# omerbt/Splice

Measured on AMD Instinct MI355X. Metric: opt_steps_per_sec, higher is better.
Workload: dtype bf16

## Files before the change

### include/splice_hip.h

```cpp
#ifndef SPLICE_HIP_H
#define SPLICE_HIP_H
#include <stddef.h>
#include <stdint.h>

#ifdef __cplusplus
extern "C" {
#endif

typedef uint16_t splice_bf16;
typedef void* splice_stream_t;

#define SPLICE_OK 0
#define SPLICE_ERR_ARG -1
#define SPLICE_ERR_HIP -2
#define SPLICE_ERR_STATE -3
#define SPLICE_ERR_NOMEM -4

int splice_version(void);
int splice_dev_switches(void);
const char* splice_last_error(void);

typedef struct splice_gemm_epilogue {
    const float* bias;
    const float* resid;
    int ldr, resid_mod;
    float* out_f32;
    int ldo;
    splice_bf16* out_bf;
    int ldbf;
    splice_bf16* out_bf_t;
    int ldt;
    splice_bf16* out_pre;
    int ldp, pre_row_lo;
    const splice_bf16* aux;
    int ldaux;
    float* out_f32_cols;
    int ld_cols, col_lo, col_hi;
    float alpha;
    int ksplit;
    long long slab_stride;
    const splice_bf16* rd_other;
    int ld_rd, rd_rows;
    float* rowdot;
    const float* row_scale;
    const float* col_scale;
    uint8_t* out_f8;
    int ld8;
    uint8_t* out_f8_t;
    int ldt8;
} splice_gemm_epilogue;

enum {
    SPLICE_EPI_BIAS = 1, SPLICE_EPI_RESID = 2, SPLICE_EPI_OUT_F32 = 4, SPLICE_EPI_OUT_BF = 8,
    SPLICE_EPI_OUT_T = 16, SPLICE_EPI_GELU = 32, SPLICE_EPI_GELU_GRAD = 64,
    SPLICE_EPI_COLS_F32 = 128, SPLICE_EPI_ALPHA = 256, SPLICE_EPI_ROWDOT = 512, SPLICE_EPI_SCALE_RC = 1024, SPLICE_EPI_OUT_F8 = 2048,
    SPLICE_EPI_OUT_F8T = 4096
};

int splice_gemm_nt_bf16(unsigned flags, const splice_bf16* A, int lda, const splice_bf16* B, int ldb,
                        int M, int N, int K, const splice_gemm_epilogue* epi, splice_stream_t stream);

int splice_gemm_nt_fp8(unsigned flags, const uint8_t* A, int lda, const uint8_t* B, int ldb, int M, int N, int K,
                       const splice_gemm_epilogue* epi, splice_stream_t stream);
int splice_quantize_rows_fp8(const float* x, int ldx, uint8_t* q, int ldq, float* scale, int rows, int cols, splice_stream_t stream);
int splice_gemm_splitk_slabs(int M, int ksplit);
int splice_gemm_force_tile(int tile);
int splice_attention_variant(int variant);
int splice_attention_qfold(int on);
int splice_attention_bwd_variant(int variant);

int splice_layernorm_fwd(const float* x, const float* gamma, const float* beta, splice_bf16* y,
                         float* mean, float* rstd, int rows, int D, float eps, splice_stream_t stream);
int splice_layernorm_bwd(const float* dy, const float* x, const float* gamma, const float* mean,
                         const float* rstd, const float* g_in, float* g_out, splice_bf16* g_out_bf,
                         int rows, int D, splice_stream_t stream);

int splice_attention_fwd(const splice_bf16* qkv, const splice_bf16* qkvT, int ldt, int B, int T, int Tld,
                         int D, int H, float scale, splice_bf16* out, float* lse, splice_stream_t stream);
int splice_attention_fwd_fp8(const uint8_t* qkv8, const uint8_t* qkvT8, int ldt8, int B, int T, int Tld, int D, int H, float scale,
                             splice_bf16* out, float* lse, splice_stream_t stream);
int splice_attention_bwd(const splice_bf16* qkv, const splice_bf16* qkvT, int ldt, int B, int T, int Tld,
                         int D, int H, float scale, const splice_bf16* out, const float* lse,
                         const splice_bf16* dout, const splice_bf16* doutT, float* delta,
                         splice_bf16* dqkv, splice_stream_t stream);
int splice_attention_probs(const splice_bf16* qkv, int B, int T, int Tld, int D, int H, float scale,
                           const float* lse, float* probs, splice_stream_t stream);

int splice_augment_structure(const float* img, float* out, float* scratch, int H, int W, int flip, int n_ops, const int* order,
                             const float* factors, float blur_sigma, splice_stream_t stream);

size_t splice_keys_selfsim_ws_bytes(int T, int D);
int splice_keys_selfsim_fwd(const float* K, int ldk, int T, int D, float eps, float* S, void* ws,
                            splice_stream_t stream);
int splice_keys_selfsim_bwd(const float* dS, const float* S, int T, int D, float eps, float* dK, int lddk,
                            int accumulate, void* ws, splice_stream_t stream);

int splice_mse(const float* a, int lda, const float* b, int ldb, int rows, int cols, float weight,
               float* loss_accum, float* grad, int ldg, splice_stream_t stream);

int splice_patchify(const float* img, splice_bf16* patches, int B, int H, int W, int p, int Tld,
                    int normalize, splice_stream_t stream);
int splice_unpatchify(const float* dpatches, float* dimg, int B, int H, int W, int p, int Tld,
                      int normalize, splice_stream_t stream);
int splice_cast_f32_bf16(const float* x, splice_bf16* y, size_t n, splice_stream_t stream);
int splice_cast_bf16_f32(const splice_bf16* x, float* y, size_t n, splice_stream_t stream);
int splice_transpose_f32_bf16(const float* x, splice_bf16* y, int rows, int cols, int ldy, splice_stream_t stream);
int splice_resize_bilinear_fwd(const float* in, float* out, int planes, int h, int w, int oh, int ow, splice_stream_t stream);
int splice_resize_bilinear_bwd(const float* dout, float* din, int planes, int h, int w, int oh, int ow, splice_stream_t stream);

int splice_vit_create(int patch, int dim, int depth, int heads, void** out_handle);
void splice_vit_destroy(void* vit);
int splice_vit_set_param(void* vit, const char* name, const float* data, long long numel, splice_stream_t stream);
float splice_vit_qscale(void* vit);
int splice_vit_params_complete(void* vit);
int splice_vit_enable_fp8(void* vit, splice_stream_t stream);
int splice_vit_ctx_create(void* vit, int B, int H, int W, const float* pos_TD, int need_grad,
                          splice_stream_t stream, void** out_ctx);
void splice_vit_ctx_destroy(void* ctx);
int splice_vit_ctx_info(void* ctx, int* T, int* Tld, int* rows);
int splice_vit_ctx_set_top_cls_only(void* ctx, int on);
int splice_vit_ctx_set_fp8(void* ctx, int mode);
int splice_vit_forward(void* ctx, const float* img, int normalize, splice_stream_t stream);
int splice_vit_forward_ex(void* ctx, const float* img, int normalize, int grad_pass_begin, splice_stream_t stream);
int splice_vit_forward_passes(void* ctx, const float* img, int normalize, int grad_pass_begin, int pass_begin, int pass_end,
                              splice_stream_t stream);
int splice_vit_get_tensor(void* ctx, int kind, int layer, void** out_ptr);
int splice_vit_read_tensor(void* ctx, int kind, int layer, void* dst, size_t bytes, splice_stream_t stream);
int splice_vit_backward(void* ctx, int pass_begin, int pass_end, const float* const* d_block,
                        const float* const* d_qkv, const float* const* d_keys, float* d_img,
                        int normalize, splice_stream_t stream);

int splice_gen_create(void** out_handle);
#define SPLICE_GEN_MAX_SCALES 6
typedef struct splice_gen_arch {
    int n_scales, in_channels, out_channels;
    int down[SPLICE_GEN_MAX_SCALES], up[SPLICE_GEN_MAX_SCALES], skip[SPLICE_GEN_MAX_SCALES];
    int filter_down[SPLICE_GEN_MAX_SCALES], filter_up[SPLICE_GEN_MAX_SCALES];
    int filter_skip;
    int reflect;
} splice_gen_arch;
int splice_gen_create_arch(const splice_gen_arch* arch, void** out_handle);
void splice_gen_destroy(void* gen);
long long splice_gen_param_count(void* gen);
int splice_gen_num_tensors(void* gen);
int splice_gen_tensor_info(void* gen, int i, const char** name, long long* offset, long long* numel);
int splice_gen_plan_create(void* gen, int N, int H, int W, int need_grad, void** out_plan);
void splice_gen_plan_destroy(void* plan);
int splice_gen_forward(void* plan, const float* params, const float* x, float* y, splice_stream_t stream);
int splice_gen_forward_borrowed(void* plan, const float* params, const float* x, float* y, splice_stream_t stream);
int splice_gen_backward(void* plan, const float* params, const float* dy, float* grads, int accumulate,
                        splice_stream_t stream);
long long splice_gen_buffer_count(void* gen);
int splice_gen_num_buffers(void* gen);
int splice_gen_buffer_info(void* gen, int i, const char** name, long long* offset, long long* numel);
int splice_gen_running_stats_update(void* const* plans, int n_plans, float* running, long long running_stride, float momentum,
                                    splice_stream_t stream);
int splice_adam_step(float* params, float* grads, float* m, float* v, long long n, float lr, float beta1,
                     float beta2, float eps, int step, int zero_grad, splice_stream_t stream);
int splice_optim_step(int kind, float* params, float* grads, float* m, float* v, long long n, float lr, float hp0, float hp1,
                      float eps, int step, int zero_grad, splice_stream_t stream);
int splice_optim_step_ex(int kind, float* params, float* grads, const float* g2, float* m, float* v, long long n, float lr,
                         const float* lr_dev, float hp0, float hp1, float eps, int step, int zero_grad, splice_stream_t stream);
int splice_optim_step_pairs(int kind, float* params, float* grads, const float* g2, float* m, float* v, int n_pairs, long long stride,
                            long long n, const float* lr_dev, float hp0, float hp1, float eps, int step, int zero_grad,
                            splice_stream_t stream);
int splice_optim_step_ema(int kind, float* params, float* grads, const float* g2, float* m, float* v, float* ema, long long n, float lr,
                          const float* lr_dev, float hp0, float hp1, float eps, int step, int zero_grad, float ema_decay, int ema_start,
                          splice_stream_t stream);

int splice_prof_begin(int which);
int splice_prof_end(float* total_ms, int* launches);
int splice_prof_end_ex(float* total_ms, int* calls, int* kernels);
int splice_prof_end_detail(float* total_ms, int* calls, int* kernels, char* detail, int detail_len);
int splice_prof_active(void);
int splice_vit_ctx_dims(void* ctx, int* B, int* H, int* W, int* D, int* depth, int* heads, int* patch);
int splice_gen_plan_dims(void* plan, int* N, int* H, int* W, long long* nparams);
int splice_gen_plan_set_arena_stride(void* plan, long long stride);
int splice_gen_plan_set_batch_stats(void* plan, int on);
int splice_gen_plan_set_groups(void* plan, int images_per_group);
int splice_gen_plan_resize(void* plan, int H, int W);

typedef struct splice_step_config {
    int crop_h, crop_w;
    int vit_h, vit_w;
    int ent_h, ent_w;
    int ent_vit_h, ent_vit_w;
    float lambda_global_cls, lambda_global_ssim, lambda_global_identity, lambda_entire_cls, lambda_entire_ssim;
    int entire_every, cls_warmup;
    float lr, beta1, beta2, eps;
    int pairs;
    long long arena_stride;
    int fp8_selfsim;
    int top_cls_only;
    int n_crops;
    int n_crops_b;
} splice_step_config;
#define SPLICE_STEP_MAX_PAIR_CFGS 32
#define SPLICE_STEP_MAX_GROUP_IMAGES 32
int splice_step_create(const splice_step_config* cfg, void* vit_ctx_global, void* vit_ctx_entire, void* gen_plan_a, void* gen_plan_b,
                       void* gen_plan_entire, void** out_handle);
void splice_step_destroy(void* step);
int splice_step_run(void* step, float* params, float* grads, float* m, float* v, const float* A_crop, const float* B_crop,
                    const float* A_entire, int step_idx, float* losses_out, splice_stream_t stream);
int splice_step_output(void* step, int which, float** out_ptr);
int splice_step_graph_stats(void* step, long long* out);
int splice_step_use_graph(void* step, int on);
int splice_step_use_overlap(void* step, int on);
int splice_step_set_crops(void* step, int a_h, int a_w, int b_h, int b_w);
int splice_step_set_mode(void* step, int skip_adam, int accumulate);
int splice_step_set_optimizer(void* step, int kind, float hp0, float hp1, float eps);
int splice_step_set_lr(void* step, float lr);
int splice_step_set_pair_weights(void* step, const float* lambdas);
int splice_step_set_pair_lr(void* step, const float* lr);
int splice_step_set_phases(void* step, int phases, void* leader);
int splice_step_set_running_stats(void* step, float* running, long long stride);

typedef struct splice_stop_state {
    float sum;
    int count;
    int windows;
    float best;
    int bad;
    int stop_step;
} splice_stop_state;
int splice_step_set_stop_rule(void* step, int window, float rel, int patience, int min_steps);
int splice_step_stop_state(void* step, splice_stop_state* out, splice_stream_t stream);
int splice_plateau_update(splice_stop_state* state, const float* losses8, int pairs, int window, float rel, int patience, int min_steps,
                          int step_idx, int counted, splice_stream_t stream);

int splice_step_set_ema(void* step, float* ema, float decay, int start);
int splice_optim_step_pairs_ema(int kind, float* params, float* grads, const float* g2, float* m, float* v, float* ema, int n_pairs,
                                long long stride, long long n, const float* lr_dev, float hp0, float hp1, float eps, const int* step_dev,
                                const splice_stop_state* stop, int zero_grad, float ema_decay, int ema_start, splice_stream_t stream);

#define SPLICE_CLIP_CHUNK 4096
typedef struct splice_clip_state {
    float sumsq;
    float norm;
    float coef;
    int skip;
    int clipped;
    int skipped;
} splice_clip_state;
int splice_grad_norm_pairs(const float* grads, const float* g2, int n_pairs, long long stride, long long n, float max_norm, float* partials,
                           splice_clip_state* state, const splice_stop_state* stop, const int* step_dev, splice_stream_t stream);
int splice_optim_step_pairs_clip(int kind, float* params, float* grads, const float* g2, float* m, float* v, float* ema, int n_pairs,
                                 long long stride, long long n, const float* lr_dev, float hp0, float hp1, float eps, const int* step_dev,
                                 const splice_stop_state* stop, int zero_grad, float ema_decay, int ema_start, const splice_clip_state* clip,
                                 splice_stream_t stream);
int splice_optim_step_clip(int kind, float* params, float* grads, const float* g2, float* m, float* v, float* ema, long long n, float lr,
                           const float* lr_dev, float hp0, float hp1, float eps, int step, int zero_grad, float ema_decay, int ema_start,
                           const splice_clip_state* clip, splice_stream_t stream);
int splice_step_set_grad_clip(void* step, float max_norm, splice_clip_state* state);

#define SPLICE_STOP_HISTORY 64
typedef struct splice_best_state {
    int best_step;
    int best_window;
} splice_best_state;
int splice_plateau_update_best(splice_stop_state* state, splice_best_state* best, float* means, const float* losses8, int pairs, int window,
                               float rel, int patience, int min_steps, int step_idx, int counted, splice_stream_t stream);
int splice_optim_step_pairs_best(int kind, float* params, float* grads, const float* g2, float* m, float* v, float* ema, int n_pairs,
                                 long long stride, long long n, const float* lr_dev, float hp0, float hp1, float eps, const int* step_dev,
                                 const splice_stop_state* stop, int zero_grad, float ema_decay, int ema_start, const splice_clip_state* clip,
                                 const splice_best_state* best, float* best_params, float* best_ema, splice_stream_t stream);
int splice_step_set_keep_best(void* step, float* best_params, float* best_ema, splice_best_state* state, float* means);

int splice_step_set_loss_trace(void* step, float* trace, int capacity);

typedef struct splice_lr_state {
    float scale;
    int bad;
    int cuts;
    int last_cut_step;
} splice_lr_state;
int splice_step_set_lr_plateau(void* step, float factor, int patience, float min_scale, splice_lr_state* state, int* cut_steps);
int splice_plateau_update_lr(splice_stop_state* state, splice_lr_state* lr_state, int* cut_steps, const float* losses8, const float* lr_in,
                             int per_pair, float* lr_eff, int pairs, int window, float rel, int patience, int min_steps, float factor,
                             int lr_patience, float min_scale, int step_idx, int counted, splice_stream_t stream);

size_t splice_selfsim_loss_pairs_ws_bytes(int T, int D, int pairs);
int splice_selfsim_loss_pairs(const splice_bf16* k_tgt, const splice_bf16* k_x, int ldk, size_t k_pstride, const splice_bf16* kT_x, int ldt,
                              size_t kT_pstride, int T, int D, int pairs, float lambda, const float* e_scale_tab, int fp8, float eps,
                              float* loss_part, size_t part_pstride, float* dk, int lddk, size_t dk_pstride, void* ws, splice_stream_t stream);
int splice_mse_pairs(const float* a, int lda, size_t a_ps, const float* b, int ldb, size_t b_ps, int rows, int cols, float loss_weight,
                     float grad_weight, float* part, size_t part_ps, float* grad, int ldg, size_t g_ps, int pairs, const float* grad_tab,
                     splice_stream_t stream);
int splice_total_loss_pairs(float* lbase, size_t lstride, int lp, float w_ssim, float w_essim, float w_ecls, float w_cls, float w_id,
                            float* out8, int pairs, int n_a, int n_b, int n_c, int n_e, const float* wtab, int ssim_on, int entire,
                            splice_stream_t stream);
int splice_total_loss_pairs_trace(float* lbase, size_t lstride, int lp, float w_ssim, float w_essim, float w_ecls, float w_cls, float w_id,
                                  float* out8, int pairs, int n_a, int n_b, int n_c, int n_e, const float* wtab, int ssim_on, int entire,
                                  splice_stop_state* stop, int window, float rel, int patience, int min_steps, const int* dev_t,
                                  float* trace, int capacity, splice_stream_t stream);

int splice_attn_cls_fwd(const splice_bf16* qkv, const splice_bf16* qkvT, int ldt, int B, int T, int Tld, int D, int H, float scale, splice_bf16* out,
                        float* probs, splice_stream_t stream);
int splice_attn_cls_bwd(const splice_bf16* qkv, const splice_bf16* qkvT, int ldt, int B, int T, int Tld, int D, int H, float scale, const float* probs,
                        const float* dout_slabs, int n_slabs, size_t slab_stride, splice_bf16* dqkv, splice_stream_t stream);
int splice_ln_rows_fwd(float* x, size_t xs, const float* gamma, const float* beta, splice_bf16* y, size_t ys, float* mean, float* rstd, size_t ss,
                       int rows, int D, float eps, const float* slabs, int n_slabs, size_t slab_stride, const float* bias, const float* resid, size_t rs,
                       splice_stream_t stream);
int splice_ln_rows_bwd(float* dy, size_t dys, const float* x, size_t xs, const float* gamma, const float* mean, const float* rstd, size_t ss, float* g,
                       splice_bf16* g_bf, int rows, int D, int n_slabs, size_t slab_stride, splice_stream_t stream);
int splice_rows_finish(int mode, const float* slabs, int n_slabs, size_t slab_stride, int rows, int N, const float* bias, const float* resid, size_t rs,
                       float* out_f32, size_t os, splice_bf16* out_bf, splice_bf16* pre_bf, const splice_bf16* aux, size_t ps, int pre_lo,
                       splice_stream_t stream);

typedef struct splice_gen_conv_args {
    const float* in;
    const float* w;
    const float* bias;
    float* out;
    size_t in_nstride, in_cstride, out_nstride, out_cstride, w_jstride, w_cstride, p_nstride;
    int N, Cin, Hi, Wi, Cout, Ho, Wo, ks, stride, pad;
    int reflect, act, transposed, accumulate;
    float* ws;
    size_t ws_floats;
    int p_group, defer_reduce;
} splice_gen_conv_args;
#define SPLICE_GEN_CONV_FORM_INTS 5
int splice_gen_conv(const splice_gen_conv_args* args, int* form_out, splice_stream_t stream);
int splice_gen_conv_pair(const splice_gen_conv_args* a, const splice_gen_conv_args* b, int* forms_out, splice_stream_t stream);
int splice_gen_conv_reflect_dgrad(const splice_gen_conv_args* args, float* pad_scratch, size_t scratch_floats, splice_stream_t stream);

typedef struct splice_gen_wgrad_args {
    const float* x;
    const float* dy;
    float* ws;
    size_t ws_floats;
    size_t x_nstride, x_cstride, dy_nstride, dy_cstride;
    int N, Cin, Hi, Wi, Cout, Ho, Wo, ks, stride, pad, reflect;
} splice_gen_wgrad_args;
#define SPLICE_GEN_WGRAD_FORM_INTS 6
size_t splice_gen_conv_wgrad_ws_floats(int N, int Cin, int Cout, int ks, int Ho, int Wo);
int splice_gen_conv_wgrad(const splice_gen_wgrad_args* args, float* dw, int accumulate, int n_img, size_t p_nstride, int* form_out,
                          splice_stream_t stream);

typedef struct splice_gen_bn_args {
    float* y;
    float* out;
    size_t y_nstride, out_nstride;
    int N, C, HW, batch;
    const float* gamma;
    const float* beta;
    float eps, slope;
    size_t p_nstride;
    float* part;
    size_t part_floats;
    float* mean;
    float* rstd;
    const float* up_src;
    float* up_d_src;
    size_t up_src_ns, up_d_src_ns;
    int up_c0, up_h, up_w, up_Ho, up_Wo;
    const float* slabs;
    const float* bias;
    int ksplit;
    const float* da;
    float* dy;
    size_t da_nstride, dy_nstride;
    float* dgamma;
    float* dbeta;
    int accumulate;
    const float* da_slabs;
    int da_ksplit, da_accumulate;
    float* pre_y;
    size_t pre_y_ns;
    const float* pre_slabs;
    const float* pre_bias;
    int pre_ksplit, pre_C;
    const float* pre_gamma;
    const float* pre_beta;
    float* pre_mean;
    float* pre_rstd;
    float pre_slope;
    float* pre_dy;
    float* pre_dgamma;
    float* pre_dbeta;
} splice_gen_bn_args;
#define SPLICE_GEN_BN_FORM_INTS 7
int splice_gen_bn_form(int HW, int N, size_t p_nstride, int batch, int* out);
size_t splice_gen_bn_part_floats(int N, int C);
int splice_gen_bn_fwd(const splice_gen_bn_args* args, splice_stream_t stream);
int splice_gen_bn_bwd(const splice_gen_bn_args* args, splice_stream_t stream);

int splice_gen_upsample2x_fwd(const float* in, size_t in_nstride, float* out, size_t out_nstride, int N, int C, int h, int w, int Ho, int Wo,
                              splice_stream_t stream);
int splice_gen_upsample2x_bwd(const float* dout, size_t dout_nstride, float* din, size_t din_nstride, int N, int C, int h, int w, int Ho, int Wo,
                              splice_stream_t stream);
size_t splice_gen_sigmoid_bias_part_floats(int N, int C);
int splice_gen_sigmoid_bwd_bias(const float* dout, const float* sout, float* dpre, int N, int C, int HW, float* part, size_t part_floats,
                                size_t p_nstride, int group, int* chunks_out, splice_stream_t stream);

#ifdef __cplusplus
}
#endif
#endif
```

### splice_amd/_lib.py

```python
import ctypes as C
import os

_HERE = os.path.dirname(os.path.abspath(__file__))
LIB_PATH = os.path.join(_HERE, "libsplice_hip.so")

_lib = None


class GemmEpilogue(C.Structure):
    _fields_ = [
        ("bias", C.c_void_p), ("resid", C.c_void_p), ("ldr", C.c_int), ("resid_mod", C.c_int),
        ("out_f32", C.c_void_p), ("ldo", C.c_int),
        ("out_bf", C.c_void_p), ("ldbf", C.c_int),
        ("out_bf_t", C.c_void_p), ("ldt", C.c_int),
        ("out_pre", C.c_void_p), ("ldp", C.c_int), ("pre_row_lo", C.c_int),
        ("aux", C.c_void_p), ("ldaux", C.c_int),
        ("out_f32_cols", C.c_void_p), ("ld_cols", C.c_int), ("col_lo", C.c_int), ("col_hi", C.c_int),
        ("alpha", C.c_float), ("ksplit", C.c_int), ("slab_stride", C.c_longlong),
        ("rd_other", C.c_void_p), ("ld_rd", C.c_int), ("rd_rows", C.c_int), ("rowdot", C.c_void_p),
        ("row_scale", C.c_void_p), ("col_scale", C.c_void_p),
        ("out_f8", C.c_void_p), ("ld8", C.c_int),
        ("out_f8_t", C.c_void_p), ("ldt8", C.c_int),
    ]


class GenArch(C.Structure):
    _fields_ = [("n_scales", C.c_int), ("in_channels", C.c_int), ("out_channels", C.c_int),
                ("down", C.c_int * 6), ("up", C.c_int * 6), ("skip", C.c_int * 6),
                ("filter_down", C.c_int * 6), ("filter_up", C.c_int * 6), ("filter_skip", C.c_int), ("reflect", C.c_int)]


class StepConfig(C.Structure):
    _fields_ = [
        ("crop_h", C.c_int), ("crop_w", C.c_int), ("vit_h", C.c_int), ("vit_w", C.c_int),
        ("ent_h", C.c_int), ("ent_w", C.c_int), ("ent_vit_h", C.c_int), ("ent_vit_w", C.c_int),
        ("lambda_global_cls", C.c_float), ("lambda_global_ssim", C.c_float), ("lambda_global_identity", C.c_float),
        ("lambda_entire_cls", C.c_float), ("lambda_entire_ssim", C.c_float),
        ("entire_every", C.c_int), ("cls_warmup", C.c_int),
        ("lr", C.c_float), ("beta1", C.c_float), ("beta2", C.c_float), ("eps", C.c_float),
        ("pairs", C.c_int), ("arena_stride", C.c_longlong), ("fp8_selfsim", C.c_int), ("top_cls_only", C.c_int), ("n_crops", C.c_int), ("n_crops_b", C.c_int),
    ]


class StopState(C.Structure):
    _fields_ = [("sum", C.c_float), ("count", C.c_int), ("windows", C.c_int), ("best", C.c_float), ("bad", C.c_int), ("stop_step", C.c_int)]


class ClipState(C.Structure):
    _fields_ = [("sumsq", C.c_float), ("norm", C.c_float), ("coef", C.c_float), ("skip", C.c_int), ("clipped", C.c_int), ("skipped", C.c_int)]


class BestState(C.Structure):
    _fields_ = [("best_step", C.c_int), ("best_window", C.c_int)]


class LrState(C.Structure):
    _fields_ = [("scale", C.c_float), ("bad", C.c_int), ("cuts", C.c_int), ("last_cut_step", C.c_int)]


class GenConvArgs(C.Structure):
    _fields_ = [("in", C.c_void_p), ("w", C.c_void_p), ("bias", C.c_void_p), ("out", C.c_void_p)] + \
               [(n, C.c_size_t) for n in ("in_nstride", "in_cstride", "out_nstride", "out_cstride", "w_jstride", "w_cstride", "p_nstride")] + \
               [(n, C.c_int) for n in ("N", "Cin", "Hi", "Wi", "Cout", "Ho", "Wo", "ks", "stride", "pad", "reflect", "act", "transposed", "accumulate")] + \
               [("ws", C.c_void_p), ("ws_floats", C.c_size_t), ("p_group", C.c_int), ("defer_reduce", C.c_int)]


class GenWgradArgs(C.Structure):
    _fields_ = [("x", C.c_void_p), ("dy", C.c_void_p), ("ws", C.c_void_p), ("ws_floats", C.c_size_t)] + \
               [(n, C.c_size_t) for n in ("x_nstride", "x_cstride", "dy_nstride", "dy_cstride")] + \
               [(n, C.c_int) for n in ("N", "Cin", "Hi", "Wi", "Cout", "Ho", "Wo", "ks", "stride", "pad", "reflect")]


class GenBnArgs(C.Structure):
    _fields_ = [("y", C.c_void_p), ("out", C.c_void_p), ("y_nstride", C.c_size_t), ("out_nstride", C.c_size_t),
                ("N", C.c_int), ("C", C.c_int), ("HW", C.c_int), ("batch", C.c_int),
                ("gamma", C.c_void_p), ("beta", C.c_void_p), ("eps", C.c_float), ("slope", C.c_float), ("p_nstride", C.c_size_t),
                ("part", C.c_void_p), ("part_floats", C.c_size_t), ("mean", C.c_void_p), ("rstd", C.c_void_p),
                ("up_src", C.c_void_p), ("up_d_src", C.c_void_p), ("up_src_ns", C.c_size_t), ("up_d_src_ns", C.c_size_t),
                ("up_c0", C.c_int), ("up_h", C.c_int), ("up_w", C.c_int), ("up_Ho", C.c_int), ("up_Wo", C.c_int),
                ("slabs", C.c_void_p), ("bias", C.c_void_p), ("ksplit", C.c_int),
                ("da", C.c_void_p), ("dy", C.c_void_p), ("da_nstride", C.c_size_t), ("dy_nstride", C.c_size_t),
                ("dgamma", C.c_void_p), ("dbeta", C.c_void_p), ("accumulate", C.c_int),
                ("da_slabs", C.c_void_p), ("da_ksplit", C.c_int), ("da_accumulate", C.c_int),
                ("pre_y", C.c_void_p), ("pre_y_ns", C.c_size_t), ("pre_slabs", C.c_void_p), ("pre_bias", C.c_void_p),
                ("pre_ksplit", C.c_int), ("pre_C", C.c_int), ("pre_gamma", C.c_void_p), ("pre_beta", C.c_void_p),
                ("pre_mean", C.c_void_p), ("pre_rstd", C.c_void_p), ("pre_slope", C.c_float),
                ("pre_dy", C.c_void_p), ("pre_dgamma", C.c_void_p), ("pre_dbeta", C.c_void_p)]


GEN_CONV_FORM_INTS, GEN_WGRAD_FORM_INTS, GEN_BN_FORM_INTS = 5, 6, 7

STOP_HISTORY = 64

EPI_BIAS, EPI_RESID, EPI_OUT_F32, EPI_OUT_BF, EPI_OUT_T = 1, 2, 4, 8, 16
EPI_GELU, EPI_GELU_GRAD, EPI_COLS_F32, EPI_ALPHA, EPI_ROWDOT, EPI_SCALE_RC, EPI_OUT_F8, EPI_OUT_F8T = 32, 64, 128, 256, 512, 1024, 2048, 4096

_vp, _i, _f, _sz, _u = C.c_void_p, C.c_int, C.c_float, C.c_size_t, C.c_uint

_SIGNATURES = {
    "splice_version": ([], C.c_int),
    "splice_dev_switches": ([], C.c_int),
    "splice_last_error": ([], C.c_char_p),
    "splice_gemm_nt_bf16": ([_u, _vp, _i, _vp, _i, _i, _i, _i, C.POINTER(GemmEpilogue), _vp], _i),
    "splice_gemm_nt_fp8": ([_u, _vp, _i, _vp, _i, _i, _i, _i, C.POINTER(GemmEpilogue), _vp], _i),
    "splice_quantize_rows_fp8": ([_vp, _i, _vp, _i, _vp, _i, _i, _vp], _i),
    "splice_gemm_splitk_slabs": ([_i, _i], _i),
    "splice_gemm_force_tile": ([_i], _i),
    "splice_attention_variant": ([_i], _i),
    "splice_attention_qfold": ([_i], _i),
    "splice_attention_bwd_variant": ([_i], _i),
    "splice_layernorm_fwd": ([_vp, _vp, _vp, _vp, _vp, _vp, _i, _i, _f, _vp], _i),
    "splice_layernorm_bwd": ([_vp, _vp, _vp, _vp, _vp, _vp, _vp, _vp, _i, _i, _vp], _i),
    "splice_attention_fwd": ([_vp, _vp, _i, _i, _i, _i, _i, _i, _f, _vp, _vp, _vp], _i),
    "splice_attention_fwd_fp8": ([_vp, _vp, _i, _i, _i, _i, _i, _i, _f, _vp, _vp, _vp], _i),
    "splice_attention_bwd": ([_vp, _vp, _i, _i, _i, _i, _i, _i, _f, _vp, _vp, _vp, _vp, _vp, _vp, _vp], _i),
    "splice_attention_probs": ([_vp, _i, _i, _i, _i, _i, _f, _vp, _vp, _vp], _i),
    "splice_augment_structure": ([_vp, _vp, _vp, _i, _i, _i, _i, C.POINTER(C.c_int), C.POINTER(C.c_float), _f, _vp], _i),
    "splice_keys_selfsim_ws_bytes": ([_i, _i], _sz),
    "splice_keys_selfsim_fwd": ([_vp, _i, _i, _i, _f, _vp, _vp, _vp], _i),
    "splice_keys_selfsim_bwd": ([_vp, _vp, _i, _i, _f, _vp, _i, _i, _vp, _vp], _i),
    "splice_mse": ([_vp, _i, _vp, _i, _i, _i, _f, _vp, _vp, _i, _vp], _i),
    "splice_selfsim_loss_pairs_ws_bytes": ([_i, _i, _i], _sz),
    "splice_selfsim_loss_pairs": ([_vp, _vp, _i, _sz, _vp, _i, _sz, _i, _i, _i, _f, _vp, _i, _f, _vp, _sz, _vp, _i, _sz, _vp, _vp], _i),
    "splice_mse_pairs": ([_vp, _i, _sz, _vp, _i, _sz, _i, _i, _f, _f, _vp, _sz, _vp, _i, _sz, _i, _vp, _vp], _i),
    "splice_total_loss_pairs": ([_vp, _sz, _i, _f, _f, _f, _f, _f, _vp, _i, _i, _i, _i, _i, _vp, _i, _i, _vp], _i),
    "splice_attn_cls_fwd": ([_vp, _vp, _i, _i, _i, _i, _i, _i, _f, _vp, _vp, _vp], _i),
    "splice_attn_cls_bwd": ([_vp, _vp, _i, _i, _i, _i, _i, _i, _f, _vp, _vp, _i, _sz, _vp, _vp], _i),
    "splice_ln_rows_fwd": ([_vp, _sz, _vp, _vp, _vp, _sz, _vp, _vp, _sz, _i, _i, _f, _vp, _i, _sz, _vp, _vp, _sz, _vp], _i),
    "splice_ln_rows_bwd": ([_vp, _sz, _vp, _sz, _vp, _vp, _vp, _sz, _vp, _vp, _i, _i, _i, _sz, _vp], _i),
    "splice_rows_finish": ([_i, _vp, _i, _sz, _i, _i, _vp, _vp, _sz, _vp, _sz, _vp, _vp, _vp, _sz, _i, _vp], _i),
    "splice_gen_conv": ([C.POINTER(GenConvArgs), C.POINTER(_i), _vp], _i),
    "splice_gen_conv_pair": ([C.POINTER(GenConvArgs), C.POINTER(GenConvArgs), C.POINTER(_i), _vp], _i),
    "splice_gen_conv_reflect_dgrad": ([C.POINTER(GenConvArgs), _vp, _sz, _vp], _i),
    "splice_gen_conv_wgrad_ws_floats": ([_i, _i, _i, _i, _i, _i], _sz),
    "splice_gen_conv_wgrad": ([C.POINTER(GenWgradArgs), _vp, _i, _i, _sz, C.POINTER(_i), _vp], _i),
    "splice_gen_bn_form": ([_i, _i, _sz, _i, C.POINTER(_i)], _i),
    "splice_gen_bn_part_floats": ([_i, _i], _sz),
    "splice_gen_bn_fwd": ([C.POINTER(GenBnArgs), _vp], _i),
    "splice_gen_bn_bwd": ([C.POINTER(GenBnArgs), _vp], _i),
    "splice_gen_upsample2x_fwd": ([_vp, _sz, _vp, _sz, _i, _i, _i, _i, _i, _i, _vp], _i),
    "splice_gen_upsample2x_bwd": ([_vp, _sz, _vp, _sz, _i, _i, _i, _i, _i, _i, _vp], _i),
    "splice_gen_sigmoid_bias_part_floats": ([_i, _i], _sz),
    "splice_gen_sigmoid_bwd_bias": ([_vp, _vp, _vp, _i, _i, _i, _vp, _sz, _sz, _i, C.POINTER(_i), _vp], _i),
    "splice_patchify": ([_vp, _vp, _i, _i, _i, _i, _i, _i, _vp], _i),
    "splice_unpatchify": ([_vp, _vp, _i, _i, _i, _i, _i, _i, _vp], _i),
    "splice_cast_f32_bf16": ([_vp, _vp, _sz, _vp], _i),
    "splice_cast_bf16_f32": ([_vp, _vp, _sz, _vp], _i),
    "splice_transpose_f32_bf16": ([_vp, _vp, _i, _i, _i, _vp], _i),
    "splice_resize_bilinear_fwd": ([_vp, _vp, _i, _i, _i, _i, _i, _vp], _i),
    "splice_resize_bilinear_bwd": ([_vp, _vp, _i, _i, _i, _i, _i, _vp], _i),
    "splice_vit_create": ([_i, _i, _i, _i, C.POINTER(_vp)], _i),
    "splice_vit_destroy": ([_vp], None),
    "splice_vit_set_param": ([_vp, C.c_char_p, _vp, C.c_longlong, _vp], _i),
    "splice_vit_params_complete": ([_vp], _i),
    "splice_vit_enable_fp8": ([_vp, _vp], _i),
    "splice_vit_ctx_create": ([_vp, _i, _i, _i, _vp, _i, _vp, C.POINTER(_vp)], _i),
    "splice_vit_ctx_destroy": ([_vp], None),
    "splice_vit_ctx_info": ([_vp, C.POINTER(_i), C.POINTER(_i), C.POINTER(_i)], _i),
    "splice_vit_ctx_set_top_cls_only": ([_vp, _i], _i),
    "splice_vit_ctx_set_fp8": ([_vp, _i], _i),
    "splice_vit_forward": ([_vp, _vp, _i, _vp], _i),
    "splice_vit_forward_ex": ([_vp, _vp, _i, _i, _vp], _i),
    "splice_vit_forward_passes": ([_vp, _vp, _i, _i, _i, _i, _vp], _i),
    "splice_vit_get_tensor": ([_vp, _i, _i, C.POINTER(_vp)], _i),
    "splice_vit_qscale": ([_vp], C.c_float),
    "splice_vit_read_tensor": ([_vp, _i, _i, _vp, _sz, _vp], _i),
    "splice_vit_backward": ([_vp, _i, _i, C.POINTER(_vp), C.POINTER(_vp), C.POINTER(_vp), _vp, _i, _vp], _i),
    "splice_gen_create": ([C.POINTER(_vp)], _i),
    "splice_gen_create_arch": ([C.POINTER(GenArch), C.POINTER(_vp)], _i),
    "splice_gen_destroy": ([_vp], None),
    "splice_gen_param_count": ([_vp], C.c_longlong),
    "splice_gen_num_tensors": ([_vp], _i),
    "splice_gen_tensor_info": ([_vp, _i, C.POINTER(C.c_char_p), C.POINTER(C.c_longlong), C.POINTER(C.c_longlong)], _i),
    "splice_gen_plan_create": ([_vp, _i, _i, _i, _i, C.POINTER(_vp)], _i),
    "splice_gen_plan_destroy": ([_vp], None),
    "splice_gen_forward": ([_vp, _vp, _vp, _vp, _vp], _i),
    "splice_gen_forward_borrowed": ([_vp, _vp, _vp, _vp, _vp], _i),
    "splice_gen_backward": ([_vp, _vp, _vp, _vp, _i, _vp], _i),
    "splice_adam_step": ([_vp, _vp, _vp, _vp, C.c_longlong, _f, _f, _f, _f, _i, _i, _vp], _i),
    "splice_optim_step": ([_i, _vp, _vp, _vp, _vp, C.c_longlong, _f, _f, _f, _f, _i, _i, _vp], _i),
    "splice_optim_step_ex": ([_i, _vp, _vp, _vp, _vp, _vp, C.c_longlong, _f, _vp, _f, _f, _f, _i, _i, _vp], _i),
    "splice_optim_step_pairs": ([_i, _vp, _vp, _vp, _vp, _vp, _i, C.c_longlong, C.c_longlong, _vp, _f, _f, _f, _i, _i, _vp], _i),
    "splice_optim_step_ema": ([_i, _vp, _vp, _vp, _vp, _vp, _vp, C.c_longlong, _f, _vp, _f, _f, _f, _i, _i, _f, _i, _vp], _i),
    "splice_optim_step_pairs_ema": ([_i, _vp, _vp, _vp, _vp, _vp, _vp, _i, C.c_longlong, C.c_longlong, _vp, _f, _f, _f, _vp, _vp, _i, _f, _i, _vp], _i),
    "splice_step_set_ema": ([_vp, _vp, _f, _i], _i),
    "splice_grad_norm_pairs": ([_vp, _vp, _i, C.c_longlong, C.c_longlong, _f, _vp, _vp, _vp, _vp, _vp], _i),
    "splice_optim_step_pairs_clip": ([_i, _vp, _vp, _vp, _vp, _vp, _vp, _i, C.c_longlong, C.c_longlong, _vp, _f, _f, _f, _vp, _vp, _i, _f, _i, _vp, _vp], _i),
    "splice_optim_step_clip": ([_i, _vp, _vp, _vp, _vp, _vp, _vp, C.c_longlong, _f, _vp, _f, _f, _f, _i, _i, _f, _i, _vp, _vp], _i),
    "splice_step_set_grad_clip": ([_vp, _f, _vp], _i),
    "splice_plateau_update_best": ([_vp, _vp, _vp, _vp, _i, _i, _f, _i, _i, _i, _i, _vp], _i),
    "splice_optim_step_pairs_best": ([_i, _vp, _vp, _vp, _vp, _vp, _vp, _i, C.c_longlong, C.c_longlong, _vp, _f, _f, _f, _vp, _vp, _i, _f, _i, _vp, _vp, _vp, _vp, _vp], _i),
    "splice_step_set_keep_best": ([_vp, _vp, _vp, _vp, _vp], _i),
    "splice_step_set_loss_trace": ([_vp, _vp, _i], _i),
    "splice_total_loss_pairs_trace": ([_vp, _sz, _i, _f, _f, _f, _f, _f, _vp, _i, _i, _i, _i, _i, _vp, _i, _i, _vp, _i, _f, _i, _i, _vp, _vp, _i, _vp], _i),
    "splice_step_set_lr_plateau": ([_vp, _f, _i, _f, _vp, _vp], _i),
    "splice_plateau_update_lr": ([_vp, _vp, _vp, _vp, _vp, _i, _vp, _i, _i, _f, _i, _i, _f, _i, _f, _i, _i, _vp], _i),
    "splice_prof_begin": ([_i], _i),
    "splice_prof_end": ([C.POINTER(_f), C.POINTER(_i)], _i),
    "splice_prof_end_ex": ([C.POINTER(_f), C.POINTER(_i), C.POINTER(_i)], _i),
    "splice_prof_end_detail": ([C.POINTER(_f), C.POINTER(_i), C.POINTER(_i), C.c_char_p, _i], _i),
    "splice_prof_active": ([], _i),
    "splice_step_use_graph": ([_vp, _i], _i),
    "splice_step_graph_stats": ([_vp, C.POINTER(C.c_longlong)], _i),
    "splice_step_use_overlap": ([_vp, _i], _i),
    "splice_vit_ctx_dims": ([_vp] + [C.POINTER(_i)] * 7, _i),
    "splice_gen_plan_dims": ([_vp, C.POINTER(_i), C.POINTER(_i), C.POINTER(_i), C.POINTER(C.c_longlong)], _i),
    "splice_step_create": ([C.POINTER(StepConfig), _vp, _vp, _vp, _vp, _vp, C.POINTER(_vp)], _i),
    "splice_step_destroy": ([_vp], None),
    "splice_step_run": ([_vp, _vp, _vp, _vp, _vp, _vp, _vp, _vp, _i, _vp, _vp], _i),
    "splice_step_output": ([_vp, _i, C.POINTER(_vp)], _i),
    "splice_step_set_crops": ([_vp, _i, _i, _i, _i], _i),
    "splice_step_set_running_stats": ([_vp, _vp, C.c_longlong], _i),
    "splice_step_set_mode": ([_vp, _i, _i], _i),
    "splice_step_set_optimizer": ([_vp, _i, _f, _f, _f], _i),
    "splice_step_set_lr": ([_vp, _f], _i),
    "splice_step_set_pair_weights": ([_vp, _vp], _i),
    "splice_step_set_pair_lr": ([_vp, _vp], _i),
    "splice_step_set_phases": ([_vp, _i, _vp], _i),
    "splice_step_set_stop_rule": ([_vp, _i, _f, _i, _i], _i),
    "splice_step_stop_state": ([_vp, _vp, _vp], _i),
    "splice_plateau_update": ([_vp, _vp, _i, _i, _f, _i, _i, _i, _i, _vp], _i),
    "splice_gen_buffer_count": ([_vp], C.c_longlong),
    "splice_gen_num_buffers": ([_vp], _i),
    "splice_gen_buffer_info": ([_vp, _i, C.POINTER(C.c_char_p), C.POINTER(C.c_longlong), C.POINTER(C.c_longlong)], _i),
    "splice_gen_running_stats_update": ([C.POINTER(_vp), _i, _vp, C.c_longlong, _f, _vp], _i),
    "splice_gen_plan_resize": ([_vp, _i, _i], _i),
    "splice_gen_plan_set_arena_stride": ([_vp, C.c_longlong], _i),
    "splice_gen_plan_set_batch_stats": ([_vp, _i], _i),
    "splice_gen_plan_set_groups": ([_vp, _i], _i),
}


def exported_symbols():
    return sorted(_SIGNATURES)


def register(name, argtypes, restype):
    _SIGNATURES[name] = (argtypes, restype)


def lib():
    global _lib
    if _lib is None:
        if not os.path.exists(LIB_PATH):
            raise RuntimeError(
                f"{LIB_PATH} not found: the HIP extension is not built "
                "(run __graft_entry__.build() or `make -C splice_amd/csrc`). There is no CPU fallback.")
        _lib = C.CDLL(LIB_PATH)
        for name, (argtypes, restype) in _SIGNATURES.items():
            fn = getattr(_lib, name)
            fn.argtypes = argtypes
            fn.restype = restype
    return _lib


def check(rc, what=""):
    if rc != 0:
        msg = lib().splice_last_error().decode(errors="replace")
        raise RuntimeError(f"libsplice_hip {what} failed (rc={rc}): {msg}")


def ptr(t):
    return None if t is None else C.c_void_p(t.data_ptr())


def current_stream():
    import torch
    return C.c_void_p(torch.cuda.current_stream().cuda_stream)
```

### splice_amd/csrc/capi.hip

```cpp
#include <stdarg.h>
#include <stdio.h>

#include "gen_kernels.h"
#include "kernels.h"

static thread_local char g_err[512] = "";

void splice_set_error(const char* fmt, ...) {
    va_list ap;
    va_start(ap, fmt);
    vsnprintf(g_err, sizeof(g_err), fmt, ap);
    va_end(ap);
}

static int finish(int rc, const char* what) {
    if (rc != SPLICE_OK) {
        splice_set_error("%s: invalid argument", what);
        return rc;
    }
    const hipError_t e = hipGetLastError();
    if (e != hipSuccess) {
        splice_set_error("%s: HIP error %d (%s)", what, (int)e, hipGetErrorString(e));
        return SPLICE_ERR_HIP;
    }
    return SPLICE_OK;
}

#define ST(s) ((hipStream_t)(s))

extern "C" {

int splice_version(void) { return 100; }
int splice_dev_switches(void) {
#ifdef SPLICE_DEV_SWITCHES
    return 1;
#else
    return 0;
#endif
}
const char* splice_last_error(void) { return g_err; }

int splice_gemm_nt_bf16(unsigned flags, const splice_bf16* A, int lda, const splice_bf16* B, int ldb, int M, int N, int K,
                        const splice_gemm_epilogue* epi, splice_stream_t stream) {
    if (!A || !B || !epi) return finish(SPLICE_ERR_ARG, "splice_gemm_nt_bf16");
    return finish(gemm_nt_launch(flags, A, lda, B, ldb, M, N, K, *epi, ST(stream)), "splice_gemm_nt_bf16");
}

int splice_gemm_nt_fp8(unsigned flags, const uint8_t* A, int lda, const uint8_t* B, int ldb, int M, int N, int K,
                       const splice_gemm_epilogue* epi, splice_stream_t stream) {
    if (!A || !B || !epi) return finish(SPLICE_ERR_ARG, "splice_gemm_nt_fp8");
    return finish(gemm_nt_fp8_launch(flags, A, lda, B, ldb, M, N, K, *epi, ST(stream)), "splice_gemm_nt_fp8");
}
int splice_quantize_rows_fp8(const float* x, int ldx, uint8_t* q, int ldq, float* scale, int rows, int cols, splice_stream_t stream) {
    if (!x || !q || !scale) return finish(SPLICE_ERR_ARG, "splice_quantize_rows_fp8");
    return finish(quantize_rows_fp8_launch(x, ldx, q, ldq, scale, rows, cols, ST(stream)), "splice_quantize_rows_fp8");
}

int splice_gemm_splitk_slabs(int M, int ksplit) { return gemm_splitk_slabs(M, ksplit); }

int splice_gemm_force_tile(int tile) { gemm_force_tile(tile); return SPLICE_OK; }
int splice_attention_variant(int variant) { attn_set_variant(variant); return SPLICE_OK; }
int splice_attention_qfold(int on) { attn_set_qfold(on); return SPLICE_OK; }
int splice_attention_bwd_variant(int variant) { attn_set_bwd_variant(variant); return SPLICE_OK; }

int splice_layernorm_fwd(const float* x, const float* gamma, const float* beta, splice_bf16* y, float* mean, float* rstd,
                         int rows, int D, float eps, splice_stream_t stream) {
    return finish(layernorm_fwd_launch(x, gamma, beta, y, mean, rstd, rows, D, eps, ST(stream)), "splice_layernorm_fwd");
}
int splice_layernorm_bwd(const float* dy, const float* x, const float* gamma, const float* mean, const float* rstd,
                         const float* g_in, float* g_out, splice_bf16* g_out_bf, int rows, int D, splice_stream_t stream) {
    return finish(layernorm_bwd_launch(dy, x, gamma, mean, rstd, g_in, g_out, g_out_bf, rows, D, ST(stream)), "splice_layernorm_bwd");
}

int splice_attention_fwd(const splice_bf16* qkv, const splice_bf16* qkvT, int ldt, int B, int T, int Tld, int D, int H,
                         float scale, splice_bf16* out, float* lse, splice_stream_t stream) {
    AttnArgs a = {};
    a.qkv = qkv; a.qkvT = qkvT; a.ldt = ldt; a.B = B; a.T = T; a.Tld = Tld; a.D = D; a.H = H; a.scale = scale;
    a.out = out; a.lse = lse; a.qfold = attn_qfold_hook();
    return finish(attn_fwd_launch(&a, ST(stream)), "splice_attention_fwd");
}
int splice_attention_fwd_fp8(const uint8_t* qkv8, const uint8_t* qkvT8, int ldt8, int B, int T, int Tld, int D, int H, float scale,
                             splice_bf16* out, float* lse, splice_stream_t stream) {
    if (!qkv8 || !qkvT8 || !out || !lse) return finish(SPLICE_ERR_ARG, "splice_attention_fwd_fp8");
    AttnArgs a = {};
    a.qkv8 = qkv8; a.qkvT8 = qkvT8; a.ldt8 = ldt8; a.ldt = 4; a.B = B; a.T = T; a.Tld = Tld; a.D = D; a.H = H; a.scale = scale;
    a.out = out; a.lse = lse;
    return finish(attn_fwd_launch(&a, ST(stream)), "splice_attention_fwd_fp8");
}
int splice_attention_bwd(const splice_bf16* qkv, const splice_bf16* qkvT, int ldt, int B, int T, int Tld, int D, int H,
                         float scale, const splice_bf16* out, const float* lse, const splice_bf16* dout,
                         const splice_bf16* doutT, float* delta, splice_bf16* dqkv, splice_stream_t stream) {
    AttnArgs a = {};
    a.qkv = qkv; a.qkvT = qkvT; a.ldt = ldt; a.B = B; a.T = T; a.Tld = Tld; a.D = D; a.H = H; a.scale = scale;
    a.out = const_cast<splice_bf16*>(out); a.lse = const_cast<float*>(lse);
    a.dout = dout; a.doutT = doutT; a.delta = delta; a.dqkv = dqkv; a.qfold = attn_qfold_hook();
    return finish(attn_bwd_launch(&a, ST(stream)), "splice_attention_bwd");
}
int splice_attention_probs(const splice_bf16* qkv, int B, int T, int Tld, int D, int H, float scale, const float* lse,
                           float* probs, splice_stream_t stream) {
    AttnArgs a = {};
    a.qkv = qkv; a.B = B; a.T = T; a.Tld = Tld; a.D = D; a.H = H; a.scale = scale; a.lse = const_cast<float*>(lse);
    return finish(attn_probs_launch(&a, probs, ST(stream)), "splice_attention_probs");
}

int splice_augment_structure(const float* img, float* out, float* scratch, int H, int W, int flip, int n_ops, const int* order,
                             const float* factors, float blur_sigma, splice_stream_t stream) {
    return finish(augment_structure_launch(img, out, scratch, H, W, flip, n_ops, order, factors, blur_sigma, ST(stream)), "splice_augment_structure");
}

size_t splice_keys_selfsim_ws_bytes(int T, int D) { return selfsim_ws_bytes(T, D); }
int splice_keys_selfsim_fwd(const float* K, int ldk, int T, int D, float eps, float* S, void* ws, splice_stream_t stream) {
    SelfSimWs w;
    selfsim_ws_carve(ws, T, D, &w);
    return finish(selfsim_fwd_launch(K, ldk, T, D, eps, S, w, ST(stream)), "splice_keys_selfsim_fwd");
}
int splice_keys_selfsim_bwd(const float* dS, const float* S, int T, int D, float eps, float* dK, int lddk, int accumulate,
                            void* ws, splice_stream_t stream) {
    SelfSimWs w;
    selfsim_ws_carve(ws, T, D, &w);
    return finish(selfsim_bwd_launch(dS, S, T, D, eps, dK, lddk, accumulate, w, ST(stream)), "splice_keys_selfsim_bwd");
}
int splice_mse(const float* a, int lda, const float* b, int ldb, int rows, int cols, float weight, float* loss_accum,
               float* grad, int ldg, splice_stream_t stream) {
    return finish(mse_launch(a, lda, b, ldb, rows, cols, weight, loss_accum, grad, ldg, ST(stream)), "splice_mse");
}

size_t splice_selfsim_loss_pairs_ws_bytes(int T, int D, int pairs) { return selfsim_batch_ws_bytes(T, D, pairs); }
int splice_selfsim_loss_pairs(const splice_bf16* k_tgt, const splice_bf16* k_x, int ldk, size_t k_pstride, const splice_bf16* kT_x, int ldt,
                              size_t kT_pstride, int T, int D, int pairs, float lambda, const float* e_scale_tab, int fp8, float eps,
                              float* loss_part, size_t part_pstride, float* dk, int lddk, size_t dk_pstride, void* ws, splice_stream_t stream) {
    const char* who = "splice_selfsim_loss_pairs";
    if (!k_tgt || !k_x || !kT_x || !loss_part || !dk || !ws || T < 1 || pairs < 1 || D < 64 || D % 64 || ldk < D || ldk % 8 || ldt % 8 ||
        k_pstride % 8 || kT_pstride % 8 || lddk < D)
        return finish(SPLICE_ERR_ARG, who);
    const int nt = (T + 63) / 64;
    if ((fp8 && D % 128) || (size_t)(nt * (nt + 1) / 2) > part_pstride) return finish(SPLICE_ERR_ARG, who);
    SelfSimBatch b = {};
    selfsim_batch_carve(ws, T, D, pairs, &b);
    b.ldk = ldk; b.ldt = ldt; b.k_pstride = k_pstride; b.kT_pstride = kT_pstride;
    b.k_tgt = k_tgt; b.k_x = k_x; b.kT_x = kT_x;
    b.loss_part = loss_part; b.part_pstride = part_pstride;
    b.dk = dk; b.dk_pstride = dk_pstride; b.lddk = lddk;
    b.eps = eps;
    b.fp8 = fp8 != 0;
    b.loss_scale = 1.0f / ((float)T * (float)T);
    b.e_scale = 4.0f * lambda * b.loss_scale;
    b.e_scale_tab = e_scale_tab;
    const int rc = selfsim_target_launch(b, ST(stream));
    if (rc != SPLICE_OK) return finish(rc, who);
    return finish(selfsim_loss_launch(b, ST(stream)), who);
}
int splice_mse_pairs(const float* a, int lda, size_t a_ps, const float* b, int ldb, size_t b_ps, int rows, int cols, float loss_weight,
                     float grad_weight, float* part, size_t part_ps, float* grad, int ldg, size_t g_ps, int pairs, const float* grad_tab,
                     splice_stream_t stream) {
    if (!a || !b || rows < 1 || cols < 1) return finish(SPLICE_ERR_ARG, "splice_mse_pairs");
    return finish(mse_batched_launch(a, lda, a_ps, b, ldb, b_ps, rows, cols, loss_weight, grad_weight, part, part_ps, grad, ldg, g_ps, pairs,
                                     ST(stream), grad_tab),
                  "splice_mse_pairs");
}

static bool attn_cls_args_ok(const void* qkv, const void* qkvT, int ldt, int B, int T, int Tld, int D, int H, size_t lds) {
    if (!qkv || !qkvT || B < 1 || T < 1 || T > Tld || Tld % 32 || ldt % 8 || (long long)ldt < (long long)B * Tld || D < 64 || D % 64 || H != D / 64)
        return false;
    int dev = 0, lim = 0;
    if (hipGetDevice(&dev) != hipSuccess || hipDeviceGetAttribute(&lim, hipDeviceAttributeMaxSharedMemoryPerBlock, dev) != hipSuccess) return false;
    return lds <= (size_t)(lim < 65536 ? lim : 65536);
}
int splice_attn_cls_fwd(const splice_bf16* qkv, const splice_bf16* qkvT, int ldt, int B, int T, int Tld, int D, int H, float scale, splice_bf16* out,
                        float* probs, splice_stream_t stream) {
    const char* who = "splice_attn_cls_fwd";
    if (!out || !probs || !attn_cls_args_ok(qkv, qkvT, ldt, B, T, Tld, D, H, ((size_t)Tld + Tld / 2 + 256 + 8) * sizeof(float)))
        return finish(SPLICE_ERR_ARG, who);
    return finish(attn_cls_fwd_launch(qkv, qkvT, ldt, B, T, Tld, D, H, scale, out, probs, ST(stream)), who);
}
int splice_attn_cls_bwd(const splice_bf16* qkv, const splice_bf16* qkvT, int ldt, int B, int T, int Tld, int D, int H, float scale, const float* probs,
                        const float* dout_slabs, int n_slabs, size_t slab_stride, splice_bf16* dqkv, splice_stream_t stream) {
    const char* who = "splice_attn_cls_bwd";
    if (!probs || !dout_slabs || !dqkv || n_slabs < 1 || n_slabs > 16 ||
        !attn_cls_args_ok(qkv, qkvT, ldt, B, T, Tld, D, H, ((size_t)Tld + Tld / 2 + 64 + 64 + 32 + 256 + 8) * sizeof(float)))
        return finish(SPLICE_ERR_ARG, who);
    return finish(attn_cls_bwd_launch(qkv, qkvT, ldt, B, T, Tld, D, H, scale, probs, dout_slabs, n_slabs, slab_stride, dqkv, ST(stream)), who);
}
int splice_ln_rows_fwd(float* x, size_t xs, const float* gamma, const float* beta, splice_bf16* y, size_t ys, float* mean, float* rstd, size_t ss,
                       int rows, int D, float eps, const float* slabs, int n_slabs, size_t slab_stride, const float* bias, const float* resid, size_t rs,
                       splice_stream_t stream) {
    const char* who = "splice_ln_rows_fwd";
    if (!x || !gamma || !beta || !y || !mean || !rstd || (slabs && (n_slabs < 1 || !bias || !resid))) return finish(SPLICE_ERR_ARG, who);
    return finish(ln_rows_fwd_launch(x, xs, gamma, beta, y, ys, mean, rstd, ss, rows, D, eps, slabs, n_slabs, slab_stride, bias, resid, rs, ST(stream)), who);
}
int splice_ln_rows_bwd(float* dy, size_t dys, const float* x, size_t xs, const float* gamma, const float* mean, const float* rstd, size_t ss, float* g,
                       splice_bf16* g_bf, int rows, int D, int n_slabs, size_t slab_stride, splice_stream_t stream) {
    const char* who = "splice_ln_rows_bwd";
    if (!dy || !x || !gamma || !mean || !rstd || !g || !g_bf) return finish(SPLICE_ERR_ARG, who);
    return finish(ln_rows_bwd_launch(dy, dys, x, xs, gamma, mean, rstd, ss, g, g_bf, rows, D, n_slabs, slab_stride, ST(stream)), who);
}
int splice_rows_finish(int mode, const float* slabs, int n_slabs, size_t slab_stride, int rows, int N, const float* bias, const float* resid, size_t rs,
                       float* out_f32, size_t os, splice_bf16* out_bf, splice_bf16* pre_bf, const splice_bf16* aux, size_t ps, int pre_lo,
                       splice_stream_t stream) {
    const char* who = "splice_rows_finish";
    if (mode < 0 || mode > 2 || !slabs || n_slabs < 1 || rows < 1 || N < 1 || (long long)rows * N > 0x7fffffffLL) return finish(SPLICE_ERR_ARG, who);
    if ((mode == 0 && (!out_f32 || !resid)) || (mode != 0 && !out_bf) || (mode == 2 && !aux)) return finish(SPLICE_ERR_ARG, who);
    return finish(rows_finish_launch(mode, slabs, n_slabs, slab_stride, rows, N, bias, resid, rs, out_f32, os, out_bf, pre_bf, aux, ps, pre_lo, ST(stream)), who);
}

static bool gen_conv_args_ok(const splice_gen_conv_args* g, bool reflect_dgrad) {
    if (!g || !g->in || !g->w || !g->out) return false;
    if (g->N < 1 || g->Cin < 1 || g->Hi < 1 || g->Wi < 1 || g->Cout < 1 || g->Ho < 1 || g->Wo < 1 || g->pad < 0) return false;
    if (g->ks != 1 && g->ks != 3 && g->ks != 5 && g->ks != 7) return false;
    if (g->stride != 1 && g->stride != 2) return false;
    if ((g->act != 0 && g->act != 1) || (g->reflect && g->transposed && !reflect_dgrad)) return false;
    const long long HWi = (long long)g->Hi * g->Wi, HWo = (long long)g->Ho * g->Wo;
    if (HWi > 0x1fffffffLL || HWo > 0x1fffffffLL) return false;
    if (g->in_cstride < (size_t)HWi || g->out_cstride < (size_t)HWo) return false;
    if (g->N > 1 && (g->in_nstride < (size_t)g->Cin * g->in_cstride || g->out_nstride < (size_t)g->Cout * g->out_cstride)) return false;
    if ((size_t)g->Cin * g->in_cstride > 0x1fffffffULL) return false;
    if ((size_t)g->Cout * g->w_jstride + (size_t)g->Cin * g->w_cstride + (size_t)g->ks * g->ks > 0x1fffffffULL) return false;
    if ((size_t)g->Cout * g->out_cstride > 0x7fffffffULL) return false;
    if (g->w_jstride < 1 || g->w_cstride < 1) return false;
    if (g->p_group < 0 || (g->p_group > 1 && (!g->p_nstride || g->N % g->p_group))) return false;
    if (g->reflect && !reflect_dgrad && (g->pad >= g->Hi || g->pad >= g->Wi)) return false;
    if (reflect_dgrad && (g->pad >= g->Ho || g->pad >= g->Wo || g->act)) return false;
    if (g->ws && g->ws_floats < 1) return false;
    if (g->defer_reduce && !g->ws) return false;
    return true;
}
static ConvArgs gen_conv_fill(const splice_gen_conv_args* g) {
    ConvArgs a = {};
    a.in = g->in; a.w = g->w; a.bias = g->bias; a.out = g->out;
    a.in_nstride = g->in_nstride; a.in_cstride = g->in_cstride; a.out_nstride = g->out_nstride; a.out_cstride = g->out_cstride;
    a.w_jstride = g->w_jstride; a.w_cstride = g->w_cstride; a.p_nstride = g->p_nstride;
    a.N = g->N; a.Cin = g->Cin; a.Hi = g->Hi; a.Wi = g->Wi; a.Cout = g->Cout; a.Ho = g->Ho; a.Wo = g->Wo;
    a.ks = g->ks; a.stride = g->stride; a.pad = g->pad;
    a.reflect = g->reflect; a.act = g->act; a.transposed = g->transposed; a.accumulate = g->accumulate;
    a.ws = g->ws; a.ws_floats = g->ws_floats; a.p_group = g->p_group; a.defer_reduce = g->defer_reduce;
    return a;
}
int splice_gen_conv(const splice_gen_conv_args* args, int* form_out, splice_stream_t stream) {
    const char* who = "splice_gen_conv";
    if (!gen_conv_args_ok(args, false)) return finish(SPLICE_ERR_ARG, who);
    const ConvArgs a = gen_conv_fill(args);
    if (form_out) conv_form_report(a, form_out);
    return finish(conv_launch(a, ST(stream)), who);
}
int splice_gen_conv_pair(const splice_gen_conv_args* a_args, const splice_gen_conv_args* b_args, int* forms_out, splice_stream_t stream) {
    const char* who = "splice_gen_conv_pair";
    if (!gen_conv_args_ok(a_args, false) || !gen_conv_args_ok(b_args, false)) return finish(SPLICE_ERR_ARG, who);
    const ConvArgs a = gen_conv_fill(a_args), b = gen_conv_fill(b_args);
    if (forms_out) { conv_form_report(a, forms_out); conv_form_report(b, forms_out + SPLICE_GEN_CONV_FORM_INTS); }
    return finish(conv_pair_launch(a, b, ST(stream)), who);
}
int splice_gen_conv_reflect_dgrad(const splice_gen_conv_args* args, float* pad_scratch, size_t scratch_floats, splice_stream_t stream) {
    const char* who = "splice_gen_conv_reflect_dgrad";
    if (!gen_conv_args_ok(args, true) || !pad_scratch) return finish(SPLICE_ERR_ARG, who);
    const size_t Hp = (size_t)args->Ho + 2 * args->pad, Wp = (size_t)args->Wo + 2 * args->pad;
    if (scratch_floats < (size_t)args->N * args->Cout * Hp * Wp || (size_t)args->Cout * Hp * Wp > 0x7fffffffULL) return finish(SPLICE_ERR_ARG, who);
    return finish(conv_reflect_dgrad_launch(gen_conv_fill(args), pad_scratch, ST(stream)), who);
}

static bool gen_wgrad_args_ok(const splice_gen_wgrad_args* g) {
    if (!g || !g->x || !g->dy) return false;
    if (g->N < 1 || g->Cin < 1 || g->Hi < 1 || g->Wi < 1 || g->Cout < 1 || g->Ho < 1 || g->Wo < 1 || g->pad < 0 || g->pad > 255) return false;
    if (g->ks != 1 && g->ks != 3 && g->ks != 5 && g->ks != 7) return false;
    if ((g->stride != 1 && g->stride != 2) || g->Cout > 128) return false;
    if (g->Hi > 65535 || g->Wi > 65535 || g->Ho > 65535 || g->Wo > 65535 || g->Cin > 65535) return false;
    const long long HWi = (long long)g->Hi * g->Wi, HWo = (long long)g->Ho * g->Wo;
    if (HWo > (1LL << 22)) return false;
    if (g->x_cstride < (size_t)HWi || g->dy_cstride < (size_t)HWo) return false;
    if (g->N > 1 && (g->x_nstride < (size_t)g->Cin * g->x_cstride || g->dy_nstride < (size_t)g->Cout * g->dy_cstride)) return false;
    if ((size_t)g->Cin * g->x_cstride > 0x1fffffffULL || (size_t)g->Cout * g->dy_cstride > 0x1fffffffULL) return false;
    if (g->x_nstride > 0xffffffffULL || g->dy_nstride > 0xffffffffULL) return false;
    if (g->reflect && (g->pad >= g->Hi || g->pad >= g->Wi)) return false;
    return true;
}
size_t splice_gen_conv_wgrad_ws_floats(int N, int Cin, int Cout, int ks, int Ho, int Wo) {
    if (N < 1 || Cin < 1 || Cout < 1 || ks < 1 || Ho < 1 || Wo < 1) return 0;
    int ppc = 0, cpi = 0;
    return (size_t)wgrad_chunks(N, Ho, Wo, &ppc, &cpi) * Cout * Cin * ks * ks;
}
int splice_gen_conv_wgrad(const splice_gen_wgrad_args* args, float* dw, int accumulate, int n_img, size_t p_nstride, int* form_out, splice_stream_t stream) {
    const char* who = "splice_gen_conv_wgrad";
    if (!gen_wgrad_args_ok(args) || !dw || !args->ws) return finish(SPLICE_ERR_ARG, who);
    const size_t n = (size_t)args->Cout * args->Cin * args->ks * args->ks;
    if (n > 0x7fffffffULL || args->ws_floats < splice_gen_conv_wgrad_ws_floats(args->N, args->Cin, args->Cout, args->ks, args->Ho, args->Wo))
        return finish(SPLICE_ERR_ARG, who);
    if (p_nstride ? (n_img != args->N || p_nstride < n) : n_img != 1) return finish(SPLICE_ERR_ARG, who);
    WgradArgs a = {};
    a.x = args->x; a.dy = args->dy; a.ws = args->ws;
    a.x_nstride = args->x_nstride; a.x_cstride = args->x_cstride; a.dy_nstride = args->dy_nstride; a.dy_cstride = args->dy_cstride;
    a.N = args->N; a.Cin = args->Cin; a.Hi = args->Hi; a.Wi = args->Wi; a.Cout = args->Cout; a.Ho = args->Ho; a.Wo = args->Wo;
    a.ks = args->ks; a.stride = args->stride; a.pad = args->pad; a.reflect = args->reflect;
    WgradBatchPair pair = {};
    int chunks = 0;
    int rc = conv_wgrad_add(&pair, a, &chunks);
    if (rc != SPLICE_OK) return finish(rc, who);
    WgradReduceAll r = {};
    r.count = 1; r.n[0] = (int)n; r.chunks[0] = chunks; r.ws_off[0] = 0; r.dw_off[0] = 0;
    if (form_out) {
        const WgradBatch& b = pair.tile.count ? pair.tile : pair.big.count ? pair.big : pair.small;
        form_out[0] = pair.tile.count ? 2 : pair.big.count ? 1 : 0;
        form_out[1] = b.d[0].variant;
        form_out[2] = b.d[0].pix_per_chunk;
        form_out[3] = chunks;
        form_out[4] = !((reinterpret_cast<size_t>(args->ws) | reinterpret_cast<size_t>(dw)) & 15) && p_nstride % 4 == 0 && n % 4 == 0;
        form_out[5] = b.total_wgs;
    }
    rc = conv_wgrad_batched_launch(pair, ST(stream));
    if (rc != SPLICE_OK) return finish(rc, who);
    return finish(wgrad_reduce_all_launch(r, args->ws, dw, accumulate, ST(stream), n_img, p_nstride), who);
}

int splice_gen_bn_form(int HW, int N, size_t p_nstride, int batch, int* out) {
    if (HW < 1 || N < 1 || batch < 0 || !out) return finish(SPLICE_ERR_ARG, "splice_gen_bn_form");
    const BnForm f = bn_form(HW, N, p_nstride, batch);
    out[0] = (int)f.kind; out[1] = f.hosts_pre; out[2] = f.fwd_takes_slabs; out[3] = f.bwd_takes_slabs;
    out[4] = f.fwd_fuses_upsample; out[5] = f.bwd_fuses_upsample; out[6] = f.sign_from_y;
    return SPLICE_OK;
}
size_t splice_gen_bn_part_floats(int N, int C) { return N < 1 || C < 1 ? 0 : (size_t)bn_part_floats(N, C); }
static bool gen_bn_fill(const splice_gen_bn_args* g, bool bwd, BnArgs* a, BnUpsample* up, BnPre* pre, BnSlabs* sl) {
    if (!g || !g->y || !g->out || !g->gamma || !g->mean || !g->rstd) return false;
    if (g->N < 1 || g->C < 1 || g->HW < 1 || g->N > 65535 || g->C > 65535 || g->batch < 0 || g->batch > 8) return false;
    if (g->batch && (g->N % g->batch || (g->N != g->batch && !g->p_nstride))) return false;
    if (g->N > 1 && (g->y_nstride < (size_t)g->C * g->HW || g->out_nstride < (size_t)g->C * g->HW)) return false;
    const BnForm f = bn_form(g->HW, g->N, g->p_nstride, g->batch);
    const bool two_stage = f.kind == BnForm::TWO_STAGE || f.kind == BnForm::TWO_STAGE_VEC;
    if (two_stage && (!g->part || g->part_floats < (size_t)bn_part_floats(g->N, g->C))) return false;
    if (!bwd && !g->beta) return false;
    if (bwd && ((f.sign_from_y && !g->beta) || !g->da || !g->dy || !g->dgamma || !g->dbeta)) return false;
    if (bwd && g->N > 1 && (g->da_nstride < (size_t)g->C * g->HW || g->dy_nstride < (size_t)g->C * g->HW)) return false;
    a->y = g->y; a->y_nstride = g->y_nstride; a->out = g->out; a->out_nstride = g->out_nstride;
    a->N = g->N; a->C = g->C; a->HW = g->HW; a->gamma = g->gamma; a->beta = g->beta; a->eps = g->eps; a->slope = g->slope;
    a->p_nstride = g->p_nstride; a->batch = g->batch; a->part = g->part; a->mean = g->mean; a->rstd = g->rstd;
    if (g->up_src || g->up_d_src) {
        if (bwd ? !g->up_d_src : !g->up_src) return false;
        if (g->up_c0 < 0 || g->up_c0 >= g->C || g->up_h < 1 || g->up_w < 1 || g->up_Ho < 1 || g->up_Wo < 1) return false;
        if (g->up_Ho > 2 * g->up_h || g->up_Wo > 2 * g->up_w || (long long)g->up_Ho * g->up_Wo != g->HW) return false;
        const size_t src = (size_t)(g->C - g->up_c0) * g->up_h * g->up_w;
        if (g->N > 1 && (bwd ? g->up_d_src_ns : g->up_src_ns) < src) return false;
        up->src = g->up_src; up->src_ns = g->up_src_ns; up->d_src = g->up_d_src; up->d_src_ns = g->up_d_src_ns;
        up->c0 = g->up_c0; up->h = g->up_h; up->w = g->up_w; up->Ho = g->up_Ho; up->Wo = g->up_Wo;
        a->up = up;
    }
    if (g->pre_y) {
        if (!g->pre_gamma || !g->pre_beta || !g->pre_mean || !g->pre_rstd || g->pre_C < 1 || g->pre_C > (a->up ? g->up_c0 : g->C)) return false;
        if (g->N > 1 && g->pre_y_ns < (size_t)g->pre_C * g->HW) return false;
        if (g->pre_slabs && (bwd || !f.fwd_takes_slabs || g->pre_ksplit < 1 || g->pre_ksplit > 16)) return false;
        if (bwd && (!g->pre_dy || !g->pre_dgamma || !g->pre_dbeta)) return false;
        pre->y = g->pre_y; pre->y_ns = g->pre_y_ns; pre->slabs = g->pre_slabs; pre->ksplit = g->pre_ksplit; pre->bias = g->pre_bias;
        pre->gamma = g->pre_gamma; pre->beta = g->pre_beta; pre->mean = g->pre_mean; pre->rstd = g->pre_rstd; pre->slope = g->pre_slope; pre->C = g->pre_C;
        pre->dy = g->pre_dy; pre->dgamma = g->pre_dgamma; pre->dbeta = g->pre_dbeta;
        a->pre = pre;
    }
    if (!bwd && g->slabs) {
        if (g->ksplit < 2 || g->ksplit > 16) return false;
        a->slabs = g->slabs; a->ksplit = g->ksplit; a->bias = g->bias;
    }
    if (bwd) {
        a->da = g->da; a->da_nstride = g->da_nstride; a->dy = g->dy; a->dy_nstride = g->dy_nstride;
        a->dgamma = g->dgamma; a->dbeta = g->dbeta; a->accumulate = g->accumulate;
        if (g->da_slabs) {
            if (g->da_ksplit < 1 || g->da_ksplit > 16) return false;
            sl->slabs = g->da_slabs; sl->ksplit = g->da_ksplit; sl->accumulate = g->da_accumulate;
            a->da_slabs = sl;
        }
    }
    return true;
}
int splice_gen_bn_fwd(const splice_gen_bn_args* args, splice_stream_t stream) {
    BnArgs a; BnUpsample up; BnPre pre; BnSlabs sl;
    if (!gen_bn_fill(args, false, &a, &up, &pre, &sl)) return finish(SPLICE_ERR_ARG, "splice_gen_bn_fwd");
    return finish(bn_fwd_launch(a, ST(stream)), "splice_gen_bn_fwd");
}
int splice_gen_bn_bwd(const splice_gen_bn_args* args, splice_stream_t stream) {
    BnArgs a; BnUpsample up; BnPre pre; BnSlabs sl;
    if (!gen_bn_fill(args, true, &a, &up, &pre, &sl)) return finish(SPLICE_ERR_ARG, "splice_gen_bn_bwd");
    return finish(bn_bwd_launch(a, ST(stream)), "splice_gen_bn_bwd");
}

static bool gen_up_args_ok(const void* a, const void* b, size_t in_ns, size_t out_ns, int N, int C, int h, int w, int Ho, int Wo) {
    if (!a || !b || N < 1 || C < 1 || h < 1 || w < 1 || Ho < 1 || Wo < 1 || N > 65535 || C > 65535) return false;
    if (Ho > 2 * h || Wo > 2 * w || (long long)h * w > 0x7fffffffLL / 4 || (long long)Ho * Wo > 0x7fffffffLL) return false;
    return N == 1 || (in_ns >= (size_t)C * h * w && out_ns >= (size_t)C * Ho * Wo);
}
int splice_gen_upsample2x_fwd(const float* in, size_t in_nstride, float* out, size_t out_nstride, int N, int C, int h, int w, int Ho, int Wo,
                              splice_stream_t stream) {
    if (!gen_up_args_ok(in, out, in_nstride, out_nstride, N, C, h, w, Ho, Wo)) return finish(SPLICE_ERR_ARG, "splice_gen_upsample2x_fwd");
    return finish(upsample2x_fwd_launch(in, in_nstride, out, out_nstride, N, C, h, w, Ho, Wo, ST(stream)), "splice_gen_upsample2x_fwd");
}
int splice_gen_upsample2x_bwd(const float* dout, size_t dout_nstride, float* din, size_t din_nstride, int N, int C, int h, int w, int Ho, int Wo,
                              splice_stream_t stream) {
    if (!gen_up_args_ok(din, dout, din_nstride, dout_nstride, N, C, h, w, Ho, Wo)) return finish(SPLICE_ERR_ARG, "splice_gen_upsample2x_bwd");
    return finish(upsample2x_bwd_launch(dout, dout_nstride, din, din_nstride, N, C, h, w, Ho, Wo, ST(stream)), "splice_gen_upsample2x_bwd");
}
size_t splice_gen_sigmoid_bias_part_floats(int N, int C) { return N < 1 || C < 1 ? 0 : (size_t)sigmoid_bias_part_floats(N, C); }
int splice_gen_sigmoid_bwd_bias(const float* dout, const float* sout, float* dpre, int N, int C, int HW, float* part, size_t part_floats, size_t p_nstride,
                                int group, int* chunks_out, splice_stream_t stream) {
    const char* who = "splice_gen_sigmoid_bwd_bias";
    if (!dout || !sout || !dpre || !part || N < 1 || C < 1 || HW < 1 || N > 65535 || C > 65535 || group < 1) return finish(SPLICE_ERR_ARG, who);
    if (part_floats < splice_gen_sigmoid_bias_part_floats(N, C) || (group > 1 && !p_nstride) || N % group) return finish(SPLICE_ERR_ARG, who);
    return finish(sigmoid_bwd_bias_launch(dout, sout, dpre, N, C, HW, part, ST(stream), p_nstride, chunks_out, group), who);
}

int splice_patchify(const float* img, splice_bf16* patches, int B, int H, int W, int p, int Tld, int normalize,
                    splice_stream_t stream) {
    return finish(patchify_launch(img, patches, B, H, W, p, Tld, normalize, ST(stream)), "splice_patchify");
}
int splice_unpatchify(const float* dpatches, float* dimg, int B, int H, int W, int p, int Tld, int normalize,
                      splice_stream_t stream) {
    return finish(unpatchify_launch(dpatches, dimg, B, H, W, p, Tld, normalize, ST(stream)), "splice_unpatchify");
}
int splice_cast_f32_bf16(const float* x, splice_bf16* y, size_t n, splice_stream_t stream) {
    return finish(cast_f32_bf16_launch(x, y, n, ST(stream)), "splice_cast_f32_bf16");
}
int splice_cast_bf16_f32(const splice_bf16* x, float* y, size_t n, splice_stream_t stream) {
    return finish(cast_bf16_f32_launch(x, y, n, ST(stream)), "splice_cast_bf16_f32");
}
int splice_resize_bilinear_fwd(const float* in, float* out, int planes, int h, int w, int oh, int ow, splice_stream_t stream) {
    return finish(resize_bilinear_fwd_launch(in, out, planes, h, w, oh, ow, ST(stream)), "splice_resize_bilinear_fwd");
}
int splice_resize_bilinear_bwd(const float* dout, float* din, int planes, int h, int w, int oh, int ow, splice_stream_t stream) {
    return finish(resize_bilinear_bwd_launch(dout, din, planes, h, w, oh, ow, ST(stream)), "splice_resize_bilinear_bwd");
}
int splice_transpose_f32_bf16(const float* x, splice_bf16* y, int rows, int cols, int ldy, splice_stream_t stream) {
    return finish(transpose_f32_to_bf16_launch(x, y, rows, cols, ldy, ST(stream)), "splice_transpose_f32_bf16");
}
}
```

### splice_amd/csrc/gen_bn.hip

```cpp
#include "gen_device.h"
#include "plateau.h"
#include <atomic>
#include <cstdlib>

__device__ __forceinline__ float part_sum(const float* __restrict__ pp, int PB, int comp, int lane) {
    if (PB <= MAX_PB) return wave_sum(lane < PB ? pp[2 * lane + comp] : 0.f);
    float a = 0.f;
    for (int b = lane; b < PB; b += 64) a += pp[2 * b + comp];
    return wave_sum(a);
}

__global__ __launch_bounds__(256) void bn_stats_partial_kernel(const float* y, size_t nstride, int C, int HW, int PB,
                                                               float* __restrict__ part , BnUpsample up) {
    __shared__ float red[8];
    const int pb = blockIdx.x, c = blockIdx.y, img = blockIdx.z;
    const int seg = seg_len(HW, PB), lo = pb * seg, hi = min(lo + seg, HW);
    const float* p = y + (size_t)img * nstride + (size_t)c * HW;
    float s = 0.f, dummy = 0.f;
    const bool in_regs = seg <= 1024;
    float keep[4] = {0.f, 0.f, 0.f, 0.f};
    if (up.src && c >= up.c0) {
        const float* sp = up.src + (size_t)img * up.src_ns + (size_t)(c - up.c0) * up.h * up.w;
        float* yo = const_cast<float*>(p);
        if (in_regs) {
#pragma unroll
            for (int k = 0; k < 4; ++k) {
                const int i = lo + threadIdx.x + k * 256;
                if (i < hi) {
                    const float v = up_value(sp, up.h, up.w, i / up.Wo, i % up.Wo);
                    yo[i] = v;
                    keep[k] = v;
                    s += v;
                }
            }
        } else {
            for (int i = lo + threadIdx.x; i < hi; i += 256) {
                const float v = up_value(sp, up.h, up.w, i / up.Wo, i % up.Wo);
                yo[i] = v;
                s += v;
            }
        }
    } else if (in_regs) {
#pragma unroll
        for (int k = 0; k < 4; ++k) {
            const int i = lo + threadIdx.x + k * 256;
            keep[k] = i < hi ? p[i] : 0.f;
        }
#pragma unroll
        for (int k = 0; k < 4; ++k)
            if (lo + threadIdx.x + k * 256 < hi) s += keep[k];
    } else {
        for (int i = lo + threadIdx.x; i < hi; i += 256) s += p[i];
    }
    block_sum2(s, dummy, red);
    const int cnt = hi - lo;
    const float m = cnt > 0 ? s / (float)cnt : 0.f;
    float sq = 0.f;
    dummy = 0.f;
    if (in_regs) {
#pragma unroll
        for (int k = 0; k < 4; ++k)
            if (lo + threadIdx.x + k * 256 < hi) { const float d = keep[k] - m; sq = __builtin_fmaf(d, d, sq); }
    } else {
        for (int i = lo + threadIdx.x; i < hi; i += 256) { const float d = p[i] - m; sq = __builtin_fmaf(d, d, sq); }
    }
    block_sum2(sq, dummy, red);
    if (threadIdx.x == 0) {
        float* o = part + (((size_t)img * C + c) * PB + pb) * 2;
        o[0] = m;
        o[1] = sq;
    }
}

__global__ __launch_bounds__(256) void bn_stats_partial_v_kernel(const float* y, size_t nstride, int C, int HW, int PB,
                                                                 float* __restrict__ part , BnUpsample up) {
    __shared__ float red[8];
    const int pb = blockIdx.x, c = blockIdx.y, img = blockIdx.z;
    const int seg = seg_len(HW, PB), lo = pb * seg, hi = min(lo + seg, HW);
    const float* p = y + (size_t)img * nstride + (size_t)c * HW;
    float keep[BN_V_CH][4];
    if (up.src && c >= up.c0) {
        const float* sp = up.src + (size_t)img * up.src_ns + (size_t)(c - up.c0) * up.h * up.w;
        float* yo = const_cast<float*>(p);
#pragma unroll
        for (int k = 0; k < BN_V_CH; ++k) {
            const int i = lo + 4 * (threadIdx.x + 256 * k);
            int oy = i / up.Wo, ox = i - oy * up.Wo;
#pragma unroll
            for (int j = 0; j < 4; ++j) {
                keep[k][j] = i + j < hi ? up_value(sp, up.h, up.w, oy, ox) : 0.f;
                if (++ox == up.Wo) { ox = 0; ++oy; }
            }
            if (i < hi) st_run(yo, i, hi, keep[k]);
        }
    } else {
#pragma unroll
        for (int k = 0; k < BN_V_CH; ++k) ld_run(p, lo + 4 * (threadIdx.x + 256 * k), hi, keep[k]);
    }
    float s = 0.f, dummy = 0.f;
#pragma unroll
    for (int k = 0; k < BN_V_CH; ++k)
#pragma unroll
        for (int j = 0; j < 4; ++j) s += keep[k][j];
    block_sum2(s, dummy, red);
    const int cnt = hi - lo;
    const float m = cnt > 0 ? s / (float)cnt : 0.f;
    float sq = 0.f;
    dummy = 0.f;
#pragma unroll
    for (int k = 0; k < BN_V_CH; ++k)
#pragma unroll
        for (int j = 0; j < 4; ++j)
            if (lo + 4 * ((int)threadIdx.x + 256 * k) + j < hi) { const float d = keep[k][j] - m; sq = __builtin_fmaf(d, d, sq); }
    block_sum2(sq, dummy, red);
    if (threadIdx.x == 0) {
        float* o = part + (((size_t)img * C + c) * PB + pb) * 2;
        o[0] = m;
        o[1] = sq;
    }
}

__device__ __forceinline__ void bn_combine_wave_raw(const float* part, int PB, int HW, float& mean, float& M2out);
__device__ __forceinline__ void bn_combine_wave(const float* part, int PB, int HW, float eps, float& mean, float& rstd) {
    float M2;
    bn_combine_wave_raw(part, PB, HW, mean, M2);
    rstd = rsqrtf(M2 / (float)HW + eps);
}
__device__ __forceinline__ void bn_combine_wave_raw(const float* part, int PB, int HW, float& mean, float& M2out) {
    const int lane = threadIdx.x & 63;
    const int seg = seg_len(HW, PB), lo = lane * seg;
    int cnt = lane < PB ? min(lo + seg, HW) - lo : 0;
    cnt = cnt > 0 ? cnt : 0;
    float n = (float)cnt, m = cnt > 0 ? part[2 * lane] : 0.f, M2 = cnt > 0 ? part[2 * lane + 1] : 0.f;
    if (PB > MAX_PB) {
        const int G = (PB + 63) >> 6;
        n = 0.f; m = 0.f; M2 = 0.f;
        for (int g = 0; g < G; ++g) {
            const int b = lane * G + g, blo = b * seg;
            const int bc = b < PB ? min(blo + seg, HW) - blo : 0;
            if (bc > 0) {
                const float nb = (float)bc, mb = part[2 * b], Mb = part[2 * b + 1];
                const float nt = n + nb, d = mb - m, w = nb / nt;
                m += d * w;
                M2 += Mb + d * d * n * w;
                n = nt;
            }
        }
    }
#pragma unroll
    for (int off = 32; off > 0; off >>= 1) {
        const float nb = __shfl_down(n, off, 64), mb = __shfl_down(m, off, 64), Mb = __shfl_down(M2, off, 64);
        const float nt = n + nb;
        if (nb > 0.f) {
            const float d = mb - m, w = nb / nt;
            m += d * w;
            M2 += Mb + d * d * n * w;
            n = nt;
        }
    }
    mean = __shfl(m, 0, 64);
    M2out = __shfl(M2, 0, 64);
}
__device__ __forceinline__ size_t bn_arena(int img, size_t p_nstride, int batch) { return (size_t)(batch ? img / batch : img) * p_nstride; }
__device__ __forceinline__ void bn_combine_batch(const float* part_c0 , size_t img_stride, int N, int PB, int HW, float eps,
                                                 float& mean, float& rstd) {
    float n = 0.f, m = 0.f, M2 = 0.f;
    for (int i = 0; i < N; ++i) {
        float mb, Mb;
        bn_combine_wave_raw(part_c0 + (size_t)i * img_stride, PB, HW, mb, Mb);
        const float nb = (float)HW, nt = n + nb, d = mb - m, w = nb / nt;
        m += d * w;
        M2 += Mb + d * d * n * w;
        n = nt;
    }
    mean = m;
    rstd = rsqrtf(M2 / n + eps);
}

__device__ __forceinline__ float bn_shift(float beta, float mean, float sc) { return __builtin_fmaf(-mean, sc, beta); }
__device__ __forceinline__ float bn_affine(float y, float sc, float sh) { return __builtin_fmaf(y, sc, sh); }
__global__ __launch_bounds__(256) void bn_act_kernel(const float* __restrict__ y, size_t y_nstride, float* __restrict__ out,
                                                     size_t out_nstride, int C, int HW, int PB, const float* __restrict__ gamma,
                                                     const float* __restrict__ beta, const float* __restrict__ part, float eps,
                                                     float* __restrict__ mean_o, float* __restrict__ rstd_o, float slope, size_t p_nstride, int batch) {
    __shared__ float st[2];
    const int c = blockIdx.y, img = blockIdx.z;
    gamma += bn_arena(img, p_nstride, batch); beta += bn_arena(img, p_nstride, batch);
    if (threadIdx.x < 64) {
        float m, r;
        if (batch) bn_combine_batch(part + ((size_t)(img / batch * batch) * C + c) * PB * 2, (size_t)C * PB * 2, batch, PB, HW, eps, m, r);
        else bn_combine_wave(part + ((size_t)img * C + c) * PB * 2, PB, HW, eps, m, r);
        if (threadIdx.x == 0) {
            st[0] = m; st[1] = r;
            if (blockIdx.x == 0) { mean_o[img * C + c] = m; rstd_o[img * C + c] = r; }
        }
    }
    __syncthreads();
    const float sc = gamma[c] * st[1];
    const float sh = beta[c] - st[0] * sc;
    const float* p = y + (size_t)img * y_nstride + (size_t)c * HW;
    float* q = out + (size_t)img * out_nstride + (size_t)c * HW;
    if (PB > MAX_PB) {
        const int seg = seg_len(HW, PB), lo = blockIdx.x * seg, hi = min(lo + seg, HW);
        float v[BN_V_CH][4];
#pragma unroll
        for (int k = 0; k < BN_V_CH; ++k) ld_run(p, lo + 4 * (threadIdx.x + 256 * k), hi, v[k]);
        const float shv = bn_shift(beta[c], st[0], sc);
#pragma unroll
        for (int k = 0; k < BN_V_CH; ++k) {
            const int i = lo + 4 * (threadIdx.x + 256 * k);
#pragma unroll
            for (int j = 0; j < 4; ++j) {
                const float t = bn_affine(v[k][j], sc, shv);
                v[k][j] = t > 0.f ? t : t * slope;
            }
            if (i < hi) st_run(q, i, hi, v[k]);
        }
        return;
    }
    for (int i = blockIdx.x * 256 + threadIdx.x; i < HW; i += gridDim.x * 256) {
        const float v = p[i] * sc + sh;
        q[i] = v > 0.f ? v : v * slope;
    }
}

__global__ __launch_bounds__(256) void bn_bwd_partial_kernel(const float* __restrict__ da, size_t da_nstride, const float* __restrict__ aout,
                                                             size_t a_nstride, const float* __restrict__ y, size_t y_nstride, int C, int HW,
                                                             int PB, const float* __restrict__ mean, const float* __restrict__ rstd,
                                                             float slope, float* __restrict__ part ,
                                                             const float* __restrict__ gamma, const float* __restrict__ beta, size_t p_nstride) {
    __shared__ float red[8];
    const int pb = blockIdx.x, c = blockIdx.y, img = blockIdx.z;
    const int seg = seg_len(HW, PB), lo = pb * seg, hi = min(lo + seg, HW);
    const float m = mean[img * C + c], r = rstd[img * C + c];
    const float* pd = da + (size_t)img * da_nstride + (size_t)c * HW;
    const float* pa = aout + (size_t)img * a_nstride + (size_t)c * HW;
    const float* py = y + (size_t)img * y_nstride + (size_t)c * HW;
    float s1 = 0.f, s2 = 0.f;
    if (PB > MAX_PB) {
        const bool act = slope != 1.0f, from_y = act && beta != nullptr;
        float d[BN_V_CH][4], a[BN_V_CH][4], yy[BN_V_CH][4];
#pragma unroll
        for (int k = 0; k < BN_V_CH; ++k) {
            const int i = lo + 4 * (threadIdx.x + 256 * k);
            ld_run(pd, i, hi, d[k]);
            ld_run(py, i, hi, yy[k]);
            if (act && !from_y) ld_run(pa, i, hi, a[k]);
        }
        float sc = 0.f, sh = 0.f;
        if (from_y) { sc = gamma[(size_t)img * p_nstride + c] * r; sh = bn_shift(beta[(size_t)img * p_nstride + c], m, sc); }
#pragma unroll
        for (int k = 0; k < BN_V_CH; ++k)
#pragma unroll
            for (int j = 0; j < 4; ++j) {
                float dz = d[k][j];
                const float av = from_y ? bn_affine(yy[k][j], sc, sh) : a[k][j];
                if (act && !(av > 0.f)) dz *= slope;
                s1 += dz;
                s2 += dz * (yy[k][j] - m) * r;
            }
    } else
    for (int i = lo + threadIdx.x; i < hi; i += 256) {
        float dz = pd[i];
        if (slope != 1.0f && !(pa[i] > 0.f)) dz *= slope;
        s1 += dz;
        s2 += dz * (py[i] - m) * r;
    }
    block_sum2(s1, s2, red);
    if (threadIdx.x == 0) {
        float* o = part + (((size_t)img * C + c) * PB + pb) * 2;
        o[0] = s1;
        o[1] = s2;
    }
}

__global__ __launch_bounds__(256) void bn_bwd_apply_kernel(const float* __restrict__ da, size_t da_nstride, const float* __restrict__ aout,
                                                           size_t a_nstride, const float* __restrict__ y, size_t y_nstride,
                                                           float* __restrict__ dy, size_t dy_nstride, int C, int HW, int N, int PB,
                                                           const float* __restrict__ gamma, const float* __restrict__ mean,
                                                           const float* __restrict__ rstd, float slope, const float* __restrict__ part,
                                                           float* __restrict__ dgamma, float* __restrict__ dbeta, int accumulate, size_t p_nstride, int batch,
                                                           const float* __restrict__ beta) {
    __shared__ float st[2];
    const int c = blockIdx.y, img = blockIdx.z;
    gamma += bn_arena(img, p_nstride, batch);
    if (threadIdx.x < 64) {
        const int lane = threadIdx.x;
        const float* pp = part + ((size_t)img * C + c) * PB * 2;
        const float a = part_sum(pp, PB, 0, lane), b = part_sum(pp, PB, 1, lane);
        if (lane == 0) { st[0] = a; st[1] = b; }
        if (p_nstride) {
            if (!batch && blockIdx.x == 0 && lane == 0) {
                float* dg = dgamma + (size_t)img * p_nstride + c;
                float* db = dbeta + (size_t)img * p_nstride + c;
                const float g = 0.f + b, be = 0.f + a;
                *dg = accumulate ? *dg + g : g;
                *db = accumulate ? *db + be : be;
            }
        } else if (img == 0 && blockIdx.x == 0) {
            float g = 0.f, be = 0.f;
            for (int n = 0; n < N; ++n) {
                const float* pn = part + ((size_t)n * C + c) * PB * 2;
                be += part_sum(pn, PB, 0, lane);
                g += part_sum(pn, PB, 1, lane);
            }
            if (lane == 0) {
                dgamma[c] = accumulate ? dgamma[c] + g : g;
                dbeta[c] = accumulate ? dbeta[c] + be : be;
            }
        }
    }
    if (batch && threadIdx.x < 64) {
        const int lane = threadIdx.x, n0 = img / batch * batch;
        float a = 0.f, b = 0.f;
        for (int n = 0; n < batch; ++n) {
            const float* pn = part + ((size_t)(n0 + n) * C + c) * PB * 2;
            a += part_sum(pn, PB, 0, lane);
            b += part_sum(pn, PB, 1, lane);
        }
        if (lane == 0) {
            st[0] = a; st[1] = b;
            if (p_nstride && img == n0 && blockIdx.x == 0) {
                float* dg = dgamma + bn_arena(img, p_nstride, batch) + c;
                float* db = dbeta + bn_arena(img, p_nstride, batch) + c;
                *dg = accumulate ? *dg + b : b;
                *db = accumulate ? *db + a : a;
            }
        }
    }
    __syncthreads();
    const float m = mean[img * C + c], r = rstd[img * C + c];
    const float cnt = batch ? (float)HW * (float)batch : (float)HW;
    const float k1 = st[0] / cnt, k2 = st[1] / cnt;
    const float gr = gamma[c] * r;
    const float* pd = da + (size_t)img * da_nstride + (size_t)c * HW;
    const float* pa = aout + (size_t)img * a_nstride + (size_t)c * HW;
    const float* py = y + (size_t)img * y_nstride + (size_t)c * HW;
    float* po = dy + (size_t)img * dy_nstride + (size_t)c * HW;
    if (PB > MAX_PB) {
        const int seg = seg_len(HW, PB), lo = blockIdx.x * seg, hi = min(lo + seg, HW);
        const bool act = slope != 1.0f, from_y = act && beta != nullptr;
        float d[BN_V_CH][4], a[BN_V_CH][4], yy[BN_V_CH][4];
#pragma unroll
        for (int k = 0; k < BN_V_CH; ++k) {
            const int i = lo + 4 * (threadIdx.x + 256 * k);
            ld_run(pd, i, hi, d[k]);
            ld_run(py, i, hi, yy[k]);
            if (act && !from_y) ld_run(pa, i, hi, a[k]);
        }
        const float sc = gr, sh = from_y ? bn_shift(beta[bn_arena(img, p_nstride, batch) + c], m, sc) : 0.f;
#pragma unroll
        for (int k = 0; k < BN_V_CH; ++k) {
            const int i = lo + 4 * (threadIdx.x + 256 * k);
#pragma unroll
            for (int j = 0; j < 4; ++j) {
                float dz = d[k][j];
                const float av = from_y ? bn_affine(yy[k][j], sc, sh) : a[k][j];
                if (act && !(av > 0.f)) dz *= slope;
                d[k][j] = gr * (dz - k1 - (yy[k][j] - m) * r * k2);
            }
            if (i < hi) st_run(po, i, hi, d[k]);
        }
        return;
    }
    for (int i = blockIdx.x * 256 + threadIdx.x; i < HW; i += gridDim.x * 256) {
        float dz = pd[i];
        if (slope != 1.0f && !(pa[i] > 0.f)) dz *= slope;
        po[i] = gr * (dz - k1 - (py[i] - m) * r * k2);
    }
}

__device__ __forceinline__ void rounded(float& x) { asm volatile("" : "+v"(x)); }
__device__ __forceinline__ float bn_dz(float d, float a, float slope, bool act) {
    if (act && !(a > 0.f)) { d *= slope; rounded(d); }
    return d;
}
__device__ __forceinline__ float bn_xhat(float y, float m, float r) {
    float x = (y - m) * r;
    rounded(x);
    return x;
}
__device__ __forceinline__ float bn_dy(float gr, float dz, float k1, float xh, float k2) {
    float t = xh * k2;
    rounded(t);
    float g = gr * ((dz - k1) - t);
    rounded(g);
    return g;
}
constexpr int BN_SMALL_HW = 4096;
constexpr int BN_MAX_BATCH = 8;
constexpr int BN_SMALL_PER = BN_SMALL_HW / 256;
constexpr int BN_UP_SRC = 34 * 34;
template <int PER>
__global__ __launch_bounds__(256) void bn_small_fwd_kernel(const float* y, size_t y_nstride, float* __restrict__ out,
                                                           size_t out_nstride, int C, int HW, const float* __restrict__ gamma,
                                                           const float* __restrict__ beta, float eps, float* __restrict__ mean_o,
                                                           float* __restrict__ rstd_o, float slope, const float* __restrict__ slabs,
                                                           int ksplit, const float* __restrict__ bias, float* __restrict__ y_out, BnUpsample up,
                                                           size_t p_nstride, int batch, BnPre pre) {
    __shared__ float red[8];
    __shared__ float up_src_s[BN_UP_SRC];
    const int c = blockIdx.x, img = blockIdx.y;
    gamma += bn_arena(img, p_nstride, batch); beta += bn_arena(img, p_nstride, batch);
    if (bias) bias += bn_arena(img, p_nstride, batch);
    const float* p = y + (size_t)img * y_nstride + (size_t)c * HW;
    float* q = out + (size_t)img * out_nstride + (size_t)c * HW;
    float v[PER];
    float s = 0.f, dummy = 0.f;
    if (pre.y && c < pre.C) {
        const float* py1 = pre.y + (size_t)img * pre.y_ns + (size_t)c * HW;
        if (pre.slabs) {
            const size_t per = (size_t)gridDim.y * pre.C * HW;
            const float* sp = pre.slabs + ((size_t)img * pre.C + c) * HW;
            float* yo = const_cast<float*>(py1);
            const float b = pre.bias ? pre.bias[(size_t)img * p_nstride + c] : 0.f;
#pragma unroll
            for (int k = 0; k < PER; ++k) v[k] = b;
            for (int ks = 0; ks < pre.ksplit; ks += 4) {
                float t[4][PER];
#pragma unroll
                for (int u = 0; u < 4; ++u) {
                    if (ks + u >= pre.ksplit) continue;
                    const float* sk = sp + (size_t)(ks + u) * per;
#pragma unroll
                    for (int k = 0; k < PER; ++k) {
                        if (k * 256 >= HW) continue;
                        const int i = threadIdx.x + k * 256;
                        t[u][k] = sk[i < HW ? i : 0];
                    }
                }
#pragma unroll
                for (int u = 0; u < 4; ++u) {
                    if (ks + u >= pre.ksplit) continue;
#pragma unroll
                    for (int k = 0; k < PER; ++k)
                        if (k * 256 < HW) v[k] += t[u][k];
                }
            }
#pragma unroll
            for (int k = 0; k < PER; ++k) {
                const int i = threadIdx.x + k * 256;
                if (i < HW) yo[i] = v[k]; else v[k] = 0.f;
            }
        } else {
#pragma unroll
            for (int k = 0; k < PER; ++k) {
                const int i = threadIdx.x + k * 256;
                v[k] = k * 256 < HW ? py1[i < HW ? i : 0] : 0.f;
            }
#pragma unroll
            for (int k = 0; k < PER; ++k)
                if (threadIdx.x + k * 256 >= HW) v[k] = 0.f;
        }
        float s1 = 0.f, d1 = 0.f;
#pragma unroll
        for (int k = 0; k < PER; ++k) s1 += v[k];
        block_sum2(s1, d1, red);
        const float m1 = s1 / (float)HW;
        float q1 = 0.f;
        d1 = 0.f;
#pragma unroll
        for (int k = 0; k < PER; ++k) {
            const float d = threadIdx.x + k * 256 < HW ? v[k] - m1 : 0.f;
            q1 += d * d;
        }
        block_sum2(q1, d1, red);
        const float r1 = rsqrtf(q1 / (float)HW + eps);
        if (threadIdx.x == 0) { pre.mean[img * pre.C + c] = m1; pre.rstd[img * pre.C + c] = r1; }
        const float sc1 = pre.gamma[(size_t)img * p_nstride + c] * r1;
        const float sh1 = pre.beta[(size_t)img * p_nstride + c] - m1 * sc1;
        float* yo2 = const_cast<float*>(p);
#pragma unroll
        for (int k = 0; k < PER; ++k) {
            const int i = threadIdx.x + k * 256;
            const float t = v[k] * sc1 + sh1;
            v[k] = i < HW ? (t > 0.f ? t : t * pre.slope) : 0.f;
            rounded(v[k]);
            if (i < HW) yo2[i] = v[k];
            s += v[k];
        }
    } else if (slabs) {
        const size_t per = (size_t)gridDim.y * C * HW;
        const float* sp = slabs + ((size_t)img * C + c) * HW;
        float* yo = y_out + (size_t)img * y_nstride + (size_t)c * HW;
        const float b = bias ? bias[c] : 0.f;
#pragma unroll
        for (int k = 0; k < PER; ++k) v[k] = b;
        for (int ks = 0; ks < ksplit; ks += 4) {
            float t[4][PER];
#pragma unroll
            for (int u = 0; u < 4; ++u) {
                if (ks + u >= ksplit) continue;
                const float* sk = sp + (size_t)(ks + u) * per;
#pragma unroll
                for (int k = 0; k < PER; ++k) {
                    if (k * 256 >= HW) continue;
                    const int i = threadIdx.x + k * 256;
                    t[u][k] = sk[i < HW ? i : 0];
                }
            }
#pragma unroll
            for (int u = 0; u < 4; ++u) {
                if (ks + u >= ksplit) continue;
#pragma unroll
                for (int k = 0; k < PER; ++k)
                    if (k * 256 < HW) v[k] += t[u][k];
            }
        }
#pragma unroll
        for (int k = 0; k < PER; ++k) {
            const int i = threadIdx.x + k * 256;
            if (i < HW) yo[i] = v[k]; else v[k] = 0.f;
            s += v[k];
        }
    } else if (up.src && c >= up.c0) {
        const float* sp = up.src + (size_t)img * up.src_ns + (size_t)(c - up.c0) * up.h * up.w;
        float* yo = const_cast<float*>(p);
        const bool in_lds = up.h * up.w <= BN_UP_SRC;
        if (in_lds) {
            for (int e = threadIdx.x; e < up.h * up.w; e += 256) up_src_s[e] = sp[e];
            __syncthreads();
        }
#pragma unroll
        for (int k = 0; k < PER; ++k) {
            const int i = threadIdx.x + k * 256;
            v[k] = 0.f;
            if (k * 256 < HW) {
                const int ii = i < HW ? i : HW - 1;
                const int oy = ii / up.Wo, ox = ii - oy * up.Wo;
                v[k] = in_lds ? up_value((const float*)up_src_s, up.h, up.w, oy, ox) : up_value(sp, up.h, up.w, oy, ox);
                if (i < HW) yo[i] = v[k];
            }
        }
#pragma unroll
        for (int k = 0; k < PER; ++k) {
            if (threadIdx.x + k * 256 >= HW) v[k] = 0.f;
            s += v[k];
        }
    } else {
#pragma unroll
        for (int k = 0; k < PER; ++k) {
            const int i = threadIdx.x + k * 256;
            v[k] = k * 256 < HW ? p[i < HW ? i : 0] : 0.f;
        }
#pragma unroll
        for (int k = 0; k < PER; ++k) {
            if (threadIdx.x + k * 256 >= HW) v[k] = 0.f;
            s += v[k];
        }
    }
    block_sum2(s, dummy, red);
    float m = s / (float)HW;
    float sq = 0.f;
    dummy = 0.f;
    float cnt = (float)HW;
    if (batch) {
        const int N = batch;
        const float* yg = y + (size_t)(img / batch * batch) * y_nstride;
        float tot = 0.f;
        for (int n = 0; n < N; ++n) {
            const float* pn = yg + (size_t)n * y_nstride + (size_t)c * HW;
            float sn = 0.f, d2 = 0.f;
#pragma unroll
            for (int k = 0; k < PER; ++k) {
                const int i = threadIdx.x + k * 256;
                if (k * 256 < HW) sn += i < HW ? pn[i] : 0.f;
            }
            block_sum2(sn, d2, red);
            tot += sn;
        }
        cnt = (float)HW * (float)N;
        m = tot / cnt;
        for (int n = 0; n < N; ++n) {
            const float* pn = yg + (size_t)n * y_nstride + (size_t)c * HW;
            float qn = 0.f, d2 = 0.f;
#pragma unroll
            for (int k = 0; k < PER; ++k) {
                const int i = threadIdx.x + k * 256;
                if (k * 256 < HW) { const float d = i < HW ? pn[i] - m : 0.f; qn += d * d; }
            }
            block_sum2(qn, d2, red);
            sq += qn;
        }
    } else {
#pragma unroll
        for (int k = 0; k < PER; ++k) {
            const float d = threadIdx.x + k * 256 < HW ? v[k] - m : 0.f;
            sq += d * d;
        }
        block_sum2(sq, dummy, red);
    }
    const float r = rsqrtf(sq / cnt + eps);
    if (threadIdx.x == 0) { mean_o[img * C + c] = m; rstd_o[img * C + c] = r; }
    const float sc = gamma[c] * r;
    const float sh = beta[c] - m * sc;
#pragma unroll
    for (int k = 0; k < PER; ++k) {
        const int i = threadIdx.x + k * 256;
        if (i < HW) {
            const float t = v[k] * sc + sh;
            q[i] = t > 0.f ? t : t * slope;
        }
    }
}
template <int PER>
__device__ __forceinline__ void bn_small_bwd_sums(const float* pd, const float* pa, const float* py, int HW, float m, float r, float slope,
                                                  float (&dz)[PER], float (&xh)[PER], float& s1, float& s2, float* red,
                                                  const float* sp = nullptr, size_t per = 0, int ksplit = 0, int sl_acc = 0) {
    s1 = 0.f; s2 = 0.f;
    const bool act = slope != 1.0f;
    float vd[PER], va[PER], vy[PER];
#pragma unroll
    for (int k = 0; k < PER; ++k) {
        if (k * 256 >= HW) continue;
        const int i = threadIdx.x + k * 256;
        const int j = i < HW ? i : 0;
        vd[k] = (!sp || sl_acc) ? pd[j] : 0.f;
        vy[k] = py[j];
        va[k] = act ? pa[j] : 1.f;
    }
    if (sp) {
        float v[PER];
#pragma unroll
        for (int k = 0; k < PER; ++k) v[k] = 0.f;
        for (int ks = 0; ks < ksplit; ks += 4) {
            float t[4][PER];
#pragma unroll
            for (int u = 0; u < 4; ++u) {
                if (ks + u >= ksplit) continue;
                const float* sk = sp + (size_t)(ks + u) * per;
#pragma unroll
                for (int k = 0; k < PER; ++k) {
                    if (k * 256 >= HW) continue;
                    const int i = threadIdx.x + k * 256;
                    t[u][k] = sk[i < HW ? i : 0];
                }
            }
#pragma unroll
            for (int u = 0; u < 4; ++u) {
                if (ks + u >= ksplit) continue;
#pragma unroll
                for (int k = 0; k < PER; ++k)
                    if (k * 256 < HW) v[k] += t[u][k];
            }
        }
#pragma unroll
        for (int k = 0; k < PER; ++k)
            if (k * 256 < HW) vd[k] = sl_acc ? vd[k] + v[k] : v[k];
    }
#pragma unroll
    for (int k = 0; k < PER; ++k) {
        const int i = threadIdx.x + k * 256;
        float d = 0.f, x = 0.f;
        if (k * 256 < HW) {
            d = bn_dz(vd[k], va[k], slope, act);
            x = bn_xhat(vy[k], m, r);
            if (i >= HW) { d = 0.f; x = 0.f; }
        }
        dz[k] = d; xh[k] = x;
        s1 += d;
        s2 = __builtin_fmaf(d, x, s2);
    }
    block_sum2(s1, s2, red);
}
template <int PER>
__global__ __launch_bounds__(256) void bn_small_bwd_kernel(const float* __restrict__ da, size_t da_nstride, const float* __restrict__ aout,
                                                           size_t a_nstride, const float* __restrict__ y, size_t y_nstride,
                                                           float* __restrict__ dy, size_t dy_nstride, int C, int HW, int N,
                                                           const float* __restrict__ gamma, const float* __restrict__ mean,
                                                           const float* __restrict__ rstd, float slope, float* __restrict__ dgamma,
                                                           float* __restrict__ dbeta, int accumulate, BnUpsample up, size_t p_nstride, int batch, BnPre pre,
                                                           BnSlabs sl) {
    __shared__ float red[8];
    __shared__ float up_grad_s[BN_SMALL_HW];
    const int c = blockIdx.x, img = blockIdx.y;
    gamma += bn_arena(img, p_nstride, batch);
    const int n0 = batch ? img / batch * batch : 0;
    float dz[PER], xh[PER];
    float s1, s2;
    const bool chained = pre.y && c < pre.C;
    {
        const float m = mean[img * C + c], r = rstd[img * C + c];
        float b1 = 0.f, b2 = 0.f;
        if (batch) {
            float t1s[BN_MAX_BATCH], t2s[BN_MAX_BATCH];
#pragma unroll
            for (int n = 0; n < BN_MAX_BATCH; ++n) {
                t1s[n] = 0.f; t2s[n] = 0.f;
                const int gn = n0 + n;
                if (n < batch && gn != img)
                    bn_small_bwd_sums<PER>(da + (size_t)gn * da_nstride + (size_t)c * HW, aout + (size_t)gn * a_nstride + (size_t)c * HW,
                                      y + (size_t)gn * y_nstride + (size_t)c * HW, HW, mean[gn * C + c], rstd[gn * C + c], slope, dz, xh, t1s[n], t2s[n], red);
            }
            bn_small_bwd_sums<PER>(da + (size_t)img * da_nstride + (size_t)c * HW, aout + (size_t)img * a_nstride + (size_t)c * HW,
                              y + (size_t)img * y_nstride + (size_t)c * HW, HW, m, r, slope, dz, xh, s1, s2, red);
#pragma unroll
            for (int n = 0; n < BN_MAX_BATCH; ++n)
                if (n < batch) { b1 += n0 + n == img ? s1 : t1s[n]; b2 += n0 + n == img ? s2 : t2s[n]; }
        } else {
            bn_small_bwd_sums<PER>(da + (size_t)img * da_nstride + (size_t)c * HW, aout + (size_t)img * a_nstride + (size_t)c * HW,
                              y + (size_t)img * y_nstride + (size_t)c * HW, HW, m, r, slope, dz, xh, s1, s2, red,
                              sl.slabs ? sl.slabs + ((size_t)img * C + c) * HW : nullptr, (size_t)gridDim.y * C * HW, sl.ksplit, sl.accumulate);
        }
        const float cnt = batch ? (float)HW * (float)batch : (float)HW;
        const float k1 = (batch ? b1 : s1) / cnt, k2 = (batch ? b2 : s2) / cnt;
        if (batch) { s1 = b1; s2 = b2; }
        const float gr = gamma[c] * r;
        float* po = dy + (size_t)img * dy_nstride + (size_t)c * HW;
        const bool through_adjoint = up.d_src && c >= up.c0;
#pragma unroll
        for (int k = 0; k < PER; ++k) {
            const int i = threadIdx.x + k * 256;
            if (i < HW) {
                const float gv = bn_dy(gr, dz[k], k1, xh[k], k2);
                if (through_adjoint) up_grad_s[i] = gv; else if (chained) dz[k] = gv; else po[i] = gv;
            } else if (chained) dz[k] = 0.f;
        }
        if (chained) {
            const float m1 = pre.mean[img * pre.C + c], r1 = pre.rstd[img * pre.C + c];
            const float* pa1 = y + (size_t)img * y_nstride + (size_t)c * HW;
            const float* py1 = pre.y + (size_t)img * pre.y_ns + (size_t)c * HW;
            float va[PER], vy[PER];
#pragma unroll
            for (int k = 0; k < PER; ++k) {
                if (k * 256 >= HW) continue;
                const int i = threadIdx.x + k * 256, j = i < HW ? i : 0;
                va[k] = pa1[j];
                vy[k] = py1[j];
            }
            float t1 = 0.f, t2 = 0.f;
#pragma unroll
            for (int k = 0; k < PER; ++k) {
                const int i = threadIdx.x + k * 256;
                float d = 0.f, x = 0.f;
                if (k * 256 < HW && i < HW) {
                    d = bn_dz(dz[k], va[k], pre.slope, true);
                    x = bn_xhat(vy[k], m1, r1);
                }
                dz[k] = d; xh[k] = x;
                t1 += d;
                t2 = __builtin_fmaf(d, x, t2);
            }
            block_sum2(t1, t2, red);
            const float j1 = t1 / (float)HW, j2 = t2 / (float)HW;
            const float gr1 = pre.gamma[(size_t)img * p_nstride + c] * r1;
            float* pd1 = pre.dy + (size_t)img * pre.y_ns + (size_t)c * HW;
#pragma unroll
            for (int k = 0; k < PER; ++k) {
                const int i = threadIdx.x + k * 256;
                if (i < HW) pd1[i] = bn_dy(gr1, dz[k], j1, xh[k], j2);
            }
            if (threadIdx.x == 0) {
                float* dg = pre.dgamma + (size_t)img * p_nstride + c;
                float* db = pre.dbeta + (size_t)img * p_nstride + c;
                *dg = accumulate ? *dg + t2 : t2;
                *db = accumulate ? *db + t1 : t1;
            }
        }
        if (through_adjoint) {
            __syncthreads();
            float* qd = up.d_src + (size_t)img * up.d_src_ns + (size_t)(c - up.c0) * up.h * up.w;
            for (int e = threadIdx.x; e < up.h * up.w; e += 256)
                qd[e] = up_adjoint_value((const float*)up_grad_s, up.h, up.w, up.Ho, up.Wo, e / up.w, e % up.w);
        }
    }
    if (p_nstride) {
        if (threadIdx.x == 0 && (!batch || img == n0)) {
            float* dg = dgamma + bn_arena(img, p_nstride, batch) + c;
            float* db = dbeta + bn_arena(img, p_nstride, batch) + c;
            *dg = accumulate ? *dg + s2 : s2;
            *db = accumulate ? *db + s1 : s1;
        }
        return;
    }
    if (img != 0) return;
    float g = s2, be = s1;
    for (int n = 1; n < (batch ? 0 : N); ++n) {
        float t1, t2;
        bn_small_bwd_sums<PER>(da + (size_t)n * da_nstride + (size_t)c * HW, aout + (size_t)n * a_nstride + (size_t)c * HW,
                          y + (size_t)n * y_nstride + (size_t)c * HW, HW, mean[n * C + c], rstd[n * C + c], slope, dz, xh, t1, t2, red);
        be += t1;
        g += t2;
    }
    if (threadIdx.x == 0) {
        dgamma[c] = accumulate ? dgamma[c] + g : g;
        dbeta[c] = accumulate ? dbeta[c] + be : be;
    }
}

constexpr int BN_MID_HW = 16384;
constexpr int BN_MID_THREADS = 1024;
__device__ __forceinline__ void block_sum2_1024(float& a, float& b, float* red ) {
    a = wave_sum(a);
    b = wave_sum(b);
    const int w = threadIdx.x >> 6;
    __syncthreads();
    if ((threadIdx.x & 63) == 0) { red[w] = a; red[16 + w] = b; }
    __syncthreads();
    float sa = 0.f, sb = 0.f;
#pragma unroll
    for (int k = 0; k < 16; ++k) { sa += red[k]; sb += red[16 + k]; }
    a = sa; b = sb;
}
constexpr int BN_MID_SRC = 4096;
template <class F4, class F1>
__device__ __forceinline__ void bn_mid_for(int HW, bool vec, F4&& f4, F1&& f1) {
    const int n4 = vec ? HW >> 2 : 0;
    for (int i = threadIdx.x; i < n4; i += BN_MID_THREADS) f4(i);
    for (int i = n4 * 4 + threadIdx.x; i < HW; i += BN_MID_THREADS) f1(i);
}
__global__ __launch_bounds__(BN_MID_THREADS) void bn_mid_fwd_kernel(const float* y, size_t y_nstride, float* __restrict__ out, size_t out_nstride, int C, int HW,
                                                                    const float* __restrict__ gamma, const float* __restrict__ beta, float eps,
                                                                    float* __restrict__ mean_o, float* __restrict__ rstd_o, float slope, BnUpsample up,
                                                                    size_t p_nstride, BnPre pre) {
    extern __shared__ __attribute__((aligned(16))) float bn_mid_plane[];
    __shared__ float red[32];
    const int c = blockIdx.x, img = blockIdx.y;
    gamma += (size_t)img * p_nstride; beta += (size_t)img * p_nstride;
    const float* p = y + (size_t)img * y_nstride + (size_t)c * HW;
    float* q = out + (size_t)img * out_nstride + (size_t)c * HW;
    const bool vec = !(HW & 3) && !((reinterpret_cast<size_t>(p) | reinterpret_cast<size_t>(q)) & 15);
    float s = 0.f, dummy = 0.f;
    if (pre.y && c < pre.C) {
        const float* py1 = pre.y + (size_t)img * pre.y_ns + (size_t)c * HW;
        const bool vec1 = vec && !(reinterpret_cast<size_t>(py1) & 15);
        float s1 = 0.f, d1 = 0.f;
        bn_mid_for(HW, vec1,
                   [&](int i) { const float4 v = reinterpret_cast<const float4*>(py1)[i]; reinterpret_cast<float4*>(bn_mid_plane)[i] = v; s1 += (v.x + v.y) + (v.z + v.w); },
                   [&](int i) { const float v = py1[i]; bn_mid_plane[i] = v; s1 += v; });
        block_sum2_1024(s1, d1, red);
        const float m1 = s1 / (float)HW;
        float q1 = 0.f;
        d1 = 0.f;
        bn_mid_for(HW, vec1,
                   [&](int i) { const float4 v = reinterpret_cast<const float4*>(bn_mid_plane)[i]; const float a = v.x - m1, b = v.y - m1, cc = v.z - m1, d = v.w - m1; q1 += (a * a + b * b) + (cc * cc + d * d); },
                   [&](int i) { const float d = bn_mid_plane[i] - m1; q1 += d * d; });
        block_sum2_1024(q1, d1, red);
        const float r1 = rsqrtf(q1 / (float)HW + eps);
        if (threadIdx.x == 0) { pre.mean[img * pre.C + c] = m1; pre.rstd[img * pre.C + c] = r1; }
        const float sc1 = pre.gamma[(size_t)img * p_nstride + c] * r1;
        const float sh1 = pre.beta[(size_t)img * p_nstride + c] - m1 * sc1;
        float* yo2 = const_cast<float*>(p);
        auto act1 = [&](float x) { const float t = x * sc1 + sh1; float a = t > 0.f ? t : t * pre.slope; rounded(a); return a; };
        bn_mid_for(HW, vec1,
                   [&](int i) {
                       const float4 v = reinterpret_cast<const float4*>(bn_mid_plane)[i];
                       const float4 a = float4{act1(v.x), act1(v.y), act1(v.z), act1(v.w)};
                       reinterpret_cast<float4*>(bn_mid_plane)[i] = a;
                       reinterpret_cast<float4*>(yo2)[i] = a;
                       s += (a.x + a.y) + (a.z + a.w);
                   },
                   [&](int i) { const float a = act1(bn_mid_plane[i]); bn_mid_plane[i] = a; yo2[i] = a; s += a; });
    } else if (up.src && c >= up.c0) {
        const float* sp = up.src + (size_t)img * up.src_ns + (size_t)(c - up.c0) * up.h * up.w;
        float* yo = const_cast<float*>(p);
        const int hw = up.h * up.w;
        const bool in_lds = hw <= BN_MID_SRC;
        float* srcs = bn_mid_plane + ((HW + 3) & ~3);
        if (in_lds) {
            for (int e = threadIdx.x; e < hw; e += BN_MID_THREADS) srcs[e] = sp[e];
            __syncthreads();
        }
        for (int i = threadIdx.x; i < HW; i += BN_MID_THREADS) {
            const int oy = i / up.Wo, ox = i - oy * up.Wo;
            const float v = in_lds ? up_value((const float*)srcs, up.h, up.w, oy, ox) : up_value(sp, up.h, up.w, oy, ox);
            yo[i] = v;
            bn_mid_plane[i] = v;
            s += v;
        }
    } else {
        bn_mid_for(HW, vec,
                   [&](int i) { const float4 v = reinterpret_cast<const float4*>(p)[i]; reinterpret_cast<float4*>(bn_mid_plane)[i] = v; s += (v.x + v.y) + (v.z + v.w); },
                   [&](int i) { const float v = p[i]; bn_mid_plane[i] = v; s += v; });
    }
    block_sum2_1024(s, dummy, red);
    const float m = s / (float)HW;
    float sq = 0.f;
    dummy = 0.f;
    bn_mid_for(HW, vec,
               [&](int i) { const float4 v = reinterpret_cast<const float4*>(bn_mid_plane)[i]; const float a = v.x - m, b = v.y - m, cc = v.z - m, d = v.w - m; sq += (a * a + b * b) + (cc * cc + d * d); },
               [&](int i) { const float d = bn_mid_plane[i] - m; sq += d * d; });
    block_sum2_1024(sq, dummy, red);
    const float r = rsqrtf(sq / (float)HW + eps);
    if (threadIdx.x == 0) { mean_o[img * C + c] = m; rstd_o[img * C + c] = r; }
    const float sc = gamma[c] * r;
    const float sh = beta[c] - m * sc;
    auto act = [&](float x) { const float t = x * sc + sh; return t > 0.f ? t : t * slope; };
    bn_mid_for(HW, vec,
               [&](int i) { const float4 v = reinterpret_cast<const float4*>(bn_mid_plane)[i]; reinterpret_cast<float4*>(q)[i] = float4{act(v.x), act(v.y), act(v.z), act(v.w)}; },
               [&](int i) { q[i] = act(bn_mid_plane[i]); });
}
__global__ __launch_bounds__(BN_MID_THREADS) void bn_mid_bwd_kernel(const float* __restrict__ da, size_t da_nstride, const float* __restrict__ aout, size_t a_nstride,
                                                                    const float* __restrict__ y, size_t y_nstride, float* __restrict__ dy, size_t dy_nstride, int C, int HW,
                                                                    const float* __restrict__ gamma, const float* __restrict__ mean, const float* __restrict__ rstd,
                                                                    float slope, float* __restrict__ dgamma, float* __restrict__ dbeta, int accumulate, BnUpsample up,
                                                                    size_t p_nstride, BnPre pre) {
    extern __shared__ __attribute__((aligned(16))) float bn_mid_plane[];
    __shared__ float red[32];
    const int c = blockIdx.x, img = blockIdx.y;
    gamma += (size_t)img * p_nstride;
    const float m = mean[img * C + c], r = rstd[img * C + c];
    const float* pd = da + (size_t)img * da_nstride + (size_t)c * HW;
    const float* pa = aout + (size_t)img * a_nstride + (size_t)c * HW;
    const float* py = y + (size_t)img * y_nstride + (size_t)c * HW;
    float* po = dy + (size_t)img * dy_nstride + (size_t)c * HW;
    const bool act = slope != 1.0f;
    const bool vec = !(HW & 3) && !((reinterpret_cast<size_t>(pd) | reinterpret_cast<size_t>(pa) | reinterpret_cast<size_t>(py) | reinterpret_cast<size_t>(po)) & 15);
    float s1 = 0.f, s2 = 0.f;
    auto one = [&](float d, float a, float yv) {
        d = bn_dz(d, a, slope, act);
        s1 += d;
        s2 = __builtin_fmaf(d, bn_xhat(yv, m, r), s2);
        return d;
    };
    bn_mid_for(HW, vec,
               [&](int i) {
                   const float4 d = reinterpret_cast<const float4*>(pd)[i], yv = reinterpret_cast<const float4*>(py)[i];
                   const float4 a = act ? reinterpret_cast<const float4*>(pa)[i] : float4{1.f, 1.f, 1.f, 1.f};
                   reinterpret_cast<float4*>(bn_mid_plane)[i] = float4{one(d.x, a.x, yv.x), one(d.y, a.y, yv.y), one(d.z, a.z, yv.z), one(d.w, a.w, yv.w)};
               },
               [&](int i) { bn_mid_plane[i] = one(pd[i], act ? pa[i] : 1.f, py[i]); });
    block_sum2_1024(s1, s2, red);
    const float k1 = s1 / (float)HW, k2 = s2 / (float)HW;
    const float gr = gamma[c] * r;
    const bool through_adjoint = up.d_src && c >= up.c0;
    auto grad = [&](float dz, float yv) { return bn_dy(gr, dz, k1, bn_xhat(yv, m, r), k2); };
    if (pre.y && c < pre.C) {
        const float m1 = pre.mean[img * pre.C + c], r1 = pre.rstd[img * pre.C + c];
        const float* py1 = pre.y + (size_t)img * pre.y_ns + (size_t)c * HW;
        float* pd1 = pre.dy + (size_t)img * pre.y_ns + (size_t)c * HW;
        const bool vec1 = vec && !((reinterpret_cast<size_t>(py1) | reinterpret_cast<size_t>(pd1)) & 15);
        float t1 = 0.f, t2 = 0.f;
        auto one1 = [&](float dzc, float a, float y1) {
            const float d = bn_dz(grad(dzc, a), a, pre.slope, true);
            t1 += d;
            t2 = __builtin_fmaf(d, bn_xhat(y1, m1, r1), t2);
            return d;
        };
        bn_mid_for(HW, vec1,
                   [&](int i) {
                       const float4 dzc = reinterpret_cast<const float4*>(bn_mid_plane)[i], a = reinterpret_cast<const float4*>(py)[i], y1 = reinterpret_cast<const float4*>(py1)[i];
                       reinterpret_cast<float4*>(bn_mid_plane)[i] = float4{one1(dzc.x, a.x, y1.x), one1(dzc.y, a.y, y1.y), one1(dzc.z, a.z, y1.z), one1(dzc.w, a.w, y1.w)};
                   },
                   [&](int i) { bn_mid_plane[i] = one1(bn_mid_plane[i], py[i], py1[i]); });
        block_sum2_1024(t1, t2, red);
        const float j1 = t1 / (float)HW, j2 = t2 / (float)HW;
        const float gr1 = pre.gamma[(size_t)img * p_nstride + c] * r1;
        auto grad1 = [&](float dz, float y1) { return bn_dy(gr1, dz, j1, bn_xhat(y1, m1, r1), j2); };
        bn_mid_for(HW, vec1,
                   [&](int i) {
                       const float4 dz = reinterpret_cast<const float4*>(bn_mid_plane)[i], y1 = reinterpret_cast<const float4*>(py1)[i];
                       reinterpret_cast<float4*>(pd1)[i] = float4{grad1(dz.x, y1.x), grad1(dz.y, y1.y), grad1(dz.z, y1.z), grad1(dz.w, y1.w)};
                   },
                   [&](int i) { pd1[i] = grad1(bn_mid_plane[i], py1[i]); });
        if (threadIdx.x == 0) {
            float* dg = pre.dgamma + (size_t)img * p_nstride + c;
            float* db = pre.dbeta + (size_t)img * p_nstride + c;
            *dg = accumulate ? *dg + t2 : t2;
            *db = accumulate ? *db + t1 : t1;
        }
    } else if (through_adjoint) {
        for (int i = threadIdx.x; i < HW; i += BN_MID_THREADS) bn_mid_plane[i] = grad(bn_mid_plane[i], py[i]);
        __syncthreads();
        float* qd = up.d_src + (size_t)img * up.d_src_ns + (size_t)(c - up.c0) * up.h * up.w;
        for (int e = threadIdx.x; e < up.h * up.w; e += BN_MID_THREADS)
            qd[e] = up_adjoint_value((const float*)bn_mid_plane, up.h, up.w, up.Ho, up.Wo, e / up.w, e % up.w);
    } else {
        bn_mid_for(HW, vec,
                   [&](int i) {
                       const float4 dz = reinterpret_cast<const float4*>(bn_mid_plane)[i], yv = reinterpret_cast<const float4*>(py)[i];
                       reinterpret_cast<float4*>(po)[i] = float4{grad(dz.x, yv.x), grad(dz.y, yv.y), grad(dz.z, yv.z), grad(dz.w, yv.w)};
                   },
                   [&](int i) { po[i] = grad(bn_mid_plane[i], py[i]); });
    }
    if (threadIdx.x == 0) {
        float* dg = dgamma + (size_t)img * p_nstride + c;
        float* db = dbeta + (size_t)img * p_nstride + c;
        *dg = accumulate ? *dg + s2 : s2;
        *db = accumulate ? *db + s1 : s1;
    }
}
static void bn_mid_allow_lds() {
    int dev = 0;
    (void)hipGetDevice(&dev);
    static std::atomic<unsigned long long> done{0};
    const unsigned long long bit = 1ull << (dev & 63);
    if (!(done.load(std::memory_order_relaxed) & bit)) {
        (void)hipFuncSetAttribute((const void*)bn_mid_fwd_kernel, hipFuncAttributeMaxDynamicSharedMemorySize, (BN_MID_HW + BN_MID_SRC) * 4);
        (void)hipFuncSetAttribute((const void*)bn_mid_bwd_kernel, hipFuncAttributeMaxDynamicSharedMemorySize, BN_MID_HW * 4);
        done.fetch_or(bit, std::memory_order_relaxed);
    }
}
#define BN_SMALL_DISPATCH(HW_, KERNEL, GRID, STREAM, ...)                                                         \
    do {                                                                                                          \
        if ((HW_) <= 256) SPLICE_LAUNCH(KERNEL<1>, GRID, dim3(256), 0, STREAM, __VA_ARGS__);                  \
        else if ((HW_) <= 1024) SPLICE_LAUNCH(KERNEL<4>, GRID, dim3(256), 0, STREAM, __VA_ARGS__);            \
        else SPLICE_LAUNCH(KERNEL<16>, GRID, dim3(256), 0, STREAM, __VA_ARGS__);                              \
    } while (0)
int bn_part_floats(int N, int C) { return N * C * MAX_PB_V * 2; }
static inline int bn_plane_blocks(int HW) {
    if (!(HW > MAX_PB * 1024 && (long long)HW <= (long long)MAX_PB_V * BN_V_CH * 1024)) return plane_blocks(HW);
    const int b = cdiv(HW, 4096);
    return b <= MAX_PB ? MAX_PB + 1 : (b > MAX_PB_V ? MAX_PB_V : b);
}
BnForm bn_form(int HW, int N, size_t p_nstride, int batch) {
    static const int chain = getenv("SPLICE_BN_CHAIN") ? atoi(getenv("SPLICE_BN_CHAIN")) : 1;
    static const int bwd_slabs = getenv("SPLICE_BN_BWD_SLABS") ? atoi(getenv("SPLICE_BN_BWD_SLABS")) : 1;
    static const int sign_from_y = getenv("SPLICE_BN_SIGN_FROM_Y") ? atoi(getenv("SPLICE_BN_SIGN_FROM_Y")) : 1;
    const bool own_plane = !batch && (N == 1 || p_nstride);
    BnForm f;
    f.kind = HW <= BN_SMALL_HW ? BnForm::SMALL
           : HW <= BN_MID_HW && own_plane ? BnForm::MID
           : bn_plane_blocks(HW) > MAX_PB ? BnForm::TWO_STAGE_VEC : BnForm::TWO_STAGE;
    const bool one_launch = f.kind == BnForm::SMALL || f.kind == BnForm::MID;
    f.hosts_pre = chain && own_plane && one_launch;
    f.fwd_takes_slabs = f.kind == BnForm::SMALL && !batch;
    f.bwd_takes_slabs = bwd_slabs && f.kind == BnForm::SMALL && own_plane;
    f.fwd_fuses_upsample = !batch;
    f.bwd_fuses_upsample = !batch && one_launch;
    f.sign_from_y = sign_from_y && !batch && f.kind == BnForm::TWO_STAGE_VEC;
    return f;
}
static bool bn_args_ok(const BnArgs& a, const BnForm& f) {
    if (a.batch && (a.batch > BN_MAX_BATCH || a.N % a.batch || (a.N != a.batch && !a.p_nstride))) return false;
    if (a.pre && !f.hosts_pre) return false;
    if (a.slabs && (!f.fwd_takes_slabs || a.ksplit < 2 || a.up || a.pre)) return false;
    if (a.da_slabs && a.da_slabs->slabs && !f.bwd_takes_slabs) return false;
    return true;
}
int bn_fwd_launch(const BnArgs& a, hipStream_t s) {
    const BnForm f = bn_form(a.HW, a.N, a.p_nstride, a.batch);
    if (!bn_args_ok(a, f)) return SPLICE_ERR_ARG;
    const int N = a.N, C = a.C, HW = a.HW;
    const bool fused_up = a.up && f.fwd_fuses_upsample;
    if (a.up && !fused_up) {
        const int rc = upsample2x_fwd_launch(a.up->src, a.up->src_ns, const_cast<float*>(a.y) + (size_t)a.up->c0 * HW, a.y_nstride, N, C - a.up->c0, a.up->h,
                                             a.up->w, a.up->Ho, a.up->Wo, s);
        if (rc != SPLICE_OK) return rc;
    }
    const BnUpsample u = fused_up ? *a.up : BnUpsample{};
    const BnPre pr = a.pre ? *a.pre : BnPre{};
    switch (f.kind) {
    case BnForm::SMALL: {
        const int ksplit = a.slabs ? a.ksplit : 0;
        const float* bias = a.slabs ? a.bias : nullptr;
        float* y_store = a.slabs ? const_cast<float*>(a.y) : nullptr;
        BN_SMALL_DISPATCH(HW, bn_small_fwd_kernel, dim3(C, N), s, a.y, a.y_nstride, a.out, a.out_nstride, C, HW, a.gamma, a.beta, a.eps, a.mean, a.rstd, a.slope,
                          a.slabs, ksplit, bias, y_store, u, a.p_nstride, a.batch, pr);
        break;
    }
    case BnForm::MID:
        bn_mid_allow_lds();
        SPLICE_LAUNCH(bn_mid_fwd_kernel, dim3(C, N), dim3(BN_MID_THREADS), (size_t)(((HW + 3) & ~3) + (u.src ? BN_MID_SRC : 0)) * 4, s, a.y, a.y_nstride, a.out, a.out_nstride, C, HW, a.gamma, a.beta, a.eps, a.mean, a.rstd, a.slope, u, a.p_nstride, pr);
        break;
    case BnForm::TWO_STAGE:
    case BnForm::TWO_STAGE_VEC: {
        const int PB = bn_plane_blocks(HW);
        if (f.kind == BnForm::TWO_STAGE_VEC) SPLICE_LAUNCH(bn_stats_partial_v_kernel, dim3(PB, C, N), dim3(256), 0, s, a.y, a.y_nstride, C, HW, PB, a.part, u);
        else SPLICE_LAUNCH(bn_stats_partial_kernel, dim3(PB, C, N), dim3(256), 0, s, a.y, a.y_nstride, C, HW, PB, a.part, u);
        SPLICE_LAUNCH(bn_act_kernel, dim3(PB, C, N), dim3(256), 0, s, a.y, a.y_nstride, a.out, a.out_nstride, C, HW, PB, a.gamma, a.beta, a.part, a.eps, a.mean, a.rstd, a.slope, a.p_nstride, a.batch);
        break;
    }
    }
    return SPLICE_OK;
}
int bn_bwd_launch(const BnArgs& a, hipStream_t s) {
    const BnForm f = bn_form(a.HW, a.N, a.p_nstride, a.batch);
    if (!bn_args_ok(a, f)) return SPLICE_ERR_ARG;
    const int N = a.N, C = a.C, HW = a.HW;
    const bool fused_up = a.up && f.bwd_fuses_upsample;
    const BnUpsample u = fused_up ? *a.up : BnUpsample{};
    const BnPre pr = a.pre ? *a.pre : BnPre{};
    switch (f.kind) {
    case BnForm::SMALL: {
        const BnSlabs sl = a.da_slabs ? *a.da_slabs : BnSlabs{};
        BN_SMALL_DISPATCH(HW, bn_small_bwd_kernel, dim3(C, N), s, a.da, a.da_nstride, a.out, a.out_nstride, a.y, a.y_nstride, a.dy, a.dy_nstride, C, HW, N,
                          a.gamma, a.mean, a.rstd, a.slope, a.dgamma, a.dbeta, a.accumulate, u, a.p_nstride, a.batch, pr, sl);
        break;
    }
    case BnForm::MID:
        bn_mid_allow_lds();
        SPLICE_LAUNCH(bn_mid_bwd_kernel, dim3(C, N), dim3(BN_MID_THREADS), (size_t)HW * 4, s, a.da, a.da_nstride, a.out, a.out_nstride, a.y, a.y_nstride, a.dy, a.dy_nstride, C, HW, a.gamma, a.mean,
                      a.rstd, a.slope, a.dgamma, a.dbeta, a.accumulate, u, a.p_nstride, pr);
        break;
    case BnForm::TWO_STAGE:
    case BnForm::TWO_STAGE_VEC: {
        const int PB = bn_plane_blocks(HW);
        const float* be = f.sign_from_y ? a.beta : nullptr;
        SPLICE_LAUNCH(bn_bwd_partial_kernel, dim3(PB, C, N), dim3(256), 0, s, a.da, a.da_nstride, a.out, a.out_nstride, a.y, a.y_nstride, C, HW, PB, a.mean, a.rstd, a.slope, a.part, a.gamma, be, a.p_nstride);
        SPLICE_LAUNCH(bn_bwd_apply_kernel, dim3(PB, C, N), dim3(256), 0, s, a.da, a.da_nstride, a.out, a.out_nstride, a.y, a.y_nstride, a.dy,
                           a.dy_nstride, C, HW, N, PB, a.gamma, a.mean, a.rstd, a.slope, a.part, a.dgamma, a.dbeta, a.accumulate, a.p_nstride, a.batch, be);
        break;
    }
    }
    if (a.up && !fused_up)
        return upsample2x_bwd_launch(a.dy + (size_t)a.up->c0 * HW, a.dy_nstride, a.up->d_src, a.up->d_src_ns, N, C - a.up->c0, a.up->h, a.up->w, a.up->Ho, a.up->Wo, s);
    return SPLICE_OK;
}

template <bool MASKED>
__global__ __launch_bounds__(256) void bn_running_update_kernel(RunStatTable t, float* __restrict__ running, size_t r_nstride, float momentum, float eps,
                                                                const splice_stop_state* __restrict__ mask, const int* __restrict__ mask_step) {
    const int bn = blockIdx.x, c = threadIdx.x;
    if (c >= t.C[bn]) return;
    const int step_idx = MASKED ? *mask_step - 1 : 0;
    for (int p = 0; p < t.n_plans; ++p) {
        const bool indep = t.indep[p] != 0;
        if (indep && (int)blockIdx.y >= t.N[p]) continue;
        if (!indep && blockIdx.y != 0) continue;
        if (MASKED && stop_frozen(mask + (indep ? blockIdx.y : 0), step_idx)) continue;
        const int n_lo = indep ? blockIdx.y : 0, n_hi = indep ? blockIdx.y + 1 : t.N[p];
        const int step = t.img_step[p] > 1 ? t.img_step[p] : 1;
        float* arena = running + (indep ? (size_t)blockIdx.y * r_nstride : 0) + t.r_off[bn];
        const float hw = (float)t.HW[p][bn];
        const float unbias = hw > 1.f ? hw / (hw - 1.f) : 1.f;
        for (int n = n_lo; n < n_hi; ++n) {
            const float m = t.mean[p][bn][n * step * t.C[bn] + c], r = t.rstd[p][bn][n * step * t.C[bn] + c];
            const float var = fmaxf(1.0f / (r * r) - eps, 0.f) * unbias;
            arena[c] = (1.f - momentum) * arena[c] + momentum * m;
            arena[t.C[bn] + c] = (1.f - momentum) * arena[t.C[bn] + c] + momentum * var;
        }
    }
}
int bn_running_update_launch(const RunStatTable& t, float* running, size_t r_nstride, float momentum, float eps, int max_images, hipStream_t s,
                             const splice_stop_state* mask, const int* mask_step) {
    if (t.n_plans < 1 || t.n_plans > RUNSTAT_MAX_PLANS || t.n_bn < 1 || t.n_bn > RUNSTAT_MAX_BN || (mask && !mask_step)) return SPLICE_ERR_ARG;
    if (mask) SPLICE_LAUNCH(bn_running_update_kernel<true>, dim3(t.n_bn, max_images), dim3(256), 0, s, t, running, r_nstride, momentum, eps, mask, mask_step);
    else SPLICE_LAUNCH(bn_running_update_kernel<false>, dim3(t.n_bn, max_images), dim3(256), 0, s, t, running, r_nstride, momentum, eps, mask, mask_step);
    return SPLICE_OK;
}
```

### splice_amd/csrc/gen_kernels.h

```cpp
#pragma once
#include "common.h"

struct ConvArgs {
    const float* in;
    const float* w;
    const float* bias;
    float* out;
    size_t in_nstride, in_cstride, out_nstride, out_cstride;
    size_t w_jstride, w_cstride;
    size_t p_nstride;
    int N, Cin, Hi, Wi, Cout, Ho, Wo;
    int ks, stride, pad;
    int reflect;
    int act;
    int transposed;
    int accumulate;
    float* ws;
    size_t ws_floats;
    int ksplit;
    int p_group;
    int defer_reduce;
};
int conv_launch(const ConvArgs& a, hipStream_t s, int* ksplit_out = nullptr);
void conv_form_report(const ConvArgs& a, int* form);
int conv_pair_launch(ConvArgs a, ConvArgs b, hipStream_t s, int* ksplit_a = nullptr, int* ksplit_b = nullptr);
int conv_reflect_dgrad_launch(ConvArgs a, float* pad_scratch, hipStream_t s);

struct WgradArgs {
    const float* x;
    const float* dy;
    float* ws;
    size_t x_nstride, x_cstride, dy_nstride, dy_cstride;
    int N, Cin, Hi, Wi, Cout, Ho, Wo, ks, stride, pad;
    int pix_per_chunk, chunks_per_img;
    int reflect;
};
int wgrad_chunks(int N, int Ho, int Wo, int* pix_per_chunk, int* chunks_per_img);
constexpr int WGRAD_BATCH_MAX = 32;
struct WgradDesc {
    const float* x; const float* dy; float* ws;
    uint32_t x_nstride, x_cstride, dy_nstride, dy_cstride;
    uint16_t Cin, Cout, Hi, Wi, Ho, Wo;
    uint8_t ks, stride, pad, variant;
    uint16_t pix_per_chunk, chunks_per_img;
    uint32_t wg_begin, chunks;
    uint32_t reflect;
};
struct WgradBatch { int count; int total_wgs; WgradDesc d[WGRAD_BATCH_MAX]; };
struct WgradBatchPair { WgradBatch small, big, tile; };
int conv_wgrad_add(WgradBatchPair* b, WgradArgs a, int* chunks_out);
int conv_wgrad_batched_launch(const WgradBatchPair& b, hipStream_t s);

constexpr int WGRAD_MAX_LAYERS = 64;
struct WgradReduceAll {
    long long prefix[WGRAD_MAX_LAYERS + 1];
    long long ws_off[WGRAD_MAX_LAYERS];
    long long dw_off[WGRAD_MAX_LAYERS];
    int n[WGRAD_MAX_LAYERS], chunks[WGRAD_MAX_LAYERS];
    long long total;
    int count;
    unsigned char vec[WGRAD_MAX_LAYERS];
};
int wgrad_reduce_all_launch(const WgradReduceAll& d, const float* ws, float* grads, int accumulate, hipStream_t s, int n_img = 1, size_t p_nstride = 0);

int bn_part_floats(int N, int C);
struct BnUpsample {
    const float* src = nullptr; size_t src_ns = 0;
    float* d_src = nullptr; size_t d_src_ns = 0;
    int c0 = 0, h = 0, w = 0, Ho = 0, Wo = 0;
};
struct BnPre {
    const float* y = nullptr; size_t y_ns = 0;
    const float* slabs = nullptr; int ksplit = 0;
    const float* bias = nullptr;
    const float* gamma = nullptr; const float* beta = nullptr;
    float* mean = nullptr; float* rstd = nullptr;
    float slope = 0.2f;
    int C = 0;
    float* dy = nullptr;
    float* dgamma = nullptr; float* dbeta = nullptr;
};
struct BnSlabs {
    const float* slabs = nullptr;
    int ksplit = 0, accumulate = 0;
};
struct BnForm {
    enum Kind { SMALL, MID, TWO_STAGE, TWO_STAGE_VEC } kind;
    bool hosts_pre;
    bool fwd_takes_slabs;
    bool bwd_takes_slabs;
    bool fwd_fuses_upsample;
    bool bwd_fuses_upsample;
    bool sign_from_y;
};
BnForm bn_form(int HW, int N, size_t p_nstride, int batch);
struct BnArgs {
    const float* y = nullptr; size_t y_nstride = 0;
    float* out = nullptr; size_t out_nstride = 0;
    int N = 0, C = 0, HW = 0;
    const float* gamma = nullptr; const float* beta = nullptr;
    float eps = 0.f, slope = 1.f;
    size_t p_nstride = 0;
    int batch = 0;
    float* part = nullptr;
    float* mean = nullptr; float* rstd = nullptr;
    const BnUpsample* up = nullptr;
    const BnPre* pre = nullptr;
    const float* slabs = nullptr; int ksplit = 0; const float* bias = nullptr;
    const float* da = nullptr; size_t da_nstride = 0;
    float* dy = nullptr; size_t dy_nstride = 0;
    float* dgamma = nullptr; float* dbeta = nullptr;
    int accumulate = 0;
    const BnSlabs* da_slabs = nullptr;
};
int bn_fwd_launch(const BnArgs& a, hipStream_t s);
int bn_bwd_launch(const BnArgs& a, hipStream_t s);
int upsample2x_fwd_launch(const float* in, size_t in_nstride, float* out, size_t out_nstride, int N, int C, int h, int w, int Ho, int Wo, hipStream_t s);
int upsample2x_bwd_launch(const float* dout, size_t dout_nstride, float* din, size_t din_nstride, int N, int C, int h, int w, int Ho, int Wo, hipStream_t s);
int sigmoid_bwd_bias_launch(const float* dout, const float* sout, float* dpre, int N, int C, int HW, float* part, hipStream_t s, size_t p_nstride, int* chunks,
                            int group = 1);
int sigmoid_bias_part_floats(int N, int C);
constexpr int RUNSTAT_MAX_PLANS = 3, RUNSTAT_MAX_BN = 36;
struct RunStatTable {
    int n_plans, n_bn;
    int C[RUNSTAT_MAX_BN], r_off[RUNSTAT_MAX_BN];
    int N[RUNSTAT_MAX_PLANS], indep[RUNSTAT_MAX_PLANS];
    int img_step[RUNSTAT_MAX_PLANS];
    int HW[RUNSTAT_MAX_PLANS][RUNSTAT_MAX_BN];
    const float* mean[RUNSTAT_MAX_PLANS][RUNSTAT_MAX_BN];
    const float* rstd[RUNSTAT_MAX_PLANS][RUNSTAT_MAX_BN];
};
int bn_running_update_launch(const RunStatTable& t, float* running, size_t r_nstride, float momentum, float eps, int max_images, hipStream_t s,
                             const splice_stop_state* mask = nullptr, const int* mask_step = nullptr);
int gen_running_stats_update(void* const* plans, int n_plans, float* running, long long running_stride, float momentum, const splice_stop_state* mask,
                             const int* mask_step, hipStream_t s);
```

### splice_amd/csrc/gen_wgrad.hip

```cpp
#include "gen_device.h"
#include <cstdlib>

constexpr int WG_PC = 64;
constexpr int WG_LD = WG_PC + 2;
constexpr int WG_XS_FLOATS = 3 * 16 * WG_LD;
constexpr int WG_DS_FLOATS = 8 * 16 * WG_LD;
template <int KS, int NI, bool ROWS = false>
__device__ __forceinline__ void conv_wgrad_body(const WgradArgs& a, int chunk, int ktile_in, float* Xs, float* Ds) {
    constexpr int T = ROWS ? KS : KS * KS;
    constexpr int CK = (ROWS || KS == 3) ? 4 : 16;
    constexpr int KT = CK * T;
    const int ktile = ROWS ? ktile_in / KS : ktile_in;
    const int krow = ROWS ? ktile_in % KS : 0;
    constexpr int NJ = (KT + 15) / 16;
    constexpr int PC = WG_PC;
    constexpr int LD = WG_LD;
    constexpr int NQ = (NI * NJ + 3) / 4;
    constexpr int NA = KT / 4;
    constexpr int ND = NI * 16 * PC / 256;
    const int tid = threadIdx.x, lane = tid & 63, wave = tid >> 6;
    const int c0 = ktile * CK;
    const int HWo = a.Ho * a.Wo;
    const int chunks_per_img = a.chunks_per_img;
    const int img = chunk / chunks_per_img, ch_in_img = chunk % chunks_per_img;
    const float* x = a.x + (size_t)img * a.x_nstride + (size_t)c0 * a.x_cstride;
    const float* dy = a.dy + (size_t)img * a.dy_nstride;
    f32x4 acc[NQ];
#pragma unroll
    for (int q = 0; q < NQ; ++q) acc[q] = f32x4{0.f, 0.f, 0.f, 0.f};
    for (int e = tid; e < (NJ * 16 - KT) * LD; e += 256) Xs[KT * LD + e] = 0.f;
    const int pl = tid & 63;
    const int p_begin = ch_in_img * a.pix_per_chunk;
    const int p_end = min(p_begin + a.pix_per_chunk, HWo);
    int g_coff[NA], g_dy[NA], g_dx[NA];
    unsigned g_cok = 0;
#pragma unroll
    for (int i = 0; i < NA; ++i) {
        const int k = wave + 4 * i;
        const int cl = k / T, tap = k % T;
        g_coff[i] = (int)(cl * a.x_cstride);
        g_dy[i] = (ROWS ? krow : tap / KS) - a.pad;
        g_dx[i] = (ROWS ? tap : tap % KS) - a.pad;
        if (c0 + cl < a.Cin) g_cok |= 1u << i;
    }
    float xv[NA], dv[ND];
    const __amdgpu_buffer_rsrc_t rx = __builtin_amdgcn_make_buffer_rsrc(const_cast<float*>(x), 0, 0x7FFFFFFF, 0x00020000);
    const __amdgpu_buffer_rsrc_t rdy = __builtin_amdgcn_make_buffer_rsrc(const_cast<float*>(dy), 0, 0x7FFFFFFF, 0x00020000);
    int d_vo[ND];
#pragma unroll
    for (int t = 0; t < ND; ++t) {
        const int e = tid + 256 * t;
        const int n = e / PC, q = e % PC;
        d_vo[t] = n < a.Cout ? (int)((n * a.dy_cstride + q) * 4) : (int)0x80000000;
    }
    auto fetch = [&](int pb) {
        const int p = pb + pl;
        const bool pvalid = p < p_end;
        const int oy = pvalid ? p / a.Wo : 0, ox = pvalid ? p % a.Wo : 0;
        const int by = oy * a.stride, bx = ox * a.stride;
#pragma unroll
        for (int i = 0; i < NA; ++i) {
            int sy = by + g_dy[i], sx = bx + g_dx[i];
            if (a.reflect) {
                sy = sy < 0 ? -sy : (sy >= a.Hi ? 2 * (a.Hi - 1) - sy : sy);
                sx = sx < 0 ? -sx : (sx >= a.Wi ? 2 * (a.Wi - 1) - sx : sx);
            }
            const bool ok = pvalid && ((g_cok >> i) & 1u) && (unsigned)sy < (unsigned)a.Hi && (unsigned)sx < (unsigned)a.Wi;
            const int vo = ok ? (g_coff[i] + sy * a.Wi + sx) * 4 : (int)0x80000000;
            xv[i] = __builtin_bit_cast(float, __builtin_amdgcn_raw_buffer_load_b32(rx, vo, 0, 0));
        }
        if (pb + PC <= p_end) {
            const int so = __builtin_amdgcn_readfirstlane(pb * 4);
#pragma unroll
            for (int t = 0; t < ND; ++t) dv[t] = __builtin_bit_cast(float, __builtin_amdgcn_raw_buffer_load_b32(rdy, d_vo[t], so, 0));
        } else {
#pragma unroll
            for (int t = 0; t < ND; ++t) {
                const int e = tid + 256 * t;
                const int n = e / PC, q = e % PC;
                const int pp = pb + q;
                dv[t] = (n < a.Cout && pp < p_end) ? dy[(size_t)n * a.dy_cstride + pp] : 0.f;
            }
        }
    };
    fetch(p_begin);
    constexpr int WB = 4, NB = PC / 4 / WB;
    [[maybe_unused]] int lds_rd = (lane & 15) * LD + (lane >> 4);
    for (int pb = p_begin; pb < p_end; pb += PC) {
        if constexpr (NI < 4) asm volatile("" : "+v"(lds_rd));
        __syncthreads();
#pragma unroll
        for (int i = 0; i < NA; ++i) Xs[(wave + 4 * i) * LD + pl] = xv[i];
#pragma unroll
        for (int t = 0; t < ND; ++t) {
            const int e = tid + 256 * t;
            Ds[(e / PC) * LD + (e % PC)] = dv[t];
        }
        __syncthreads();
        if (pb + PC < p_end) fetch(pb + PC);
#pragma unroll
        for (int q = 0; q < NQ; ++q) {
            const int pair = wave + 4 * q;
            if (pair < NI * NJ) {
                const int fi = pair / NJ, fj = pair % NJ;
                if constexpr (NI >= 4) {
#pragma unroll
                    for (int s4 = 0; s4 < PC / 4; ++s4) {
                        const float av = Ds[(fi * 16 + (lane & 15)) * LD + s4 * 4 + (lane >> 4)];
                        const float bv = Xs[(fj * 16 + (lane & 15)) * LD + s4 * 4 + (lane >> 4)];
                        acc[q] = mfma4(av, bv, acc[q]);
                    }
                } else {
                    const int d_rd = lds_rd + fi * 16 * LD, x_rd = lds_rd + fj * 16 * LD;
                    float af[2][WB], bf[2][WB];
#pragma unroll
                    for (int t = 0; t < WB; ++t) { af[0][t] = Ds[d_rd + t * 4]; bf[0][t] = Xs[x_rd + t * 4]; }
#pragma unroll
                    for (int b = 0; b < NB; ++b) {
                        if (b + 1 < NB) {
#pragma unroll
                            for (int t = 0; t < WB; ++t) { af[(b + 1) & 1][t] = Ds[d_rd + ((b + 1) * WB + t) * 4]; bf[(b + 1) & 1][t] = Xs[x_rd + ((b + 1) * WB + t) * 4]; }
                        }
                        __builtin_amdgcn_sched_barrier(0);
#pragma unroll
                        for (int t = 0; t < WB; ++t) acc[q] = mfma4(af[b & 1][t], bf[b & 1][t], acc[q]);
                        __builtin_amdgcn_sched_barrier(0);
                    }
                }
            }
        }
    }
    constexpr int TT = KS * KS;
    float* ws = a.ws + (size_t)chunk * a.Cout * a.Cin * TT;
#pragma unroll
    for (int q = 0; q < NQ; ++q) {
        const int pair = wave + 4 * q;
        if (pair < NI * NJ) {
            const int fi = pair / NJ, fj = pair % NJ;
            const int k = fj * 16 + (lane & 15);
            const int cl = k / T, tap = k % T;
            if (k < KT && c0 + cl < a.Cin) {
#pragma unroll
                for (int r = 0; r < 4; ++r) {
                    const int n = fi * 16 + (lane >> 4) * 4 + r;
                    if (n < a.Cout) ws[((size_t)n * a.Cin + c0 + cl) * TT + (ROWS ? krow * KS + tap : tap)] = acc[q][r];
                }
            }
        }
    }
}

template <class Load>
__device__ __forceinline__ float wgrad_chunk_sum(int chunks, Load&& ld) {
    float s0 = 0.f, s1 = 0.f, s2 = 0.f, s3 = 0.f;
    int c = 0;
    for (; c + 15 < chunks; c += 16) {
        float v[16];
#pragma unroll
        for (int u = 0; u < 16; ++u) v[u] = ld(c + u);
#pragma unroll
        for (int u = 0; u < 16; u += 4) { s0 += v[u]; s1 += v[u + 1]; s2 += v[u + 2]; s3 += v[u + 3]; }
    }
    for (; c + 3 < chunks; c += 4) {
        s0 += ld(c);
        s1 += ld(c + 1);
        s2 += ld(c + 2);
        s3 += ld(c + 3);
    }
    for (; c < chunks; ++c) s0 += ld(c);
    return (s0 + s1) + (s2 + s3);
}
__global__ __launch_bounds__(256) void wgrad_reduce_all_kernel(WgradReduceAll d, const float* __restrict__ ws, float* __restrict__ grads,
                                                               int accumulate, int n_img, size_t p_nstride) {
    const long long gid = (long long)blockIdx.x * 256 + threadIdx.x;
    if (gid >= d.total) return;
    int l = 0;
#pragma unroll 1
    while (l + 1 < d.count && gid >= d.prefix[l + 1]) ++l;
    const bool vec = d.vec[l] != 0;
    const int i = (int)(gid - d.prefix[l]) * (vec ? 4 : 1);
    const int n = d.n[l];
    int chunks = d.chunks[l];
    const float* p = ws + d.ws_off[l] + i;
    if (p_nstride) {
        chunks /= n_img;
        p += (size_t)blockIdx.y * chunks * n;
        grads += (size_t)blockIdx.y * p_nstride;
    }
    float* q = grads + d.dw_off[l] + i;
    if (vec) {
        float4 s = {0.f, 0.f, 0.f, 0.f};
        float4 a0 = s, a1 = s, a2 = s, a3 = s;
        int c = 0;
        for (; c + 7 < chunks; c += 8) {
            float4 v[8];
#pragma unroll
            for (int u = 0; u < 8; ++u) v[u] = *reinterpret_cast<const float4*>(p + (size_t)(c + u) * n);
#pragma unroll
            for (int u = 0; u < 8; u += 4) {
                a0.x += v[u].x; a0.y += v[u].y; a0.z += v[u].z; a0.w += v[u].w;
                a1.x += v[u + 1].x; a1.y += v[u + 1].y; a1.z += v[u + 1].z; a1.w += v[u + 1].w;
                a2.x += v[u + 2].x; a2.y += v[u + 2].y; a2.z += v[u + 2].z; a2.w += v[u + 2].w;
                a3.x += v[u + 3].x; a3.y += v[u + 3].y; a3.z += v[u + 3].z; a3.w += v[u + 3].w;
            }
        }
        for (; c + 3 < chunks; c += 4) {
            const float4 v0 = *reinterpret_cast<const float4*>(p + (size_t)c * n), v1 = *reinterpret_cast<const float4*>(p + (size_t)(c + 1) * n),
                         v2 = *reinterpret_cast<const float4*>(p + (size_t)(c + 2) * n), v3 = *reinterpret_cast<const float4*>(p + (size_t)(c + 3) * n);
            a0.x += v0.x; a0.y += v0.y; a0.z += v0.z; a0.w += v0.w;
            a1.x += v1.x; a1.y += v1.y; a1.z += v1.z; a1.w += v1.w;
            a2.x += v2.x; a2.y += v2.y; a2.z += v2.z; a2.w += v2.w;
            a3.x += v3.x; a3.y += v3.y; a3.z += v3.z; a3.w += v3.w;
        }
        for (; c < chunks; ++c) {
            const float4 v0 = *reinterpret_cast<const float4*>(p + (size_t)c * n);
            a0.x += v0.x; a0.y += v0.y; a0.z += v0.z; a0.w += v0.w;
        }
        s.x = (a0.x + a1.x) + (a2.x + a3.x); s.y = (a0.y + a1.y) + (a2.y + a3.y);
        s.z = (a0.z + a1.z) + (a2.z + a3.z); s.w = (a0.w + a1.w) + (a2.w + a3.w);
        float4* q4 = reinterpret_cast<float4*>(q);
        if (accumulate) { const float4 o = *q4; s.x = o.x + s.x; s.y = o.y + s.y; s.z = o.z + s.z; s.w = o.w + s.w; }
        *q4 = s;
        return;
    }
    const float s = wgrad_chunk_sum(chunks, [&](int c) { return p[(size_t)c * n]; });
    *q = accumulate ? *q + s : s;
}

int wgrad_chunks(int N, int Ho, int Wo, int* pix_per_chunk, int* chunks_per_img) {
    const int HWo = Ho * Wo;
    int ppc = 512;
    if (HWo <= 1024) ppc = 256;
    if (HWo <= 256) ppc = 64;
    if (HWo > 128 * 512) ppc = (cdiv(HWo, 128) + 63) / 64 * 64;
    *pix_per_chunk = ppc;
    *chunks_per_img = cdiv(HWo, ppc);
    return N * *chunks_per_img;
}

template <bool BIG>
__global__ __launch_bounds__(256, 2) void conv_wgrad_batched_kernel(WgradBatch b) {
    __shared__ float Xs[WG_XS_FLOATS];
    __shared__ float Ds[(BIG ? 8 : 2) * 16 * WG_LD];
    int l = 0;
#pragma unroll 1
    while (l + 1 < b.count && blockIdx.x >= b.d[l + 1].wg_begin) ++l;
    const WgradDesc& d = b.d[l];
    WgradArgs a;
    a.x = d.x; a.dy = d.dy; a.ws = d.ws;
    a.x_nstride = d.x_nstride; a.x_cstride = d.x_cstride; a.dy_nstride = d.dy_nstride; a.dy_cstride = d.dy_cstride;
    a.N = 0; a.Cin = d.Cin; a.Hi = d.Hi; a.Wi = d.Wi; a.Cout = d.Cout; a.Ho = d.Ho; a.Wo = d.Wo;
    a.ks = d.ks; a.stride = d.stride; a.pad = d.pad; a.pix_per_chunk = d.pix_per_chunk; a.chunks_per_img = d.chunks_per_img;
    a.reflect = (int)d.reflect;
    const int local = blockIdx.x - d.wg_begin;
    const int chunk = local % d.chunks, ktile = local / d.chunks;
    if (BIG) {
        switch (d.variant) {
            case 2: conv_wgrad_body<1, 4>(a, chunk, ktile, Xs, Ds); break;
            case 3: conv_wgrad_body<1, 8>(a, chunk, ktile, Xs, Ds); break;
            case 6: conv_wgrad_body<3, 4>(a, chunk, ktile, Xs, Ds); break;
            case 7: conv_wgrad_body<3, 8>(a, chunk, ktile, Xs, Ds); break;
            case 10: conv_wgrad_body<5, 4, true>(a, chunk, ktile, Xs, Ds); break;
            case 11: conv_wgrad_body<5, 8, true>(a, chunk, ktile, Xs, Ds); break;
            case 14: conv_wgrad_body<7, 4, true>(a, chunk, ktile, Xs, Ds); break;
            default: conv_wgrad_body<7, 8, true>(a, chunk, ktile, Xs, Ds); break;
        }
    } else {
        switch (d.variant) {
            case 0: conv_wgrad_body<1, 1>(a, chunk, ktile, Xs, Ds); break;
            case 1: conv_wgrad_body<1, 2>(a, chunk, ktile, Xs, Ds); break;
            case 4: conv_wgrad_body<3, 1>(a, chunk, ktile, Xs, Ds); break;
            case 5: conv_wgrad_body<3, 2>(a, chunk, ktile, Xs, Ds); break;
            case 8: conv_wgrad_body<5, 1, true>(a, chunk, ktile, Xs, Ds); break;
            case 9: conv_wgrad_body<5, 2, true>(a, chunk, ktile, Xs, Ds); break;
            case 12: conv_wgrad_body<7, 1, true>(a, chunk, ktile, Xs, Ds); break;
            default: conv_wgrad_body<7, 2, true>(a, chunk, ktile, Xs, Ds); break;
        }
    }
}

constexpr int WT_CK = 8, WT_NJ = 5, WT_PH = 6, WT_PLANE = WT_PH * CT_PW, WT_PE = WT_CK * WT_PLANE, WT_NP = (WT_PE + 255) / 256;
template <int NI>
__device__ __forceinline__ void conv_wgrad_tile_body(const WgradDesc& d, int chunk, int ktile, int nb , float* Ps) {
    const int tid = threadIdx.x, lane = tid & 63, wave = __builtin_amdgcn_readfirstlane(tid >> 6);
    const int Cin = d.Cin, Cout = d.Cout, Hi = d.Hi, Wi = d.Wi, Ho = d.Ho, Wo = d.Wo, pad = d.pad;
    const int img = chunk / d.chunks_per_img, strip = chunk % d.chunks_per_img;
    const int tiles_x = (Wo + CT_TW - 1) / CT_TW, tiles_y = (Ho + 3) / 4, T = tiles_x * tiles_y;
    const int t_begin = (int)((long long)strip * T / d.chunks_per_img), t_end = (int)((long long)(strip + 1) * T / d.chunks_per_img);
    const int c0 = ktile * WT_CK;
    const float* x = d.x + (size_t)img * d.x_nstride + (size_t)c0 * d.x_cstride;
    const float* dy = d.dy + (size_t)img * d.dy_nstride;
    const __amdgpu_buffer_rsrc_t rx = __builtin_amdgcn_make_buffer_rsrc(const_cast<float*>(x), 0, 0x7FFFFFFF, 0x00020000);
    const __amdgpu_buffer_rsrc_t rdy = __builtin_amdgcn_make_buffer_rsrc(const_cast<float*>(dy), 0, 0x7FFFFFFF, 0x00020000);
    int p_rel[WT_NP];
#pragma unroll
    for (int j = 0; j < WT_NP; ++j) {
        const int e = tid + 256 * j;
        const int c = e / WT_PLANE, rem = e % WT_PLANE, r = rem / CT_PW, xx = rem % CT_PW;
        p_rel[j] = (e < WT_PE && c0 + c < Cin) ? (int)(c * d.x_cstride + (unsigned)(r * Wi + xx)) * 4 : (int)0x80000000;
    }
    int b_base[WT_NJ];
#pragma unroll
    for (int jf = 0; jf < WT_NJ; ++jf) {
        const int j = jf * 16 + (lane & 15);
        const int cl = j / 9, tap = j % 9;
        b_base[jf] = (j < WT_CK * 9 ? cl * WT_PLANE + (tap / 3) * CT_PW + tap % 3 : 0) + wave * CT_PW + 4 * (lane >> 4);
    }
    int dy_off[NI];
#pragma unroll
    for (int fi = 0; fi < NI; ++fi) {
        const int n = nb + fi * 16 + (lane & 15);
        dy_off[fi] = n < Cout ? (int)(n * d.dy_cstride) * 4 : (int)0x80000000;
    }
    f32x4 acc[NI][WT_NJ];
#pragma unroll
    for (int fi = 0; fi < NI; ++fi)
#pragma unroll
        for (int jf = 0; jf < WT_NJ; ++jf) acc[fi][jf] = f32x4{0.f, 0.f, 0.f, 0.f};
    float pv[WT_NP];
    float dyn[NI][4][4], dyc[NI][4][4];
    auto fetch = [&](int t) __attribute__((always_inline)) {
        const int ty = t / tiles_x, tx = t - ty * tiles_x;
        const int y0 = ty * 4, x0 = tx * CT_TW, sy0 = y0 - pad, sx0 = x0 - pad;
        const bool interior = sy0 >= 0 && sx0 >= 0 && sy0 + WT_PH <= Hi && sx0 + CT_PW <= Wi;
        if (interior) {
            const int so = __builtin_amdgcn_readfirstlane((sy0 * Wi + sx0) * 4);
#pragma unroll
            for (int j = 0; j < WT_NP; ++j) pv[j] = __builtin_bit_cast(float, __builtin_amdgcn_raw_buffer_load_b32(rx, p_rel[j], so, 0));
        } else {
#pragma unroll
            for (int j = 0; j < WT_NP; ++j) {
                const int e = tid + 256 * j;
                const int c = e / WT_PLANE, rem = e % WT_PLANE, r = rem / CT_PW, xx = rem % CT_PW;
                int sy = sy0 + r, sx = sx0 + xx;
                if (d.reflect) {
                    sy = sy < 0 ? -sy : (sy >= Hi ? 2 * (Hi - 1) - sy : sy);
                    sx = sx < 0 ? -sx : (sx >= Wi ? 2 * (Wi - 1) - sx : sx);
                }
                const bool ok = p_rel[j] >= 0 && sy >= 0 && sy < Hi && sx >= 0 && sx < Wi;
                pv[j] = __builtin_bit_cast(float, __builtin_amdgcn_raw_buffer_load_b32(rx, ok ? (int)(c * d.x_cstride + (unsigned)(sy * Wi + sx)) * 4 : (int)0x80000000, 0, 0));
            }
        }
        const int row = y0 + wave;
        const int col0 = x0 + 4 * (lane >> 4);
#pragma unroll
        for (int fi = 0; fi < NI; ++fi)
#pragma unroll
            for (int q = 0; q < 4; ++q) {
                const int col = col0 + 16 * q;
                const bool ok = row < Ho && col < Wo && dy_off[fi] >= 0;
                const u32x4 v = __builtin_bit_cast(u32x4, __builtin_amdgcn_raw_buffer_load_b128(rdy, ok ? dy_off[fi] + (row * Wo + col) * 4 : (int)0x80000000, 0, 0));
#pragma unroll
                for (int tt = 0; tt < 4; ++tt) dyn[fi][q][tt] = col + tt < Wo ? __uint_as_float(v[tt]) : 0.f;
            }
    };
    if (t_begin < t_end) fetch(t_begin);
    for (int t = t_begin; t < t_end; ++t) {
        asm volatile("" : "+v"(b_base[0]), "+v"(b_base[1]), "+v"(b_base[2]), "+v"(b_base[3]), "+v"(b_base[4]));
        __syncthreads();
#pragma unroll
        for (int j = 0; j < WT_NP; ++j)
            if (tid + 256 * j < WT_PE) Ps[tid + 256 * j] = pv[j];
#pragma unroll
        for (int fi = 0; fi < NI; ++fi)
#pragma unroll
            for (int q = 0; q < 4; ++q)
#pragma unroll
                for (int tt = 0; tt < 4; ++tt) dyc[fi][q][tt] = dyn[fi][q][tt];
        __syncthreads();
        if (t + 1 < t_end) fetch(t + 1);
        float bv[2][WT_NJ];
#pragma unroll
        for (int jf = 0; jf < WT_NJ; ++jf) bv[0][jf] = Ps[b_base[jf]];
#pragma unroll
        for (int st = 0; st < 16; ++st) {
            if (st + 1 < 16) {
#pragma unroll
                for (int jf = 0; jf < WT_NJ; ++jf) bv[(st + 1) & 1][jf] = Ps[b_base[jf] + 16 * ((st + 1) >> 2) + ((st + 1) & 3)];
            }
            __builtin_amdgcn_sched_barrier(0);
#pragma unroll
            for (int fi = 0; fi < NI; ++fi)
#pragma unroll
                for (int jf = 0; jf < WT_NJ; ++jf) acc[fi][jf] = mfma4(dyc[fi][st >> 2][st & 3], bv[st & 1][jf], acc[fi][jf]);
            __builtin_amdgcn_sched_barrier(0);
        }
    }
    __syncthreads();
    constexpr int NV = NI * WT_NJ * 4;
    if (wave > 0) {
#pragma unroll
        for (int fi = 0; fi < NI; ++fi)
#pragma unroll
            for (int jf = 0; jf < WT_NJ; ++jf)
#pragma unroll
                for (int r = 0; r < 4; ++r) Ps[((wave - 1) * NV + (fi * WT_NJ + jf) * 4 + r) * 64 + lane] = acc[fi][jf][r];
    }
    __syncthreads();
    if (wave > 0) return;
    float* ws = d.ws + (size_t)chunk * Cout * Cin * 9;
#pragma unroll
    for (int fi = 0; fi < NI; ++fi)
#pragma unroll
        for (int jf = 0; jf < WT_NJ; ++jf) {
            const int j = jf * 16 + (lane & 15);
            const int cl = j / 9, tap = j % 9;
#pragma unroll
            for (int r = 0; r < 4; ++r) {
                float v = acc[fi][jf][r];
#pragma unroll
                for (int w = 0; w < 3; ++w) v += Ps[(w * NV + (fi * WT_NJ + jf) * 4 + r) * 64 + lane];
                const int n = nb + fi * 16 + (lane >> 4) * 4 + r;
                if (j < WT_CK * 9 && c0 + cl < Cin && n < Cout) ws[((size_t)n * Cin + c0 + cl) * 9 + tap] = v;
            }
        }
}
constexpr int WT_LDS_FLOATS = 3 * 2 * WT_NJ * 4 * 64 > WT_PE ? 3 * 2 * WT_NJ * 4 * 64 : WT_PE;
__global__ __launch_bounds__(256) void conv_wgrad_tile_kernel(WgradBatch b) {
    __shared__ float Ps[WT_LDS_FLOATS];
    int l = 0;
#pragma unroll 1
    while (l + 1 < b.count && blockIdx.x >= b.d[l + 1].wg_begin) ++l;
    const WgradDesc& d = b.d[l];
    const int local = blockIdx.x - d.wg_begin;
    const int chunk = local % d.chunks, kt_all = local / d.chunks, ktiles_c = (d.Cin + WT_CK - 1) / WT_CK;
    const int ktile = kt_all % ktiles_c, nb = (kt_all / ktiles_c) * 32;
    if (d.variant == 1) conv_wgrad_tile_body<1>(d, chunk, ktile, nb, Ps);
    else conv_wgrad_tile_body<2>(d, chunk, ktile, nb, Ps);
}
static bool wgrad_tile_ok(const WgradArgs& a) {
    static const int on = getenv("SPLICE_WGRAD_TILE") ? atoi(getenv("SPLICE_WGRAD_TILE")) : 1;
    constexpr int min_px = 40000;
    return on && a.ks == 3 && a.stride == 1 && a.Wo >= 64 && (long long)a.Ho * a.Wo > min_px && a.Hi == a.Ho && a.Wi == a.Wo && a.pad == 1 &&
           (size_t)a.Cin * a.x_cstride <= 0x1fffffffULL && (size_t)a.Cout * a.dy_cstride <= 0x1fffffffULL;
}

int conv_wgrad_add(WgradBatchPair* pair, WgradArgs a, int* chunks_out) {
    const bool tile = wgrad_tile_ok(a);
    WgradBatch* b = tile ? &pair->tile : a.Cout > 32 ? &pair->big : &pair->small;
    if (a.Cout > 128 || (a.ks != 1 && a.ks != 3 && a.ks != 5 && a.ks != 7) || b->count >= WGRAD_BATCH_MAX) return SPLICE_ERR_ARG;
    if ((size_t)a.Cin * a.x_cstride > 0x7fffffffULL || a.x_nstride > 0xffffffffULL || a.dy_nstride > 0xffffffffULL) return SPLICE_ERR_ARG;
    if (a.Hi > 65535 || a.Wi > 65535 || a.Cin > 65535) return SPLICE_ERR_ARG;
    const int chunks = wgrad_chunks(a.N, a.Ho, a.Wo, &a.pix_per_chunk, &a.chunks_per_img);
    const int CK = tile ? WT_CK : a.ks == 1 ? 16 : 4;
    const int ktiles = cdiv(a.Cin, CK) * (a.ks >= 5 ? a.ks : 1) * (tile ? cdiv(a.Cout, 32) : 1);
    const int ni = cdiv(a.Cout, 16);
    WgradDesc& d = b->d[b->count++];
    d.x = a.x; d.dy = a.dy; d.ws = a.ws;
    d.x_nstride = (uint32_t)a.x_nstride; d.x_cstride = (uint32_t)a.x_cstride; d.dy_nstride = (uint32_t)a.dy_nstride; d.dy_cstride = (uint32_t)a.dy_cstride;
    d.Cin = (uint16_t)a.Cin; d.Cout = (uint16_t)a.Cout; d.Hi = (uint16_t)a.Hi; d.Wi = (uint16_t)a.Wi; d.Ho = (uint16_t)a.Ho; d.Wo = (uint16_t)a.Wo;
    d.ks = (uint8_t)a.ks; d.stride = (uint8_t)a.stride; d.pad = (uint8_t)a.pad;
    d.variant = (uint8_t)((a.ks == 3 ? 4 : a.ks == 5 ? 8 : a.ks == 7 ? 12 : 0) + (ni <= 1 ? 0 : ni <= 2 ? 1 : ni <= 4 ? 2 : 3));
    if (tile) d.variant = (uint8_t)(ni < 2 ? 1 : 2);
    d.reflect = (uint32_t)(a.reflect ? 1 : 0);
    d.pix_per_chunk = (uint16_t)a.pix_per_chunk; d.chunks_per_img = (uint16_t)a.chunks_per_img;
    d.wg_begin = (uint32_t)b->total_wgs; d.chunks = (uint32_t)chunks;
    b->total_wgs += chunks * ktiles;
    if (chunks_out) *chunks_out = chunks;
    return SPLICE_OK;
}
int conv_wgrad_batched_launch(const WgradBatchPair& p, hipStream_t s) {
    if (p.big.count > 0) SPLICE_LAUNCH(conv_wgrad_batched_kernel<true>, dim3((unsigned)p.big.total_wgs), dim3(256), 0, s, p.big);
    if (p.small.count > 0) SPLICE_LAUNCH(conv_wgrad_batched_kernel<false>, dim3((unsigned)p.small.total_wgs), dim3(256), 0, s, p.small);
    if (p.tile.count > 0) SPLICE_LAUNCH(conv_wgrad_tile_kernel, dim3((unsigned)p.tile.total_wgs), dim3(256), 0, s, p.tile);
    return SPLICE_OK;
}

int wgrad_reduce_all_launch(const WgradReduceAll& d0, const float* ws, float* grads, int accumulate, hipStream_t s, int n_img, size_t p_nstride) {
    if (d0.count < 1 || d0.count > WGRAD_MAX_LAYERS) return SPLICE_ERR_ARG;
    WgradReduceAll d = d0;
    static const int vec_on = getenv("SPLICE_WGRAD_REDUCE_VEC") ? atoi(getenv("SPLICE_WGRAD_REDUCE_VEC")) : 1;
    const bool base_ok = vec_on && !((reinterpret_cast<size_t>(ws) | reinterpret_cast<size_t>(grads)) & 15) && p_nstride % 4 == 0;
    d.prefix[0] = 0;
    for (int i = 0; i < d.count; ++i) {
        const bool v = base_ok && d.n[i] % 4 == 0 && d.ws_off[i] % 4 == 0 && d.dw_off[i] % 4 == 0;
        d.vec[i] = v ? 1 : 0;
        d.prefix[i + 1] = d.prefix[i] + (v ? d.n[i] / 4 : d.n[i]);
    }
    d.total = d.prefix[d.count];
    SPLICE_LAUNCH(wgrad_reduce_all_kernel, dim3((unsigned)((d.total + 255) / 256), p_nstride ? n_img : 1), dim3(256), 0, s, d, ws, grads, accumulate,
                       n_img, p_nstride);
    return SPLICE_OK;
}
```

Measured before the change: 265.8.

## Specialize small BN kernels by feature flags and deepen wgrad reduce batching

Templates the small batch-norm forward and backward kernels on a compile-time feature mask, so unused paths (batch, slabs, pre-chain, upsample, tail) are compiled out, along with their shared memory and registers. The dispatcher picks the smallest instance that covers the call. The change also hoists the chained-BN loads earlier, splits the slab loop into full groups plus a remainder, and adds asm barriers to limit rematerialization. The wgrad reduce kernel gets a 32-wide load batch to put more loads in flight, and replaces the serial layer search with a lane-parallel readlane scan. A standalone wgrad_reduce entry point and a test hook for forcing a BN instance are also exposed; the price is more template instances and higher register pressure in the 32-wide loops.

Result: faster. 270.8 (median of 6 runs) (+1.9%).

```diff
diff --git a/include/splice_hip.h b/include/splice_hip.h
--- a/include/splice_hip.h
+++ b/include/splice_hip.h
@@ -336,6 +336,7 @@
 size_t splice_gen_conv_wgrad_ws_floats(int N, int Cin, int Cout, int ks, int Ho, int Wo);
 int splice_gen_conv_wgrad(const splice_gen_wgrad_args* args, float* dw, int accumulate, int n_img, size_t p_nstride, int* form_out,
                           splice_stream_t stream);
+int splice_gen_wgrad_reduce(const float* partials, int n, int chunks, float* dw, int accumulate, int n_img, size_t p_nstride, splice_stream_t stream);
 
 typedef struct splice_gen_bn_args {
     float* y;
@@ -384,6 +385,7 @@
 size_t splice_gen_bn_part_floats(int N, int C);
 int splice_gen_bn_fwd(const splice_gen_bn_args* args, splice_stream_t stream);
 int splice_gen_bn_bwd(const splice_gen_bn_args* args, splice_stream_t stream);
+int splice_gen_bn_small_instance(int mask);
 
 int splice_gen_upsample2x_fwd(const float* in, size_t in_nstride, float* out, size_t out_nstride, int N, int C, int h, int w, int Ho, int Wo,
                               splice_stream_t stream);
diff --git a/splice_amd/_lib.py b/splice_amd/_lib.py
--- a/splice_amd/_lib.py
+++ b/splice_amd/_lib.py
@@ -134,6 +134,8 @@
     "splice_gen_conv_reflect_dgrad": ([C.POINTER(GenConvArgs), _vp, _sz, _vp], _i),
     "splice_gen_conv_wgrad_ws_floats": ([_i, _i, _i, _i, _i, _i], _sz),
     "splice_gen_conv_wgrad": ([C.POINTER(GenWgradArgs), _vp, _i, _i, _sz, C.POINTER(_i), _vp], _i),
+    "splice_gen_wgrad_reduce": ([_vp, _i, _i, _vp, _i, _i, _sz, _vp], _i),
+    "splice_gen_bn_small_instance": ([_i], _i),
     "splice_gen_bn_form": ([_i, _i, _sz, _i, C.POINTER(_i)], _i),
     "splice_gen_bn_part_floats": ([_i, _i], _sz),
     "splice_gen_bn_fwd": ([C.POINTER(GenBnArgs), _vp], _i),
diff --git a/splice_amd/csrc/capi.hip b/splice_amd/csrc/capi.hip
--- a/splice_amd/csrc/capi.hip
+++ b/splice_amd/csrc/capi.hip
@@ -309,6 +309,16 @@
     return finish(wgrad_reduce_all_launch(r, args->ws, dw, accumulate, ST(stream), n_img, p_nstride), who);
 }
 
+int splice_gen_wgrad_reduce(const float* partials, int n, int chunks, float* dw, int accumulate, int n_img, size_t p_nstride, splice_stream_t stream) {
+    const char* who = "splice_gen_wgrad_reduce";
+    if (!partials || !dw || n < 1 || chunks < 0 || n_img < 1 || n_img > 65535 || (long long)n * (chunks > 0 ? chunks : 1) > 0x7fffffffLL) return finish(SPLICE_ERR_ARG, who);
+    if (p_nstride ? (chunks % n_img || p_nstride < (size_t)n) : n_img != 1) return finish(SPLICE_ERR_ARG, who);
+    WgradReduceAll r = {};
+    r.count = 1; r.n[0] = n; r.chunks[0] = chunks; r.ws_off[0] = 0; r.dw_off[0] = 0;
+    return finish(wgrad_reduce_all_launch(r, partials, dw, accumulate, ST(stream), n_img, p_nstride), who);
+}
+
+int splice_gen_bn_small_instance(int mask) { return finish(bn_small_force_instance(mask), "splice_gen_bn_small_instance"); }
 int splice_gen_bn_form(int HW, int N, size_t p_nstride, int batch, int* out) {
     if (HW < 1 || N < 1 || batch < 0 || !out) return finish(SPLICE_ERR_ARG, "splice_gen_bn_form");
     const BnForm f = bn_form(HW, N, p_nstride, batch);
diff --git a/splice_amd/csrc/gen_bn.hip b/splice_amd/csrc/gen_bn.hip
--- a/splice_amd/csrc/gen_bn.hip
+++ b/splice_amd/csrc/gen_bn.hip
@@ -387,11 +387,20 @@
     rounded(g);
     return g;
 }
+__device__ __forceinline__ int bn_fresh(int hw) { asm volatile("" : "+s"(hw)); return hw; }
 constexpr int BN_SMALL_HW = 4096;
 constexpr int BN_MAX_BATCH = 8;
 constexpr int BN_SMALL_PER = BN_SMALL_HW / 256;
 constexpr int BN_UP_SRC = 34 * 34;
-template <int PER>
+enum : unsigned {
+    BN_F_BATCH = 1,
+    BN_F_TAIL = 2,
+    BN_F_SLABS = 4,
+    BN_F_PRE = 8,
+    BN_F_UP = 16,
+    BN_F_ALL = 31
+};
+template <int PER, unsigned F>
 __global__ __launch_bounds__(256) void bn_small_fwd_kernel(const float* y, size_t y_nstride, float* __restrict__ out,
                                                            size_t out_nstride, int C, int HW, const float* __restrict__ gamma,
                                                            const float* __restrict__ beta, float eps, float* __restrict__ mean_o,
@@ -399,17 +408,18 @@
                                                            int ksplit, const float* __restrict__ bias, float* __restrict__ y_out, BnUpsample up,
                                                            size_t p_nstride, int batch, BnPre pre) {
     __shared__ float red[8];
-    __shared__ float up_src_s[BN_UP_SRC];
+    __shared__ float up_src_s[(F & BN_F_UP) ? BN_UP_SRC : 1];
     const int c = blockIdx.x, img = blockIdx.y;
+    if (!(F & BN_F_BATCH)) batch = 0;
     gamma += bn_arena(img, p_nstride, batch); beta += bn_arena(img, p_nstride, batch);
     if (bias) bias += bn_arena(img, p_nstride, batch);
     const float* p = y + (size_t)img * y_nstride + (size_t)c * HW;
     float* q = out + (size_t)img * out_nstride + (size_t)c * HW;
     float v[PER];
     float s = 0.f, dummy = 0.f;
-    if (pre.y && c < pre.C) {
+    if ((F & BN_F_PRE) && pre.y && c < pre.C) {
         const float* py1 = pre.y + (size_t)img * pre.y_ns + (size_t)c * HW;
-        if (pre.slabs) {
+        if ((F & BN_F_SLABS) && pre.slabs) {
             const size_t per = (size_t)gridDim.y * pre.C * HW;
             const float* sp = pre.slabs + ((size_t)img * pre.C + c) * HW;
             float* yo = const_cast<float*>(py1);
@@ -479,7 +489,7 @@
             if (i < HW) yo2[i] = v[k];
             s += v[k];
         }
-    } else if (slabs) {
+    } else if ((F & BN_F_SLABS) && slabs) {
         const size_t per = (size_t)gridDim.y * C * HW;
         const float* sp = slabs + ((size_t)img * C + c) * HW;
         float* yo = y_out + (size_t)img * y_nstride + (size_t)c * HW;
@@ -513,7 +523,7 @@
             if (i < HW) yo[i] = v[k]; else v[k] = 0.f;
             s += v[k];
         }
-    } else if (up.src && c >= up.c0) {
+    } else if ((F & BN_F_UP) && up.src && c >= up.c0) {
         const float* sp = up.src + (size_t)img * up.src_ns + (size_t)(c - up.c0) * up.h * up.w;
         float* yo = const_cast<float*>(p);
         const bool in_lds = up.h * up.w <= BN_UP_SRC;
@@ -609,25 +619,36 @@
                                                   const float* sp = nullptr, size_t per = 0, int ksplit = 0, int sl_acc = 0) {
     s1 = 0.f; s2 = 0.f;
     const bool act = slope != 1.0f;
+    const float* pa_ld = act ? pa : py;
     float vd[PER], va[PER], vy[PER];
 #pragma unroll
     for (int k = 0; k < PER; ++k) {
         if (k * 256 >= HW) continue;
         const int i = threadIdx.x + k * 256;
         const int j = i < HW ? i : 0;
-        vd[k] = (!sp || sl_acc) ? pd[j] : 0.f;
         vy[k] = py[j];
-        va[k] = act ? pa[j] : 1.f;
+        va[k] = pa_ld[j];
+    }
+    if (!sp || sl_acc) {
+#pragma unroll
+        for (int k = 0; k < PER; ++k) {
+            if (k * 256 >= HW) continue;
+            const int i = threadIdx.x + k * 256;
+            vd[k] = pd[i < HW ? i : 0];
+        }
+    } else {
+#pragma unroll
+        for (int k = 0; k < PER; ++k) vd[k] = 0.f;
     }
     if (sp) {
         float v[PER];
 #pragma unroll
         for (int k = 0; k < PER; ++k) v[k] = 0.f;
-        for (int ks = 0; ks < ksplit; ks += 4) {
+        auto group = [&](int ks, int nu) {
             float t[4][PER];
 #pragma unroll
             for (int u = 0; u < 4; ++u) {
-                if (ks + u >= ksplit) continue;
+                if (u >= nu) continue;
                 const float* sk = sp + (size_t)(ks + u) * per;
 #pragma unroll
                 for (int k = 0; k < PER; ++k) {
@@ -638,21 +659,26 @@
             }
 #pragma unroll
             for (int u = 0; u < 4; ++u) {
-                if (ks + u >= ksplit) continue;
+                if (u >= nu) continue;
 #pragma unroll
                 for (int k = 0; k < PER; ++k)
                     if (k * 256 < HW) v[k] += t[u][k];
             }
-        }
+        };
+        int ks = 0;
+        for (; ks + 3 < ksplit; ks += 4) group(ks, 4);
+        if (ks < ksplit) group(ks, ksplit - ks);
 #pragma unroll
         for (int k = 0; k < PER; ++k)
             if (k * 256 < HW) vd[k] = sl_acc ? vd[k] + v[k] : v[k];
     }
+    if (PER > 4) HW = bn_fresh(HW);
 #pragma unroll
     for (int k = 0; k < PER; ++k) {
         const int i = threadIdx.x + k * 256;
         float d = 0.f, x = 0.f;
         if (k * 256 < HW) {
+            rounded(va[k]);
             d = bn_dz(vd[k], va[k], slope, act);
             x = bn_xhat(vy[k], m, r);
             if (i >= HW) { d = 0.f; x = 0.f; }
@@ -663,7 +689,7 @@
     }
     block_sum2(s1, s2, red);
 }
-template <int PER>
+template <int PER, unsigned F>
 __global__ __launch_bounds__(256) void bn_small_bwd_kernel(const float* __restrict__ da, size_t da_nstride, const float* __restrict__ aout,
                                                            size_t a_nstride, const float* __restrict__ y, size_t y_nstride,
                                                            float* __restrict__ dy, size_t dy_nstride, int C, int HW, int N,
@@ -672,17 +698,36 @@
                                                            float* __restrict__ dbeta, int accumulate, BnUpsample up, size_t p_nstride, int batch, BnPre pre,
                                                            BnSlabs sl) {
     __shared__ float red[8];
-    __shared__ float up_grad_s[BN_SMALL_HW];
+    __shared__ float up_grad_s[(F & BN_F_UP) ? BN_SMALL_HW : 1];
     const int c = blockIdx.x, img = blockIdx.y;
+    if (!(F & BN_F_BATCH)) batch = 0;
     gamma += bn_arena(img, p_nstride, batch);
     const int n0 = batch ? img / batch * batch : 0;
     float dz[PER], xh[PER];
     float s1, s2;
-    const bool chained = pre.y && c < pre.C;
+    const bool chained = (F & BN_F_PRE) && pre.y && c < pre.C;
+    constexpr int CPER = (F & BN_F_PRE) ? PER : 1;
+    float cva[CPER], cvy[CPER];
+    float m1 = 0.f, r1 = 0.f, g1 = 0.f;
+    if constexpr ((F & BN_F_PRE) != 0) {
+        if (chained) {
+            m1 = pre.mean[img * pre.C + c]; r1 = pre.rstd[img * pre.C + c]; g1 = pre.gamma[(size_t)img * p_nstride + c];
+            const float* pa1 = y + (size_t)img * y_nstride + (size_t)c * HW;
+            const float* py1 = pre.y + (size_t)img * pre.y_ns + (size_t)c * HW;
+#pragma unroll
+            for (int k = 0; k < PER; ++k) {
+                if (k * 256 >= HW) continue;
+                const int i = threadIdx.x + k * 256, j = i < HW ? i : 0;
+                cva[k] = pa1[j];
+                cvy[k] = py1[j];
+            }
+            asm volatile("" : : : "memory");
+        }
+    }
     {
         const float m = mean[img * C + c], r = rstd[img * C + c];
         float b1 = 0.f, b2 = 0.f;
-        if (batch) {
+        if ((F & BN_F_BATCH) && batch) {
             float t1s[BN_MAX_BATCH], t2s[BN_MAX_BATCH];
 #pragma unroll
             for (int n = 0; n < BN_MAX_BATCH; ++n) {
@@ -700,14 +745,15 @@
         } else {
             bn_small_bwd_sums<PER>(da + (size_t)img * da_nstride + (size_t)c * HW, aout + (size_t)img * a_nstride + (size_t)c * HW,
                               y + (size_t)img * y_nstride + (size_t)c * HW, HW, m, r, slope, dz, xh, s1, s2, red,
-                              sl.slabs ? sl.slabs + ((size_t)img * C + c) * HW : nullptr, (size_t)gridDim.y * C * HW, sl.ksplit, sl.accumulate);
+                              (F & BN_F_SLABS) && sl.slabs ? sl.slabs + ((size_t)img * C + c) * HW : nullptr, (size_t)gridDim.y * C * HW, sl.ksplit, sl.accumulate);
         }
         const float cnt = batch ? (float)HW * (float)batch : (float)HW;
         const float k1 = (batch ? b1 : s1) / cnt, k2 = (batch ? b2 : s2) / cnt;
         if (batch) { s1 = b1; s2 = b2; }
         const float gr = gamma[c] * r;
         float* po = dy + (size_t)img * dy_nstride + (size_t)c * HW;
-        const bool through_adjoint = up.d_src && c >= up.c0;
+        const bool through_adjoint = (F & BN_F_UP) && up.d_src && c >= up.c0;
+        if (PER > 4) HW = bn_fresh(HW);
 #pragma unroll
         for (int k = 0; k < PER; ++k) {
             const int i = threadIdx.x + k * 256;
@@ -716,26 +762,17 @@
                 if (through_adjoint) up_grad_s[i] = gv; else if (chained) dz[k] = gv; else po[i] = gv;
             } else if (chained) dz[k] = 0.f;
         }
-        if (chained) {
-            const float m1 = pre.mean[img * pre.C + c], r1 = pre.rstd[img * pre.C + c];
-            const float* pa1 = y + (size_t)img * y_nstride + (size_t)c * HW;
-            const float* py1 = pre.y + (size_t)img * pre.y_ns + (size_t)c * HW;
-            float va[PER], vy[PER];
-#pragma unroll
-            for (int k = 0; k < PER; ++k) {
-                if (k * 256 >= HW) continue;
-                const int i = threadIdx.x + k * 256, j = i < HW ? i : 0;
-                va[k] = pa1[j];
-                vy[k] = py1[j];
-            }
+        if constexpr ((F & BN_F_PRE) != 0) if (chained) {
             float t1 = 0.f, t2 = 0.f;
+            if (PER > 4) HW = bn_fresh(HW);
 #pragma unroll
             for (int k = 0; k < PER; ++k) {
                 const int i = threadIdx.x + k * 256;
                 float d = 0.f, x = 0.f;
                 if (k * 256 < HW && i < HW) {
-                    d = bn_dz(dz[k], va[k], pre.slope, true);
-                    x = bn_xhat(vy[k], m1, r1);
+                    rounded(cva[k]);
+                    d = bn_dz(dz[k], cva[k], pre.slope, true);
+                    x = bn_xhat(cvy[k], m1, r1);
                 }
                 dz[k] = d; xh[k] = x;
                 t1 += d;
@@ -743,8 +780,9 @@
             }
             block_sum2(t1, t2, red);
             const float j1 = t1 / (float)HW, j2 = t2 / (float)HW;
-            const float gr1 = pre.gamma[(size_t)img * p_nstride + c] * r1;
+            const float gr1 = g1 * r1;
             float* pd1 = pre.dy + (size_t)img * pre.y_ns + (size_t)c * HW;
+            if (PER > 4) HW = bn_fresh(HW);
 #pragma unroll
             for (int k = 0; k < PER; ++k) {
                 const int i = threadIdx.x + k * 256;
@@ -775,7 +813,7 @@
     }
     if (img != 0) return;
     float g = s2, be = s1;
-    for (int n = 1; n < (batch ? 0 : N); ++n) {
+    for (int n = 1; n < ((F & BN_F_TAIL) && !batch ? N : 0); ++n) {
         float t1, t2;
         bn_small_bwd_sums<PER>(da + (size_t)n * da_nstride + (size_t)c * HW, aout + (size_t)n * a_nstride + (size_t)c * HW,
                           y + (size_t)n * y_nstride + (size_t)c * HW, HW, mean[n * C + c], rstd[n * C + c], slope, dz, xh, t1, t2, red);
@@ -991,12 +1029,38 @@
         done.fetch_or(bit, std::memory_order_relaxed);
     }
 }
-#define BN_SMALL_DISPATCH(HW_, KERNEL, GRID, STREAM, ...)                                                         \
+static const unsigned BN_SMALL_INSTANCES[] = {0, BN_F_SLABS, BN_F_UP, BN_F_PRE | BN_F_UP, BN_F_PRE | BN_F_UP | BN_F_SLABS, BN_F_BATCH, BN_F_TAIL, BN_F_ALL};
+static std::atomic<int> g_bn_small_forced{-1};
+int bn_small_force_instance(int mask) {
+    if (mask < 0) { g_bn_small_forced.store(-1); return SPLICE_OK; }
+    for (unsigned m : BN_SMALL_INSTANCES)
+        if ((unsigned)mask == m) { g_bn_small_forced.store(mask); return SPLICE_OK; }
+    return SPLICE_ERR_ARG;
+}
+static int bn_small_instance(unsigned need) {
+    const int forced = g_bn_small_forced.load(std::memory_order_relaxed);
+    if (forced >= 0) return (need & ~(unsigned)forced) ? -1 : forced;
+    for (unsigned m : BN_SMALL_INSTANCES)
+        if (!(need & ~m)) return (int)m;
+    return (int)BN_F_ALL;
+}
+#define BN_SMALL_PER_DISPATCH(HW_, KERNEL, F_, GRID, STREAM, ...)                                                 \
     do {                                                                                                          \
-        if ((HW_) <= 256) SPLICE_LAUNCH(KERNEL<1>, GRID, dim3(256), 0, STREAM, __VA_ARGS__);                  \
-        else if ((HW_) <= 1024) SPLICE_LAUNCH(KERNEL<4>, GRID, dim3(256), 0, STREAM, __VA_ARGS__);            \
-        else SPLICE_LAUNCH(KERNEL<16>, GRID, dim3(256), 0, STREAM, __VA_ARGS__);                              \
+        if ((HW_) <= 256) SPLICE_LAUNCH((KERNEL<1, F_>), GRID, dim3(256), 0, STREAM, __VA_ARGS__);            \
+        else if ((HW_) <= 1024) SPLICE_LAUNCH((KERNEL<4, F_>), GRID, dim3(256), 0, STREAM, __VA_ARGS__);      \
+        else SPLICE_LAUNCH((KERNEL<16, F_>), GRID, dim3(256), 0, STREAM, __VA_ARGS__);                        \
     } while (0)
+#define BN_SMALL_DISPATCH(INST_, HW_, KERNEL, GRID, STREAM, ...)                                                                      \
+    switch (INST_) {                                                                                                                  \
+    case 0: BN_SMALL_PER_DISPATCH(HW_, KERNEL, 0u, GRID, STREAM, __VA_ARGS__); break;                                                \
+    case BN_F_SLABS: BN_SMALL_PER_DISPATCH(HW_, KERNEL, BN_F_SLABS, GRID, STREAM, __VA_ARGS__); break;                               \
+    case BN_F_UP: BN_SMALL_PER_DISPATCH(HW_, KERNEL, BN_F_UP, GRID, STREAM, __VA_ARGS__); break;                                     \
+    case BN_F_PRE | BN_F_UP: BN_SMALL_PER_DISPATCH(HW_, KERNEL, BN_F_PRE | BN_F_UP, GRID, STREAM, __VA_ARGS__); break;               \
+    case BN_F_PRE | BN_F_UP | BN_F_SLABS: BN_SMALL_PER_DISPATCH(HW_, KERNEL, BN_F_PRE | BN_F_UP | BN_F_SLABS, GRID, STREAM, __VA_ARGS__); break; \
+    case BN_F_BATCH: BN_SMALL_PER_DISPATCH(HW_, KERNEL, BN_F_BATCH, GRID, STREAM, __VA_ARGS__); break;                               \
+    case BN_F_TAIL: BN_SMALL_PER_DISPATCH(HW_, KERNEL, BN_F_TAIL, GRID, STREAM, __VA_ARGS__); break;                                 \
+    default: BN_SMALL_PER_DISPATCH(HW_, KERNEL, BN_F_ALL, GRID, STREAM, __VA_ARGS__); break;                                         \
+    }
 int bn_part_floats(int N, int C) { return N * C * MAX_PB_V * 2; }
 static inline int bn_plane_blocks(int HW) {
     if (!(HW > MAX_PB * 1024 && (long long)HW <= (long long)MAX_PB_V * BN_V_CH * 1024)) return plane_blocks(HW);
@@ -1045,7 +1109,9 @@
         const int ksplit = a.slabs ? a.ksplit : 0;
         const float* bias = a.slabs ? a.bias : nullptr;
         float* y_store = a.slabs ? const_cast<float*>(a.y) : nullptr;
-        BN_SMALL_DISPATCH(HW, bn_small_fwd_kernel, dim3(C, N), s, a.y, a.y_nstride, a.out, a.out_nstride, C, HW, a.gamma, a.beta, a.eps, a.mean, a.rstd, a.slope,
+        const int inst = bn_small_instance((a.batch ? BN_F_BATCH : 0) | (a.slabs || pr.slabs ? BN_F_SLABS : 0) | (pr.y ? BN_F_PRE : 0) | (u.src ? BN_F_UP : 0));
+        if (inst < 0) return SPLICE_ERR_ARG;
+        BN_SMALL_DISPATCH(inst, HW, bn_small_fwd_kernel, dim3(C, N), s, a.y, a.y_nstride, a.out, a.out_nstride, C, HW, a.gamma, a.beta, a.eps, a.mean, a.rstd, a.slope,
                           a.slabs, ksplit, bias, y_store, u, a.p_nstride, a.batch, pr);
         break;
     }
@@ -1074,7 +1140,10 @@
     switch (f.kind) {
     case BnForm::SMALL: {
         const BnSlabs sl = a.da_slabs ? *a.da_slabs : BnSlabs{};
-        BN_SMALL_DISPATCH(HW, bn_small_bwd_kernel, dim3(C, N), s, a.da, a.da_nstride, a.out, a.out_nstride, a.y, a.y_nstride, a.dy, a.dy_nstride, C, HW, N,
+        const int inst = bn_small_instance((a.batch ? BN_F_BATCH : 0) | (!a.batch && !a.p_nstride && N > 1 ? BN_F_TAIL : 0) | (sl.slabs ? BN_F_SLABS : 0) |
+                                           (pr.y ? BN_F_PRE : 0) | (u.d_src ? BN_F_UP : 0));
+        if (inst < 0) return SPLICE_ERR_ARG;
+        BN_SMALL_DISPATCH(inst, HW, bn_small_bwd_kernel, dim3(C, N), s, a.da, a.da_nstride, a.out, a.out_nstride, a.y, a.y_nstride, a.dy, a.dy_nstride, C, HW, N,
                           a.gamma, a.mean, a.rstd, a.slope, a.dgamma, a.dbeta, a.accumulate, u, a.p_nstride, a.batch, pr, sl);
         break;
     }
diff --git a/splice_amd/csrc/gen_kernels.h b/splice_amd/csrc/gen_kernels.h
--- a/splice_amd/csrc/gen_kernels.h
+++ b/splice_amd/csrc/gen_kernels.h
@@ -115,6 +115,7 @@
 };
 int bn_fwd_launch(const BnArgs& a, hipStream_t s);
 int bn_bwd_launch(const BnArgs& a, hipStream_t s);
+int bn_small_force_instance(int mask);
 int upsample2x_fwd_launch(const float* in, size_t in_nstride, float* out, size_t out_nstride, int N, int C, int h, int w, int Ho, int Wo, hipStream_t s);
 int upsample2x_bwd_launch(const float* dout, size_t dout_nstride, float* din, size_t din_nstride, int N, int C, int h, int w, int Ho, int Wo, hipStream_t s);
 int sigmoid_bwd_bias_launch(const float* dout, const float* sout, float* dpre, int N, int C, int HW, float* part, hipStream_t s, size_t p_nstride, int* chunks,
diff --git a/splice_amd/csrc/gen_wgrad.hip b/splice_amd/csrc/gen_wgrad.hip
--- a/splice_amd/csrc/gen_wgrad.hip
+++ b/splice_amd/csrc/gen_wgrad.hip
@@ -32,11 +32,12 @@
     const int pl = tid & 63;
     const int p_begin = ch_in_img * a.pix_per_chunk;
     const int p_end = min(p_begin + a.pix_per_chunk, HWo);
+    const int wave_g = (KS == 3 && NI == 8) ? __builtin_amdgcn_readfirstlane(wave) : wave;
     int g_coff[NA], g_dy[NA], g_dx[NA];
     unsigned g_cok = 0;
 #pragma unroll
     for (int i = 0; i < NA; ++i) {
-        const int k = wave + 4 * i;
+        const int k = wave_g + 4 * i;
         const int cl = k / T, tap = k % T;
         g_coff[i] = (int)(cl * a.x_cstride);
         g_dy[i] = (ROWS ? krow : tap / KS) - a.pad;
@@ -150,10 +151,21 @@
     }
 }
 
+__device__ __forceinline__ void wgrad_loaded(float& x) { asm volatile("" : "+v"(x) : : "memory"); }
 template <class Load>
 __device__ __forceinline__ float wgrad_chunk_sum(int chunks, Load&& ld) {
     float s0 = 0.f, s1 = 0.f, s2 = 0.f, s3 = 0.f;
     int c = 0;
+#pragma unroll 1
+    for (; c + 31 < chunks; c += 32) {
+        float v[32];
+#pragma unroll
+        for (int u = 0; u < 32; ++u) v[u] = ld(c + u);
+#pragma unroll
+        for (int u = 0; u < 32; ++u) wgrad_loaded(v[u]);
+#pragma unroll
+        for (int u = 0; u < 32; u += 4) { s0 += v[u]; s1 += v[u + 1]; s2 += v[u + 2]; s3 += v[u + 3]; }
+    }
     for (; c + 15 < chunks; c += 16) {
         float v[16];
 #pragma unroll
@@ -173,25 +185,48 @@
 __global__ __launch_bounds__(256) void wgrad_reduce_all_kernel(WgradReduceAll d, const float* __restrict__ ws, float* __restrict__ grads,
                                                                int accumulate, int n_img, size_t p_nstride) {
     const long long gid = (long long)blockIdx.x * 256 + threadIdx.x;
+    static_assert(WGRAD_MAX_LAYERS <= 64, "one lane per layer");
+    const int lj = min((int)(threadIdx.x & 63), d.count - 1);
+    const long long hi_j = d.prefix[lj + 1], lo_j = d.prefix[lj], wso_j = d.ws_off[lj], dwo_j = d.dw_off[lj];
+    const int n_j = d.n[lj], chunks_j = d.chunks[lj], vec_j = d.vec[lj];
+    int l = 0;
+    for (int k = 0; k + 1 < d.count; ++k) {
+        const unsigned lo = (unsigned)__builtin_amdgcn_readlane((int)hi_j, k);
+        const int hi = __builtin_amdgcn_readlane((int)(hi_j >> 32), k);
+        l += gid >= (long long)(((unsigned long long)(unsigned)hi << 32) | lo) ? 1 : 0;
+    }
+    const long long first = __shfl(lo_j, l), ws_off = __shfl(wso_j, l), dw_off = __shfl(dwo_j, l);
+    const int n = __shfl(n_j, l);
+    int chunks = __shfl(chunks_j, l);
+    const bool vec = __shfl(vec_j, l) != 0;
     if (gid >= d.total) return;
-    int l = 0;
-#pragma unroll 1
-    while (l + 1 < d.count && gid >= d.prefix[l + 1]) ++l;
-    const bool vec = d.vec[l] != 0;
-    const int i = (int)(gid - d.prefix[l]) * (vec ? 4 : 1);
-    const int n = d.n[l];
-    int chunks = d.chunks[l];
-    const float* p = ws + d.ws_off[l] + i;
+    const int i = (int)(gid - first) * (vec ? 4 : 1);
+    const float* p = ws + ws_off + i;
     if (p_nstride) {
         chunks /= n_img;
         p += (size_t)blockIdx.y * chunks * n;
         grads += (size_t)blockIdx.y * p_nstride;
     }
-    float* q = grads + d.dw_off[l] + i;
+    float* q = grads + dw_off + i;
     if (vec) {
         float4 s = {0.f, 0.f, 0.f, 0.f};
         float4 a0 = s, a1 = s, a2 = s, a3 = s;
         int c = 0;
+#pragma unroll 1
+        for (; c + 31 < chunks; c += 32) {
+            float4 v[32];
+#pragma unroll
+            for (int u = 0; u < 32; ++u) v[u] = *reinterpret_cast<const float4*>(p + (size_t)(c + u) * n);
+#pragma unroll
+            for (int u = 0; u < 32; ++u) { wgrad_loaded(v[u].x); wgrad_loaded(v[u].y); wgrad_loaded(v[u].z); wgrad_loaded(v[u].w); }
+#pragma unroll
+            for (int u = 0; u < 32; u += 4) {
+                a0.x += v[u].x; a0.y += v[u].y; a0.z += v[u].z; a0.w += v[u].w;
+                a1.x += v[u + 1].x; a1.y += v[u + 1].y; a1.z += v[u + 1].z; a1.w += v[u + 1].w;
+                a2.x += v[u + 2].x; a2.y += v[u + 2].y; a2.z += v[u + 2].z; a2.w += v[u + 2].w;
+                a3.x += v[u + 3].x; a3.y += v[u + 3].y; a3.z += v[u + 3].z; a3.w += v[u + 3].w;
+            }
+        }
         for (; c + 7 < chunks; c += 8) {
             float4 v[8];
 #pragma unroll
```
